# katotetsuro/chainer-maskrcnn

Measured on AMD Instinct MI355X. Metric: images/sec (1024^2 COCO, bs=2/GPU) at 1/2/4/8 MI355X; ROIAlign bwd HBM GB/s, higher is better.
Workload: dtype f32

## Files before the change

chainer-maskrcnn_amd/chainer_maskrcnn/_hip/nn.py:

```python
import torch

from chainer_maskrcnn import _hip
from chainer_maskrcnn._hip import lib, check, ptr, stream_ptr

_ws_cache = {}

PROFILE = None
LOGICAL = None


class _prof(object):
    def __init__(self, kind, n_out_pix, KH, KW, cin, cout, geom=None):
        self.on = PROFILE is not None
        if self.on:
            pass_ = {'fwd': 0, 'bwd_data': 1, 'bwd_filter': 2}[kind]
            executed = lib().mrcnn_conv2d_executed_macs(*geom, pass_) if geom is not None else n_out_pix * KH * KW * cin * cout
            if LOGICAL is not None:
                cin, cout = LOGICAL
            self.rec = [kind, n_out_pix * KH * KW * cin * cout, torch.cuda.Event(enable_timing=True),
                        torch.cuda.Event(enable_timing=True), (n_out_pix, KH, cin, cout), executed, geom,
                        winograd_pass_tiles(),
                        split_operands()]

    def __enter__(self):
# ... 35 lines not shown
    import ctypes
    t = (ctypes.c_int * 3)()
    check(lib().mrcnn_conv2d_get_winograd_pass_tiles(t))
    return (t[0], t[1], t[2])


def split_operands():
    import ctypes
    t = (ctypes.c_int * 3)()
    check(lib().mrcnn_conv2d_get_split_operands(t))
    return (t[0], t[1], t[2])


def set_winograd_pass_tiles(fwd, bwd_data, bwd_filter):
    check(lib().mrcnn_conv2d_set_winograd_pass_tiles(int(fwd), int(bwd_data), int(bwd_filter)))


def conv_out(n, k, s, p):
    return (n + 2 * p - k) // s + 1


CONV_PLAN_FIELDS = ('path', 'bm', 'bn', 'ksplit', 'tail_ks', 'wino_m', 'smallc', 'arithmetic', 'plane_gemm')
CONV_PATHS = ('direct', 'split_k', 'tail_split', 'winograd')


def conv_plan(pass_, x_shape, w_shape, stride, pad):
    import ctypes
    N, H, W, Cin = x_shape
    Cout, KH, KW, _ = w_shape
    out = (ctypes.c_int * len(CONV_PLAN_FIELDS))()
    check(lib().mrcnn_conv2d_plan_query(int(pass_), N, H, W, Cin, Cout, KH, KW, stride, pad, out, len(CONV_PLAN_FIELDS)))
    return dict(zip(CONV_PLAN_FIELDS, out))


def conv2d_fwd_raw(x, w, b, stride, pad, relu, keep_v=False):
    _hip.require_cuda(x, w)
    N, H, W, Cin = x.shape
    Cout, KH, KW, Cin2 = w.shape
    assert Cin == Cin2, (x.shape, w.shape)
    assert x.is_contiguous() and w.is_contiguous()
    y = torch.empty((N, conv_out(H, KH, stride, pad), conv_out(W, KW, stride, pad), Cout),
                    dtype=torch.float32, device=x.device)
    nb = lib().mrcnn_conv2d_workspace_bytes(N, H, W, Cin, Cout, KH, KW, stride, pad)
    ws = workspace(nb, x.device) if nb else None
    v = None
    if keep_v:
        vb = lib().mrcnn_conv2d_winograd_v_bytes(N, H, W, Cin, Cout, KH, KW, stride, pad)
        if vb:
            v = torch.empty((vb // 4,), dtype=torch.float32, device=x.device)
    with _prof('fwd', N * y.shape[1] * y.shape[2], KH, KW, Cin, Cout, (N, H, W, Cin, Cout, KH, KW, stride, pad)):
        check(lib().mrcnn_conv2d_fwd_f32(ptr(x), ptr(w), ptr(b), ptr(y), N, H, W, Cin, Cout, KH, KW,
                                         stride, pad, int(relu), ptr(v), ptr(ws), ws.numel() if ws is not None else 0, stream_ptr()))
    return (y, v) if keep_v else y


def conv2d_fwd_bnstats_raw(x, w, stride, pad, keep_v=False):
    N, H, W, Cin = x.shape
    Cout, KH, KW, _ = w.shape
    rows = lib().mrcnn_conv2d_bnstats_rows(N, H, W, Cin, Cout, KH, KW, stride, pad)
    if rows == 0:
        return None
    assert x.is_contiguous() and w.is_contiguous()
    y = torch.empty((N, conv_out(H, KH, stride, pad), conv_out(W, KW, stride, pad), Cout), dtype=torch.float32, device=x.device)
    part = torch.empty((rows, 2, Cout), dtype=torch.float32, device=x.device)
    nb = lib().mrcnn_conv2d_workspace_bytes(N, H, W, Cin, Cout, KH, KW, stride, pad)
    ws = workspace(nb, x.device) if nb else None
    v = None
    if keep_v:
        vb = lib().mrcnn_conv2d_winograd_v_bytes(N, H, W, Cin, Cout, KH, KW, stride, pad)
        if vb:
            v = torch.empty((vb // 4,), dtype=torch.float32, device=x.device)
    with _prof('fwd', N * y.shape[1] * y.shape[2], KH, KW, Cin, Cout, (N, H, W, Cin, Cout, KH, KW, stride, pad)):
        check(lib().mrcnn_conv2d_fwd_bnstats_f32(ptr(x), ptr(w), ptr(y), N, H, W, Cin, Cout, KH, KW, stride, pad, ptr(part), ptr(v),
                                                 ptr(ws), ws.numel() if ws is not None else 0, stream_ptr()))
    return y, v, part


def winograd_w_bytes(x_shape, w_shape, stride, pad):
    N, H, W, Cin = x_shape
    Cout, KH, KW, _ = w_shape
    return lib().mrcnn_conv2d_winograd_w_bytes(N, H, W, Cin, Cout, KH, KW, stride, pad)


def conv2d_bwd_data_raw(gy, w, x_shape, stride, pad, out=None, relu_x=None, emit_w=False, gb=None, gb_accumulate=False):
    N, H, W, Cin = x_shape
    Cout, KH, KW, _ = w.shape
    assert gy.is_contiguous()
    acc = out is not None
    gx = out if acc else torch.empty(x_shape, dtype=torch.float32, device=gy.device)
    nb = lib().mrcnn_conv2d_workspace_bytes(N, H, W, Cin, Cout, KH, KW, stride, pad)
    ws = workspace(nb, gy.device) if nb else None
    wt = None
    if emit_w:
        wb = lib().mrcnn_conv2d_winograd_w_bytes(N, H, W, Cin, Cout, KH, KW, stride, pad)
        assert wb > 0, 'emit_w: the layer does not take the Winograd path'
        wt = torch.empty((wb // 4,), dtype=torch.float32, device=gy.device)
    with _prof('bwd_data', N * gy.shape[1] * gy.shape[2], KH, KW, Cin, Cout, (N, H, W, Cin, Cout, KH, KW, stride, pad)):
        check(lib().mrcnn_conv2d_bwd_data_f32(ptr(gy), ptr(w), ptr(gx), ptr(relu_x), N, H, W, Cin, Cout, KH, KW,
                                              stride, pad, int(acc), ptr(wt), ptr(gb) if emit_w else None, int(gb_accumulate),
                                              ptr(ws), ws.numel() if ws is not None else 0, stream_ptr()))
    return (gx, wt) if emit_w else gx


def conv2d_bwd_filter_raw(x, gy, w_shape, stride, pad, want_bias, gw=None, gb=None, accumulate=None, wino_v=None,
                          wino_w=None):
    N, H, W, Cin = x.shape
    Cout, KH, KW, _ = w_shape
    assert gy.is_contiguous() and x.is_contiguous()
    acc = (gw is not None) if accumulate is None else bool(accumulate)
    if gw is None:
        gw = torch.empty(w_shape, dtype=torch.float32, device=x.device)
        gb = torch.empty((Cout,), dtype=torch.float32, device=x.device) if want_bias else None
    nbytes = lib().mrcnn_conv2d_bwd_filter_workspace_bytes(N, H, W, Cin, Cout, KH, KW, stride, pad)
    ws = workspace(nbytes, x.device)
    with _prof('bwd_filter', N * gy.shape[1] * gy.shape[2], KH, KW, Cin, Cout, (N, H, W, Cin, Cout, KH, KW, stride, pad)):
        check(lib().mrcnn_conv2d_bwd_filter_f32(ptr(x), ptr(gy), ptr(gw), ptr(gb) if want_bias else None, N, H, W, Cin,
                                                Cout, KH, KW, stride, pad, int(acc), ptr(wino_v), ptr(wino_w), ptr(ws), ws.numel(),
                                                stream_ptr()))
    return gw, gb
```

chainer-maskrcnn_amd/chainer_maskrcnn/model/fpn_maskrcnn_train_chain.py:

```python
import numpy as np
import torch

from chainer_maskrcnn._hip import ops
from chainer_maskrcnn.utils.proposal_target_creator import ProposalTargetCreator


class AnchorTargetCreator(object):

    def __init__(self, n_sample=256, pos_iou_thresh=0.7, neg_iou_thresh=0.3, pos_ratio=0.5):
        self.n_sample, self.pos_iou_thresh, self.neg_iou_thresh, self.pos_ratio = n_sample, pos_iou_thresh, neg_iou_thresh, pos_ratio
        self.keys = ops.KeyStream(1 << 32)

    seed = property(lambda self: self.keys.seed)

    def set_seed(self, seed, device=None):
        self.keys.set_seed(seed, device)

    def __call__(self, bbox, anchor, img_size, n_gt=None, keys=None, per_image_hw=None):
        if bbox.dim() == 2:
            bbox = bbox[None]
        N, G, _ = bbox.shape
        if n_gt is None:
            n_gt = torch.full((N,), G, dtype=torch.int32, device=bbox.device)
        if keys is None:
# ... 78 lines not shown


def select_gemm_arithmetic(name):
    from chainer_maskrcnn._hip import lib, check
    from chainer_maskrcnn.nn import core
    split, backbone_fwd = GEMM_ARITHMETIC[name]
    check(lib().mrcnn_conv2d_set_split_operands(*split))
    core.FWD_EMULATION_IN_BACKBONE = bool(backbone_fwd)


class _PendingBackward(object):

    def __init__(self, features, g_locs, g_scores, g_box, g_mask, g_later, g_iou, point, early_rpn):
        self.features = features
        self.g_locs, self.g_scores = g_locs, g_scores
        self.g_box, self.g_mask = g_box, g_mask
        self.g_later = g_later
        self.g_iou = g_iou
        self.point = point
        self.early_rpn = early_rpn

    def seeds(self):
        return ([self.g_locs, self.g_scores, self.g_box, self.g_mask] + list(self.g_later) + ([self.g_iou] if self.g_iou is not None else [])
                + ([self.point['g_pred']] if self.point is not None else []))


class FPNMaskRCNNTrainChain(object):
    EARLY_RPN_BACKWARD = True
    ACCUMULATE_INTO_EARLY_RPN = True

    def __init__(self, faster_rcnn, mask_loss_fun=calc_mask_loss, binary_mask=True, rpn_sigma=3., roi_sigma=1.,
                 anchor_target_creator=None, strict_batch1=False, mask_rows='positives', gemm_arithmetic=None,
                 box_loss='smooth_l1', rpn_box_loss='smooth_l1', box_loss_weight=1.0, rpn_box_loss_weight=1.0, mask_iou_weight=1.0,
                 point_loss_weight=1.0):
        box_loss_settings(box_loss, rpn_box_loss, box_loss_weight, rpn_box_loss_weight)
        self.mask_iou_weight = mask_iou_weight_setting(mask_iou_weight)
        self.point_loss_weight = point_loss_weight_setting(point_loss_weight)
        self.box_loss, self.rpn_box_loss = box_loss, rpn_box_loss
        self.box_loss_weight, self.rpn_box_loss_weight = float(box_loss_weight), float(rpn_box_loss_weight)
        if gemm_arithmetic is not None and gemm_arithmetic not in GEMM_ARITHMETIC:
            raise ValueError('gemm_arithmetic must be one of %s' % sorted(GEMM_ARITHMETIC))
        self.gemm_arithmetic = gemm_arithmetic
        self.faster_rcnn = faster_rcnn
        self.proposal_target_creator = ProposalTargetCreator(faster_rcnn.extractor.anchor_sizes)
        self.anchor_target_creator = AnchorTargetCreator()
        cascade = getattr(faster_rcnn, 'cascade', None)
        if cascade is not None and cascade[0][0] != float(self.proposal_target_creator.pos_iou_thresh):
            raise ValueError('cascade_ious[0] = %r is not the sampler\'s pos_iou_thresh %r'
                             % (cascade[0][0], self.proposal_target_creator.pos_iou_thresh))
        self.rpn_sigma, self.roi_sigma = 3., 1.
        self.loc_normalize_mean = faster_rcnn.loc_normalize_mean
        self.loc_normalize_std = faster_rcnn.loc_normalize_std
        if not callable(mask_loss_fun):
            raise TypeError('mask_loss_fun must be callable: f(roi_cls_mask, gt_roi_mask, xp, gt_roi_label) -> loss')
        self.mask_loss_fun = mask_loss_fun
        self.mask_loss_kind = getattr(mask_loss_fun, 'fused_kind', None)
        if self.mask_loss_kind not in ('mask_bce', 'keypoint_ce'):
            self.mask_loss_kind = 'generic'
        if getattr(faster_rcnn, 'maskiou_head', None) is not None and self.mask_loss_kind != 'mask_bce':
            raise ValueError('a mask_iou model trains with the fused binary mask loss (calc_mask_loss): a user-supplied mask_loss_fun '
                             're-orders the mask rows, which the MaskIoU target does not follow')
        if getattr(faster_rcnn, 'point_head', None) is not None and self.mask_loss_kind != 'mask_bce':
            raise ValueError('a point_rend model trains with the fused binary mask loss (calc_mask_loss): a user-supplied mask_loss_fun '
                             're-orders the mask rows, which the point targets do not follow')
        self.unit_upstream = False
        self.backward_follows = False
        self.binary_mask = binary_mask
        self.strict_batch1 = strict_batch1
        self.mask_rows = mask_rows
        self.observation = {}
        self.grad_ready_hook = None
        self.sampler_keys = None
        self.point_keys = None
        self._point_stream = ops.KeyStream(1 << 33)
        self.use_aux_stream = True
        self.keep_outputs = False
        self.outputs = {}
        self._aux = {}
        self._loss_rows, self._n_loss_rows = loss_rows(len(getattr(faster_rcnn, 'cascade_heads', [])),
                                                       getattr(faster_rcnn, 'maskiou_head', None) is not None,
                                                       getattr(faster_rcnn, 'point_head', None) is not None)
        self._row = dict(self._loss_rows)
        self.pending = None
        self._arith_found = None

    @property
    def key_streams(self):
        streams = {'proposal_target_creator': self.proposal_target_creator.keys, 'anchor_target_creator': self.anchor_target_creator.keys}
        if getattr(self.faster_rcnn, 'point_head', None) is not None:
            streams['point_rend'] = self._point_stream
        return streams

    def _aux_stream(self, dev):
        key = (dev.type, dev.index)
        if key not in self._aux:
            self._aux[key] = torch.cuda.Stream(device=dev)
        return self._aux[key]

    def __call__(self, imgs, bboxes, labels, masks, scale, n_gt=None, img_sizes=None):
        m = self.faster_rcnn
        n = bboxes.shape[0]
        if self.strict_batch1 and n != 1:
            raise ValueError('Currently only batch size 1 is supported. n={}'.format(n))
        if self.gemm_arithmetic is not None:
            if self._arith_found is None:
                from chainer_maskrcnn._hip import nn as hnn
                from chainer_maskrcnn.nn import core
                self._arith_found = (hnn.split_operands(), core.FWD_EMULATION_IN_BACKBONE)
            select_gemm_arithmetic(self.gemm_arithmetic)
        if torch.is_tensor(scale) and scale.numel() == 1:
            scale = float(scale.reshape(-1)[0].item())
        dev = imgs.device
        _, _, H, W = imgs.shape
        img_size = (H, W)
        per_hw = None
        if img_sizes is not None:
            per_hw = (img_sizes if torch.is_tensor(img_sizes) else torch.from_numpy(np.asarray(img_sizes, np.float32))).to(dev, torch.float32).contiguous()
        i32 = torch.int32
        bboxes = bboxes.contiguous()
        labels = labels.to(i32).contiguous()
        if n_gt is None:
            n_gt = ops.count_valid_labels(labels)

        main = torch.cuda.current_stream(dev)
        aux = self._aux_stream(dev) if self.use_aux_stream else main
        if getattr(m.head, 'merge_deconv', False):
            aux.wait_stream(main)
            with torch.cuda.stream(aux):
                m.head.compose_deconv(dev)
        features = m.extractor(m.to_nhwc4(imgs))
        m.rpn.train = True
        pk, ak = self.sampler_keys if self.sampler_keys is not None else (None, None)
        losses = torch.empty((self._n_loss_rows, 2), dtype=torch.float32, device=dev)
        rpn = {}

        def rpn_loss_branch(locs, scores, anchors):
            rpn.update(self._rpn_loss_branch(locs, scores, anchors, bboxes, img_size, n_gt, ak, per_hw, losses, main, aux))

        r = m.rpn.forward_padded(features, per_hw if per_hw is not None else img_size, scale, after_heads=rpn_loss_branch, batch_size=img_size)
        A = r['anchors'].shape[0]
        t = self.proposal_target_creator.sample_batch(
            r['rois'], r['levels'], r['n_rois'], bboxes, labels, n_gt,
            masks=masks.contiguous() if self.binary_mask else None,
            keypoints=None if self.binary_mask else masks.contiguous(),
            loc_normalize_mean=self.loc_normalize_mean, loc_normalize_std=self.loc_normalize_std,
            mask_size=m.head.mask_size, keys=pk, mask_rows=self.mask_rows)

        scales = m.extractor.spatial_scales
        aux.wait_stream(main)
        with torch.cuda.stream(aux):
            box, g_boxes, casc = self._box_stages(features, t, scales, bboxes, labels, n_gt,
                                                  per_hw if per_hw is not None else (float(H), float(W)), losses)
        m_rois, m_levels, m_label, mask_out, g_mask = self._mask_loss(features, t, scales, losses)
        iou = self._maskiou_branch(masks, n_gt, t, m_label, mask_out, losses) if getattr(m, 'maskiou_head', None) is not None else None
        pt = (self._point_branch(masks, n_gt, t, m_rois, m_label, mask_out, features, scales, losses)
              if getattr(m, 'point_head', None) is not None else None)

        main.wait_stream(aux)
        if aux is not main:
            rpn['g_locs'].record_stream(main)
            rpn['g_scores'].record_stream(main)
        total = ops.loss_total(losses)
        self.pending = _PendingBackward(features, rpn['g_locs'].view(n, A, 4), rpn['g_scores'].view(n, A, 2), g_boxes[0], g_mask, g_boxes[1:],
                                        iou['g_pred'] if iou is not None else None, pt, rpn.get('g_feats'))
        self._publish(losses, total, features, r, box, mask_out, casc, g_boxes, iou, pt, g_mask)
        self.targets = t
        self.rpn_targets = (rpn['loc'], rpn['label'])
        self.mask_inputs = (m_rois, m_levels, m_label)
        self.rpn_out = r
        self._anchor = torch.zeros((), device=dev, requires_grad=True)
        return _LossHandle.apply(self._anchor, self, total[0])

    def backward(self, upstream=None):
        m = self.faster_rcnn
        st = self.pending
        features = st.features
        if upstream is not None:
            from chainer_maskrcnn.functions.loss import _scale_
            for g_ in st.seeds():
                _scale_(g_, upstream)
        hook = self.grad_ready_hook
        dev = features[0].device
        main = torch.cuda.current_stream(dev)
        aux = self._aux_stream(dev) if self.use_aux_stream else main
        into_early = (self.ACCUMULATE_INTO_EARLY_RPN and st.early_rpn is not None and upstream is None
                      and len(st.early_rpn) == len(features))
        if into_early:
            g_feats = list(st.early_rpn)
            for g in g_feats:
                g.record_stream(main)
        else:
            g_feats = [torch.empty_like(f) for f in features]
        aux.wait_stream(main)
        with torch.cuda.stream(aux):
            self._box_stages_backward(st, g_feats, into_early)
        g_iou_in = m.maskiou_head.backward(st.g_iou) if st.g_iou is not None else None
        g_pt_in = m.point_head.backward(st.point['g_pred']) if st.point is not None else None
        g_pool = m.head.backward_mask_convs(st.g_mask)
        if g_iou_in is not None:
            self._maskiou_input_backward(g_iou_in, g_pool)
        main.wait_stream(aux)
        if self.keep_outputs and g_iou_in is not None:
            self.outputs.update(g_feats_box=[g.clone() for g in g_feats])
        m.head.backward_mask_pool(g_pool, g_feats)
        if g_pt_in is not None:
            self._point_input_backward(st.point, g_pt_in, g_feats)
        if self.keep_outputs and (st.g_later or g_iou_in is not None):
            self.outputs.update(g_mask_pool=g_pool, g_feats_heads=[g.clone() for g in g_feats])
        if hook:
            hook(self._offset_of('head/'))
        self._rpn_backward(st, g_feats, into_early, upstream, main)
        if hook:
            hook(self._offset_of('rpn/'))
        m.extractor.backward(g_feats, progress=(lambda prefix: hook(self._offset_of(prefix))) if hook else None)
        from chainer_maskrcnn.nn import core
        core.join_side_stream(features[0].device)
        if hook:
            hook(0)
        self.pending = None
        if self._arith_found is not None:
            from chainer_maskrcnn._hip import lib, check
            split, in_backbone = self._arith_found
            check(lib().mrcnn_conv2d_set_split_operands(*split))
            core.FWD_EMULATION_IN_BACKBONE = in_backbone
            self._arith_found = None

    def _rpn_loss_branch(self, locs, scores, anchors, bboxes, img_size, n_gt, keys, per_hw, losses, main, aux):
        m, row, br1 = self.faster_rcnn, self._row, {}
        n, A_ = bboxes.shape[0], anchors.shape[0]
        aux.wait_stream(main)
        with torch.cuda.stream(aux):
            br1['loc'], br1['label'] = self.anchor_target_creator(bboxes, anchors, img_size, n_gt=n_gt, keys=keys, per_image_hw=per_hw)
            if self.rpn_box_loss == 'smooth_l1':
                _, br1['g_locs'] = ops.smooth_l1(locs.view(n * A_, 4), 4, br1['loc'].view(n * A_, 4), br1['label'].view(-1),
                                                 n * A_, self.rpn_sigma, out=losses[row['rpn_loc_loss']])
            else:
                _, br1['g_locs'] = ops.box_iou_loss(locs.view(n * A_, 4), 4, br1['loc'].view(n * A_, 4), anchors, br1['label'].view(-1),
                                                    n * A_, self.rpn_box_loss, (0., 0., 0., 0.), (1., 1., 1., 1.),
                                                    weight=self.rpn_box_loss_weight, roi_period=A_, out=losses[row['rpn_loc_loss']])
            _, br1['g_scores'] = ops.softmax_ce(scores.view(n * A_, 2), br1['label'].view(-1), n * A_, 2, (1, 2, 0, 1),
                                                out=losses[row['rpn_cls_loss']])
            if self.EARLY_RPN_BACKWARD and self.backward_follows and aux is not main:
                for c1, c2, _, _ in m.rpn.tape:
                    for t_ in tuple(c1) + tuple(c2):
                        if torch.is_tensor(t_):
                            t_.record_stream(aux)
                br1['g_feats'] = m.rpn.backward(br1['g_locs'].view(n, A_, 4), br1['g_scores'].view(n, A_, 2), None)
        return br1

    def _rpn_backward(self, st, g_feats, into_early, upstream, main):
        if into_early:
            st.early_rpn = None
        elif st.early_rpn is not None:
            if upstream is not None:
                raise RuntimeError('the RPN backward pass ran early with d(objective)/d(loss) = 1 (backward_follows was set): '
                                   'a scaled loss needs chain.backward_follows = False during the forward call')
            for gf, g in zip(g_feats, st.early_rpn):
                gf.add_(g)
                g.record_stream(main)
            st.early_rpn = None
        else:
            self.faster_rcnn.rpn.backward(st.g_locs, st.g_scores, g_feats)

    def _box_stage_losses(self, box, roi, gt_loc, label, std, loc_row, cls_row):
        head = self.faster_rcnn.head
        R, ld = label.shape[0], head.out_p
        g_box = torch.empty_like(box)
        ops.softmax_ce(box, label, R, head.n_class, (1, ld, 0, 1), Kfill=head.LOC0, gx=g_box, out=cls_row)
        if self.box_loss == 'smooth_l1':
            ops.smooth_l1(box, ld, gt_loc, label, R, self.roi_sigma, gfill=ld - head.LOC0, col0=head.LOC0, gx=g_box, out=loc_row)
        else:
            ops.box_iou_loss(box, ld, gt_loc, roi, label, R, self.box_loss, self.loc_normalize_mean, std, weight=self.box_loss_weight,
                             roi_period=R, gfill=ld - head.LOC0, col0=head.LOC0, gx=g_box, out=loc_row)
        return g_box

    def _box_stages(self, features, t, scales, bboxes, labels, n_gt, img_hw, losses):
        m, row = self.faster_rcnn, self._row
        head, n = m.head, bboxes.shape[0]
        box = head.box_branch(features, t['rois_xy5'], t['sample_levels'], scales)
        g_boxes = [self._box_stage_losses(box, t['sample_roi'], t['gt_roi_loc'], t['gt_roi_label'], self.loc_normalize_std,
                                          losses[row['roi_loc_loss']], losses[row['roi_cls_loss']])]
        casc = []
        prev = dict(roi=t['sample_roi'], label=t['gt_roi_label'], box=box)
        for k, stage in enumerate(getattr(m, 'cascade_heads', []), 2):
            ious, stds = m.cascade
            ref = ops.cascade_refine(prev['roi'], prev['box'], head.LOC0, n, self.loc_normalize_mean, stds[k - 2], img_hw,
                                     prev_label=prev['label'], gt_boxes=bboxes, gt_labels=labels, n_gt=n_gt, iou_thresh=ious[k - 1],
                                     std_next=stds[k - 1])
            ref['box'] = stage.box_branch(features, ref['rois_xy5'], ref['levels'], scales)
            g_boxes.append(self._box_stage_losses(ref['box'], ref['roi'], ref['gt_loc'], ref['label'], stds[k - 1],
                                                  losses[row['roi_loc_loss_s%d' % k]], losses[row['roi_cls_loss_s%d' % k]]))
            casc.append(ref)
            prev = ref
        return box, g_boxes, casc

    def _box_stages_backward(self, st, g_feats, into_early):
        m = self.faster_rcnn
        m.head.backward_box(st.g_box, g_feats, accumulate=into_early)
        for stage, g_k in zip(getattr(m, 'cascade_heads', []), st.g_later):
            stage.backward_box(g_k, g_feats, accumulate=True)

    def _mask_loss(self, features, t, scales, losses):
        head = self.faster_rcnn.head
        if self.mask_loss_kind == 'generic':
            g_mask = self._generic_mask_loss(t, features, scales, losses)
            return self._generic_inputs + (None, g_mask)
        S, rows = self.proposal_target_creator.n_sample, t['mask_rows']
        n = t['rois_xy5'].shape[0] // S
        if rows == S:
            m_rois, m_levels, m_label = t['rois_xy5'], t['sample_levels'], t['gt_roi_label']
        else:
            m_rois = t['rois_xy5'].view(n, S, 5)[:, :rows].reshape(n * rows, 5)
            m_levels = t['sample_levels'].view(n, S)[:, :rows].reshape(n * rows)
            m_label = t['gt_roi_label'].view(n, S)[:, :rows].reshape(n * rows)
        mask_out = head.mask_branch(features, m_rois, m_levels, scales)
        out = losses[self._row['mask_loss']]
        if self.mask_loss_kind == 'mask_bce':
            _, g_mask = ops.mask_bce(mask_out, t['gt_roi_mask'], m_label, out=out)
        else:
            Rm, Hm, Wm, Cm = mask_out.shape
            K = head.n_keypoints
            xmap = (K, Hm * Wm * Cm, 1, Cm)
            g_mask = torch.empty_like(mask_out) if ops.softmax_ce_fills_gradient(Rm * K, Hm * Wm, xmap) else torch.zeros_like(mask_out)
            ops.softmax_ce(mask_out, t['gt_roi_mask'].view(-1), Rm * K, Hm * Wm, xmap, gx=g_mask, out=out)
        return m_rois, m_levels, m_label, mask_out, g_mask

    def _generic_mask_loss(self, t, features, scales, losses):
        from chainer_maskrcnn.functions import loss as FL
        m = self.faster_rcnn
        head = m.head
        S = self.proposal_target_creator.n_sample
        n = t['n_pos'].shape[0]
        n_pos = [int(v) for v in t['n_pos'].cpu().tolist()]
        n_smp = [int(v) for v in t['n_sampled'].cpu().tolist()]
        rows_of = lambda x, lo, hi: [x.view(n, S, *x.shape[1:])[i, lo(i):hi(i)] for i in range(n)]
        order = lambda x: torch.cat(rows_of(x, lambda i: 0, lambda i: n_pos[i]) +
                                    rows_of(x, lambda i: n_pos[i], lambda i: n_smp[i]), 0).contiguous()
        m_rois, m_levels, m_label = order(t['rois_xy5']), order(t['sample_levels']), order(t['gt_roi_label'])
        rows = t['mask_rows']
        gt = t['gt_roi_mask']
        gt = torch.cat([gt.view(n, rows, *gt.shape[1:])[i, :n_pos[i]] for i in range(n)], 0).contiguous()
        self._generic_inputs = (m_rois, m_levels, m_label)
        mask_out = head.mask_branch(features, m_rois, m_levels, scales)
        leaf = mask_out.detach().requires_grad_(True)
        C = head.mask_out_channels
        with torch.enable_grad():
            x = FL.nhwc_to_nchw(leaf, C).as_subclass(FL.MaskLogits)
            loss = self.mask_loss_fun(x, gt, FL.XP(leaf.device), m_label)
            if not torch.is_tensor(loss) or loss.numel() != 1:
                raise TypeError('mask_loss_fun must return a scalar tensor')
            (g_mask,) = torch.autograd.grad(loss.reshape(()), leaf)
        out = losses[self._row['mask_loss']]
        out[0].copy_(loss.detach().reshape(()))
        out[1].fill_(1.0)
        return g_mask.contiguous()

    def _maskiou_branch(self, masks, n_gt, t, m_label, mask_out, losses):
        m = self.faster_rcnn
        mh, S = m.maskiou_head, self.proposal_target_creator.n_sample
        m_label = m_label.contiguous()
        iou = ops.maskiou_target(masks.contiguous(), n_gt, t['sample_roi'], t['gt_assign'], m_label, t['n_pos'], S, t['mask_rows'], mask_out,
                                 t['gt_roi_mask'], mh.out_channels, label_base=1, want_counts=self.keep_outputs)
        iou['input'] = mh.assemble(m.head.last_mask_pool, mask_out, m_label, label_base=1)
        iou['pred'] = mh.forward(iou['input'])
        _, iou['g_pred'] = ops.maskiou_l2(iou['pred'], iou['target'], m_label, mh.out_channels, weight=self.mask_iou_weight, label_base=1,
                                          out=losses[self._row['maskiou_loss']])
        return iou

    def _maskiou_input_backward(self, g_iou_in, g_pool):
        if self.keep_outputs:
            self.outputs.update(g_mask_pool_convs=g_pool.clone(), g_maskiou_in=g_iou_in)
        ops.maskiou_input_bwd(g_iou_in, g_pool)

    def _point_branch(self, masks, n_gt, t, m_rois, m_label, mask_out, features, scales, losses):
        m = self.faster_rcnn
        ph, st, S = m.point_head, m.point_rend, self.proposal_target_creator.n_sample
        m_label, m_rois = m_label.contiguous(), m_rois.contiguous()
        keys = self.point_keys
        if keys is None:
            keys = self._point_stream.draw((mask_out.shape[0], ops.point_n_keys(st['train_points'], st['n_candidates'], st['n_important'])),
                                           mask_out.device)
        pt = dict(coords=ops.point_train_coords(keys, mask_out, m_label, ph.out_channels, st['train_points'], st['n_candidates'],
                                                st['n_important'], label_base=1), rois=m_rois)
        pt['input'] = ph.assemble(pt['coords'], m_rois, features[0], scales[0], mask_out)
        pt['pred'] = ph.forward(pt['input'])
        pt['target'] = ops.point_target(masks.contiguous(), n_gt, m_rois, t['gt_assign'], m_label, t['n_pos'], S, t['mask_rows'], pt['coords'])
        _, pt['g_pred'] = ops.point_bce(pt['pred'], pt['target'], m_label, ph.out_channels, weight=self.point_loss_weight, label_base=1,
                                        out=losses[self._row['point_loss']])
        return pt

    def _point_input_backward(self, pt, g_pt_in, g_feats):
        if self.keep_outputs:
            pt['g_in'] = g_pt_in
            self.outputs.update(g_feats0_heads=g_feats[0].clone())
        ops.point_features_bwd(g_pt_in, pt['coords'], pt['rois'], self.faster_rcnn.extractor.spatial_scales[0], g_feats[0])
        if self.keep_outputs:
            self.outputs.update(g_feats0_point=g_feats[0].clone())

    def _publish(self, losses, total, features, r, box, mask_out, casc, g_boxes, iou, pt, g_mask):
        self.observation = {}
        for key, row in self._loss_rows:
# ... 19 lines not shown
```

chainer-maskrcnn_amd/chainer_maskrcnn/model/head/fpn_roi_mask_head.py:

```python
import ctypes

import numpy as np
import torch

from chainer_maskrcnn import _hip
from chainer_maskrcnn._hip import lib, check, ptr, stream_ptr, ops
from chainer_maskrcnn._hip.nn import workspace
from chainer_maskrcnn.nn.core import Conv, GroupNorm, ParamStore, normal, pad_to


def _level_args(xs, scales):
    L = len(xs)
    arr_p = (ctypes.c_void_p * L)(*[x.data_ptr() for x in xs])
    Hs = (ctypes.c_int * L)(*[x.shape[1] for x in xs])
    Ws = (ctypes.c_int * L)(*[x.shape[2] for x in xs])
    sc = (ctypes.c_float * L)(*[float(s) for s in scales])
    return L, arr_p, Hs, Ws, sc


def roi_align_fpn_fwd(xs, rois_xy5, levels, out_size, scales, sampling_ratio=2):
    _hip.require_cuda(rois_xy5, levels, *xs)
    L, arr_p, Hs, Ws, sc = _level_args(xs, scales)
    N, C = xs[0].shape[0], xs[0].shape[3]
    R = rois_xy5.shape[0]
# ... 225 lines not shown
class FPNRoIMaskHead(FPNRoIBoxHead):
    mask_size = 28
    keep_mask_pool = False
    last_mask_pool = None

    def __init__(self, n_class, roi_size_box, roi_size_mask, loc_initialW=None, score_initialW=None,
                 mask_initialW=None, ps=None, prefix='head', in_channels=256, fc_channels=1024,
                 n_mask_convs=4, mask_out_channels=None, upsample2x=False, mask_conv_names=None, norm=None, gn_groups=32):
        super().__init__(n_class, roi_size_box, loc_initialW=loc_initialW, score_initialW=score_initialW, ps=ps, prefix=prefix,
                         in_channels=in_channels, fc_channels=fc_channels, norm=norm, gn_groups=gn_groups)
        self.roi_size_mask = roi_size_mask
        c = in_channels
        gn = norm == 'gn'
        p = prefix + '/'
        mi = 0.01 if mask_initialW is None else mask_initialW
        names = mask_conv_names or ['mask%d' % (i + 1) for i in range(n_mask_convs)]
        self.mask_convs, self.mask_gns = [], []
        for nm in names:
            self.mask_convs.append(Conv(self.ps, p + nm, c, c, 3, 1, 1, relu=not gn, fwd_tile=0))
            self.mask_gns.append(GroupNorm(self.ps, p + nm + '/gn', c, gn_groups) if gn else None)
        self.mask_out_channels = (n_class - 1) if mask_out_channels is None else mask_out_channels
        self.upsample2x = upsample2x
        self.deconv1 = Conv(self.ps, p + 'deconv1', c, 4 * c, 1, bias=False, init=normal(mi))
        self.ps.register(p + 'deconv1/b', (c,), lambda rs: np.zeros((c,), np.float32))
        self.deconv_b = p + 'deconv1/b'
        self.conv2 = Conv(self.ps, p + 'conv2', c, self.mask_out_channels, 1, init=normal(mi))
        self.merge_deconv = (c % 8 == 0)

    def mask_branch(self, xs, rois_xy5, levels, spatial_scales):
        pool = roi_align_fpn_fwd(xs, rois_xy5, levels, self.roi_size_mask, spatial_scales)
        if self.keep_mask_pool:
            self.last_mask_pool = pool
        h, tapes = pool, []
        for cv, gn in zip(self.mask_convs, self.mask_gns):
            h, t = cv.fwd(h)
            nt = None
            if gn is not None:
                h, nt = gn.fwd(h, relu=True)
            tapes.append((t, nt))
        if self.merge_deconv:
            m, td, t2 = self._merged_deconv_fwd(h)
        else:
            d, td = self.deconv1.fwd(h)
            up = ops.pixel_shuffle2x(d, bias=self.ps.p(self.deconv_b))
            m, t2 = self.conv2.fwd(up)
        if self.upsample2x:
            m = ops.bilinear2x_fwd(m)
        from chainer_maskrcnn.nn import core
        plan = _plan_beside_forward(xs, rois_xy5, levels, self.roi_size_mask, spatial_scales) if core.TRAIN else None
        self.mask_tape = (tapes, td, t2, rois_xy5, levels, spatial_scales, plan)
        return m

    def compose_deconv(self, device):
        dc, c2, C = self.deconv1, self.conv2, self.channels
        K2 = c2.cout_p
        wm = torch.empty((4 * K2, 1, 1, dc.cin_p), dtype=torch.float32, device=device)
        bm = torch.empty((K2,), dtype=torch.float32, device=device)
        check(lib().mrcnn_deconv_merge_fwd_f32(ptr(dc.W), ptr(self.ps.p(self.deconv_b)), ptr(c2.W), ptr(c2.b), ptr(wm), ptr(bm),
                                               C, dc.cin_p, K2, c2.cin_p, stream_ptr()))
        ev = torch.cuda.Event()
        ev.record(torch.cuda.current_stream(device))
        self._composed = (wm, bm, ev)
        return wm, bm, ev

    def _merged_deconv_fwd(self, h):
        from chainer_maskrcnn._hip import nn as hnn
        dc, c2 = self.deconv1, self.conv2
        composed = getattr(self, '_composed', None)
        self._composed = None
        wm, bm, ev = composed if composed is not None else self.compose_deconv(h.device)
        self._composed = None
        cur = torch.cuda.current_stream(h.device)
        cur.wait_event(ev)
        wm.record_stream(cur)
        bm.record_stream(cur)
        hnn.LOGICAL = (dc.cin, 4 * c2.cout)
        try:
            d = hnn.conv2d_fwd_raw(h, wm, None, 1, 0, False)
        finally:
            hnn.LOGICAL = None
        m = ops.pixel_shuffle2x(d, bias=bm)
        return m, (h, wm), None

    def _merged_deconv_bwd(self, td, g_mask):
        from chainer_maskrcnn._hip import nn as hnn
        dc, c2, C = self.deconv1, self.conv2, self.channels
        x_in, wm = td
        K2 = c2.cout_p
        g4 = ops.pixel_shuffle2x(g_mask, inverse=True)
        hnn.LOGICAL = (dc.cin, 4 * c2.cout)
        try:
            G, gb4 = hnn.conv2d_bwd_filter_raw(x_in, g4, tuple(wm.shape), 1, 0, True)
            g = hnn.conv2d_bwd_data_raw(g4, wm, tuple(x_in.shape), 1, 0, relu_x=x_in if self.mask_convs else None)
        finally:
            hnn.LOGICAL = None
        ps = self.ps
        check(lib().mrcnn_deconv_merge_bwd_f32(ptr(G), ptr(gb4), ptr(dc.W), ptr(ps.p(self.deconv_b)), ptr(c2.W),
                                               ptr(ps.g(dc.name + '/W')), ptr(ps.g(self.deconv_b)), ptr(ps.g(c2.name + '/W')),
                                               ptr(ps.g(c2.name + '/b')) if c2.has_bias else None, C, dc.cin_p, K2, c2.cin_p,
                                               stream_ptr()))
        return g

    def __call__(self, x, indices_and_rois, levels, spatial_scales, train=True):
        xy5 = indices_and_rois[:, [0, 2, 1, 4, 3]].contiguous()
        lv = levels.to(torch.int32).contiguous()
        o = self.box_branch(x, xy5, lv, spatial_scales)
        locs, scores = o[:, self.LOC0:self.LOC0 + 4], o[:, :self.n_class]
        if not train:
            self.x = x
            return locs, scores
        m = self.mask_branch(x, xy5, lv, spatial_scales)
        return locs, scores, m[..., :self.mask_out_channels].permute(0, 3, 1, 2)

    def predict_mask(self, levels, indices_and_rois, spatial_scales):
        xy5 = indices_and_rois[:, [0, 2, 1, 4, 3]].contiguous()
        m = self.mask_branch(self.x, xy5, levels.to(torch.int32).contiguous(), spatial_scales)
        return m[..., :self.mask_out_channels].permute(0, 3, 1, 2)

    def backward(self, g_box_out, g_mask, g_feats):
        self.backward_box(g_box_out, g_feats)
        if g_mask is not None:
            self.backward_mask_pool(self.backward_mask_convs(g_mask), g_feats)

    def backward_mask_convs(self, g_mask):
        from chainer_maskrcnn._hip import nn as hnn
        tapes, td, tc2, rois, levels, scales, _ = self.mask_tape
        if self.upsample2x:
            g_mask = ops.bilinear2x_bwd(g_mask)
        if self.merge_deconv:
            g = self._merged_deconv_bwd(td, g_mask)
            n = len(self.mask_convs)
            for i in range(n - 1, -1, -1):
                t, nt = tapes[i]
                if self.mask_gns[i] is not None:
                    g = self.mask_gns[i].bwd(nt, g, gy_masked=True)
                g = self.mask_convs[i].bwd(t, g, gy_masked=True, mask_gx=(i > 0))
            return g
        g = self.conv2.bwd(tc2, g_mask)
        g4 = ops.pixel_shuffle2x(g, inverse=True)
        C = self.channels
        gb4 = torch.empty((4 * C,), dtype=torch.float32, device=g.device)
        gw = self.ps.g(self.deconv1.name + '/W')
        x_in = td[0]
        hnn.conv2d_bwd_filter_raw(x_in, g4, tuple(gw.shape), 1, 0, True, gw=gw, gb=gb4, accumulate=False)
        gb = self.ps.g(self.deconv_b)
        ops.add(gb4[0:C], gb4[C:2 * C], out=gb)
        ops.add(gb, gb4[2 * C:3 * C], out=gb)
        ops.add(gb, gb4[3 * C:4 * C], out=gb)
        g = hnn.conv2d_bwd_data_raw(g4, self.deconv1.W, tuple(x_in.shape), 1, 0)
        for cv, gn, (t, nt) in zip(reversed(self.mask_convs), reversed(self.mask_gns), reversed(tapes)):
            if gn is not None:
                g = gn.bwd(nt, g)
            g = cv.bwd(t, g)
        return g

    def backward_mask_pool(self, g_pool, g_feats):
        tapes, td, tc2, rois, levels, scales, plan = self.mask_tape
        roi_align_fpn_bwd(g_pool, g_feats, rois, levels, self.roi_size_mask, scales, accumulate=True, plan=plan)
        self.mask_tape = None
```

chainer-maskrcnn_amd/chainer_maskrcnn/nn/core.py:

```python
import math

import numpy as np
import torch

from chainer_maskrcnn._hip import nn as hnn
from chainer_maskrcnn._hip import ops


TRAIN = True

FILTER_GRAD_ON_SIDE_STREAM = True
WINOGRAD_SHARED_GY_TRANSFORM = False
LAYER_TILE_HINTS = True
FWD_TILE_RULE = None
FUSE_BN_STATS = True
FWD_EMULATION_BEHIND_BACKBONE = True
FWD_EMULATION_IN_BACKBONE = True
COMPOSITE_BLOCKS = True


class _layer_tiles(object):
    def __init__(self, conv):
        self.t = FWD_TILE_RULE(conv.name) if FWD_TILE_RULE is not None else (conv.fwd_tile if LAYER_TILE_HINTS else None)
        self.keep = None
        self.behind = not conv.in_backbone

    def __enter__(self):
        self.keep_split = None
        if (not FWD_EMULATION_BEHIND_BACKBONE and self.behind) or (not FWD_EMULATION_IN_BACKBONE and not self.behind):
            sp = hnn.split_operands()
            if sp[0] == 3:
                self.keep_split = sp
                from chainer_maskrcnn._hip import lib, check
                check(lib().mrcnn_conv2d_set_split_operands(0, sp[1], sp[2]))
        if self.t is None:
            return
        cur = hnn.winograd_pass_tiles()
        if cur[0] == 2 and cur[0] != self.t:
            self.keep = cur
            hnn.set_winograd_pass_tiles(self.t, cur[1], cur[2])

    def __exit__(self, *a):
        if self.keep is not None:
            hnn.set_winograd_pass_tiles(*self.keep)
        if self.keep_split is not None:
            from chainer_maskrcnn._hip import lib, check
            check(lib().mrcnn_conv2d_set_split_operands(*self.keep_split))


def join_side_stream(device):
    torch.cuda.current_stream(device).wait_stream(hnn.side_stream(device))


def pad_to(n, m):
    return (n + m - 1) // m * m


class ParamStore(object):

    ALIGN = 64

    def __init__(self):
        self._specs = []
        self.offsets = {}
        self.params = self.grads = self.momentum = None
        self.size = 0
        self.buffers = {}
        self._views = {}
        self.frozen = frozenset()
        self.frozen_mask = None

    def register(self, name, shape, init, trainable=True):
        if name in self.offsets:
            raise KeyError('duplicate parameter %s' % name)
        n = int(np.prod(shape))
        if trainable:
            self.offsets[name] = (self.size, tuple(shape))
            self.size += pad_to(n, self.ALIGN)
        self._specs.append((name, tuple(shape), init, trainable))

    def materialise(self, device, seed=1234):
        rs = np.random.RandomState(seed)
        host = np.zeros((self.size,), np.float32)
        for name, shape, init, trainable in self._specs:
            v = np.asarray(init(rs), np.float32).reshape(shape)
            if trainable:
                o = self.offsets[name][0]
                host[o:o + v.size] = v.ravel()
            else:
                self.buffers[name] = torch.from_numpy(v.copy()).to(device)
        self.params = torch.from_numpy(host).to(device)
        self.grads = torch.zeros_like(self.params)
        self.momentum = torch.zeros_like(self.params)
        self._views = {}
        return self
# ... 23 lines not shown
        v = cache[1].get(name)
        if v is None:
            o, shape = self.offsets[name]
            v = cache[1][name] = flat[o:o + int(np.prod(shape))].view(shape)
        return v

    def p(self, name):
        return self._view(self.params, name)

    def g(self, name):
        return self._view(self.grads, name)

    def names(self):
        return list(self.offsets)

    def n_params(self):
        return sum(int(np.prod(s)) for _, s in self.offsets.values())


def lecun_normal(fan_in):
    return lambda shape: (lambda rs: rs.standard_normal(shape) * (1.0 / math.sqrt(fan_in)))


def normal(std):
    return lambda shape: (lambda rs: rs.standard_normal(shape) * std)


class Conv(object):

    def __init__(self, ps, name, cin, cout, k=1, stride=1, pad=0, bias=True, relu=False, init=None,
                 cin_p=None, cout_p=None, cout_index=None, fwd_tile=None, in_backbone=None):
        self.ps, self.name, self.fwd_tile = ps, name, fwd_tile
        self.in_backbone = ('/resnet/' in name) if in_backbone is None else bool(in_backbone)
        self.cin, self.cout, self.k, self.stride, self.pad, self.relu = cin, cout, k, stride, pad, relu
        self.cin_p = cin_p or (4 if cin <= 4 else pad_to(cin, 32))
        self.cout_p = cout_p or pad_to(cout, 32)
        self.has_bias = bias
        idx = np.arange(cout) if cout_index is None else np.asarray(cout_index)
        fan_in = cin * k * k
        gen = (init or lecun_normal(fan_in))((cout, k, k, cin))

        def w_init(rs):
            w = np.zeros((self.cout_p, k, k, self.cin_p), np.float32)
            w[idx, :, :, :cin] = gen(rs)
            return w
        ps.register(name + '/W', (self.cout_p, k, k, self.cin_p), w_init)
        if bias:
            ps.register(name + '/b', (self.cout_p,), lambda rs: np.zeros((self.cout_p,), np.float32))

    @property
    def W(self):
        return self.ps.p(self.name + '/W')

    @property
    def b(self):
        return self.ps.p(self.name + '/b') if self.has_bias else None

    @property
    def gW(self):
        return self.ps.g(self.name + '/W')

    def fwd(self, x, relu=None, bn_stats=False, tape=True):
        relu = self.relu if relu is None else relu
        self.last_bn_part = None
        hnn.LOGICAL = (self.cin, self.cout)
        if not tape:
            with _layer_tiles(self):
                y = hnn.conv2d_fwd_raw(x, self.W, self.b, self.stride, self.pad, relu)
            hnn.LOGICAL = None
            return y, None
        if bn_stats and FUSE_BN_STATS and TRAIN and not relu and not self.has_bias:
            with _layer_tiles(self):
                res = hnn.conv2d_fwd_bnstats_raw(x, self.W, self.stride, self.pad, keep_v=True)
            if res is not None:
                hnn.LOGICAL = None
                y, v, self.last_bn_part = res
                return y, (x, None, v)
        with _layer_tiles(self):
            y, v = hnn.conv2d_fwd_raw(x, self.W, self.b, self.stride, self.pad, relu, keep_v=True) if TRAIN else \
                (hnn.conv2d_fwd_raw(x, self.W, self.b, self.stride, self.pad, relu), None)
        hnn.LOGICAL = None
        return y, (x, y if relu else None, v)

    def bwd(self, ctx, gy, need_gx=True, gx_acc=None, accumulate_params=False, gy_masked=False, mask_gx=False):
        with _layer_tiles(self):
            return self._bwd(ctx, gy, need_gx, gx_acc, accumulate_params, gy_masked, mask_gx)

    def _bwd(self, ctx, gy, need_gx, gx_acc, accumulate_params, gy_masked, mask_gx):
        x, y, v = ctx
        if y is not None and not gy_masked:
            gy = ops.relu_bwd(gy, y)
        gw = self.gW
        gb = self.ps.g(self.name + '/b') if self.has_bias else None
        hnn.LOGICAL = (self.cin, self.cout)
        try:
            if WINOGRAD_SHARED_GY_TRANSFORM and need_gx and self.stride == 1 and hnn.winograd_w_bytes(tuple(x.shape), tuple(gw.shape), 1, self.pad) > 0:
                assert not (mask_gx and gx_acc is not None)
                gx, wt = hnn.conv2d_bwd_data_raw(gy, self.W, tuple(x.shape), 1, self.pad, out=gx_acc, relu_x=x if mask_gx else None,
                                                 emit_w=True, gb=gb, gb_accumulate=accumulate_params)
                main = torch.cuda.current_stream(gy.device)
                side = hnn.side_stream(gy.device) if (FILTER_GRAD_ON_SIDE_STREAM and hnn.PROFILE is None) else main
                side.wait_stream(main)
                with torch.cuda.stream(side):
                    hnn.conv2d_bwd_filter_raw(x, gy, tuple(gw.shape), 1, self.pad, False, gw=gw, gb=None,
                                              accumulate=accumulate_params, wino_v=v, wino_w=wt)
                if side is not main:
                    for t_ in (gy, x, v, wt):
                        if t_ is not None:
                            t_.record_stream(side)
                return gx
            if FILTER_GRAD_ON_SIDE_STREAM and hnn.PROFILE is None:
                main = torch.cuda.current_stream(gy.device)
                side = hnn.side_stream(gy.device)
                side.wait_stream(main)
                with torch.cuda.stream(side):
                    hnn.conv2d_bwd_filter_raw(x, gy, tuple(gw.shape), self.stride, self.pad, self.has_bias, gw=gw, gb=gb,
                                              accumulate=accumulate_params, wino_v=v)
                gy.record_stream(side)
                x.record_stream(side)
                if v is not None:
                    v.record_stream(side)
            else:
                hnn.conv2d_bwd_filter_raw(x, gy, tuple(gw.shape), self.stride, self.pad, self.has_bias, gw=gw, gb=gb,
                                          accumulate=accumulate_params, wino_v=v)
            if not need_gx:
                return None
            if self.stride == 1:
                assert not (mask_gx and gx_acc is not None) or self.k == 1
                return hnn.conv2d_bwd_data_raw(gy, self.W, tuple(x.shape), 1, self.pad, out=gx_acc,
                                               relu_x=x if mask_gx else None)
            if self.k > 1:
                assert self.k == 2 * self.pad + 1 and gx_acc is None, 'strided k x k backward-data: odd kernel with "same" padding'
                N, H, W, _ = x.shape
                g_up = ops.subsample_bwd(gy, (N, H, W, gy.shape[3]), self.stride)
                return hnn.conv2d_bwd_data_raw(g_up, self.W, tuple(x.shape), 1, self.pad, relu_x=x if mask_gx else None)
            assert self.pad == 0, 'strided backward-data of a 1x1 convolution takes no padding'
            g_sub = self.bwd_data_sub(gy)
        finally:
            hnn.LOGICAL = None
        return ops.subsample_bwd(g_sub, tuple(x.shape), self.stride, gx=gx_acc, relu_x=x if mask_gx else None)

    def bwd_data_sub(self, gy, out=None):
        N, Ho, Wo, _ = gy.shape
        keep = hnn.LOGICAL
        hnn.LOGICAL = (self.cin, self.cout)
        g = hnn.conv2d_bwd_data_raw(gy, self.W, (N, Ho, Wo, self.cin_p), 1, 0, out=out)
        hnn.LOGICAL = keep
        return g


class _ColsGemm(Conv):

    def __init__(self, conv):
        self.ps, self.name, self.fwd_tile, self.in_backbone = conv.ps, conv.name, None, conv.in_backbone
        self.cin, self.cout, self.k, self.stride, self.pad, self.relu = 9 * conv.cin, conv.cout, 1, 1, 0, False
        self.cin_p, self.cout_p, self.has_bias = 9 * conv.cin_p, conv.cout_p, False

    @property
    def W(self):
        return self.ps.p(self.name + '/W').view(self.cout_p, 1, 1, self.cin_p)

    @property
    def gW(self):
        return self.ps.g(self.name + '/W').view(self.cout_p, 1, 1, self.cin_p)


class DeformConv(Conv):

    def __init__(self, ps, name, cin, cout, modulated=False, init=None, in_backbone=None):
        Conv.__init__(self, ps, name, cin, cout, 3, 1, 1, bias=False, init=init, in_backbone=in_backbone)
        self.modulated = bool(modulated)
        self.n_offset = 27 if self.modulated else 18
        zeros = lambda shape: (lambda rs: np.zeros(shape, np.float32))
        self.offset = Conv(ps, name + '_offset', cin, self.n_offset, 3, 1, 1, bias=True, init=zeros, in_backbone=False)
        self.gemm = _ColsGemm(self)

    def fwd(self, x, relu=None, bn_stats=False, tape=True):
        off, octx = self.offset.fwd(x, relu=False, tape=tape)
        cols = ops.deform_cols_fwd(x, off, self.modulated)
        y, gctx = self.gemm.fwd(cols, relu=self.relu if relu is None else relu, bn_stats=bn_stats, tape=tape)
        self.last_bn_part = self.gemm.last_bn_part
        return y, ((x, off, octx, gctx) if tape else None)

    def bwd(self, ctx, gy, need_gx=True, gx_acc=None, accumulate_params=False, gy_masked=False, mask_gx=False):
        x, off, octx, gctx = ctx
        g_cols = self.gemm.bwd(gctx, gy, accumulate_params=accumulate_params, gy_masked=gy_masked)
        g_off = ops.deform_offset_bwd(g_cols, x, off, self.modulated)
        if not need_gx:
            self.offset.bwd(octx, g_off, need_gx=False, accumulate_params=accumulate_params)
            return None
        gx = self.offset.bwd(octx, g_off, gx_acc=gx_acc, accumulate_params=accumulate_params)
        return ops.deform_input_bwd(g_cols, off, self.modulated, tuple(x.shape), gx=gx, relu_x=x if mask_gx else None)


class BatchNorm(object):

    def __init__(self, ps, name, c):
        self.ps, self.name, self.c = ps, name, c
        self.frozen = False
        ps.register(name + '/gamma', (c,), lambda rs: np.ones((c,), np.float32))
        ps.register(name + '/beta', (c,), lambda rs: np.zeros((c,), np.float32))
        ps.register(name + '/avg_mean', (c,), lambda rs: np.zeros((c,), np.float32), trainable=False)
        ps.register(name + '/avg_var', (c,), lambda rs: np.ones((c,), np.float32), trainable=False)

    def fwd(self, x, relu=False, residual=None, partials=None):
        gamma, beta = self.ps.p(self.name + '/gamma'), self.ps.p(self.name + '/beta')
        if not TRAIN or self.frozen:
            y = ops.bn_infer_fwd(x, gamma, beta, self.ps.buffers[self.name + '/avg_mean'], self.ps.buffers[self.name + '/avg_var'],
                                 residual, relu)
            if not TRAIN:
                return y, None
            return y, ('frozen', y if relu else None)
        if partials is not None and partials.shape[2] == x.shape[-1]:
# ... 282 lines not shown
```

chainer-maskrcnn_amd/csrc/conv.hip:

```cpp
#include "common.h"
#include "bn_common.h"
#include <algorithm>
#include <cstdlib>

namespace {

typedef float f32x16 __attribute__((ext_vector_type(16)));

constexpr int BK = 32;
constexpr int LDK = BK + 4;
constexpr int CONV_THREADS = 256;

enum { MODE_FWD = 0, MODE_BWD_DATA = 1, MODE_BWD_FILTER = 2 };

struct ConvP {
    const float *a;
    const float *b;
    float *c;
    const float *bias;
    const float *relu_x;
    int N, H, W, Cin;
    int Ho, Wo, Cout;
    int KH, KW, stride, pad;
    int pad_w;
// ... 1201 lines not shown
        const float p12 = D[1] + D[2], m12 = D[1] - D[2], p34 = D[3] + D[4], m34 = D[3] - D[4];
        r[0] = (0.25f * D[0] - p12 * (1.0f / 6.0f)) + p34 * (1.0f / 24.0f);
        r[1] = m34 * (1.0f / 12.0f) - m12 * (1.0f / 6.0f);
        r[2] = (p34 * (1.0f / 6.0f) - p12 * (1.0f / 6.0f)) + D[5];
    }
}

template <int M_>
__device__ __forceinline__ void wino_filter_body(const float *__restrict__ w, float *__restrict__ U, int Cout, int Cin,
                                                 int transposed, unsigned blk, int uplanes = 0) {
    constexpr int A_ = M_ + 2;
    const int i = (int)(blk * 256u + threadIdx.x);
    if (i >= Cout * Cin) return;
    const int ci = transposed ? i / Cout : i % Cin, co = transposed ? i % Cout : i / Cin;
    float t[A_][3];
#pragma unroll
    for (int v = 0; v < 3; ++v) {
        float g[3], c[A_];
#pragma unroll
        for (int u = 0; u < 3; ++u) {
            const int uu = transposed ? 2 - u : u, vv = transposed ? 2 - v : v;
            g[u] = w[(((size_t)co * 3 + uu) * 3 + vv) * Cin + ci];
        }
        wino_g<M_>(g, c);
#pragma unroll
        for (int r = 0; r < A_; ++r) t[r][v] = c[r];
    }
    const size_t stride = (size_t)Cout * Cin;
    const size_t o = transposed ? (size_t)ci * Cout + co : (size_t)co * Cin + ci;
    if (uplanes) {
        const unsigned rows = transposed ? (unsigned)Cin : (unsigned)Cout, cols = transposed ? (unsigned)Cout : (unsigned)Cin;
        const unsigned rr = transposed ? (unsigned)ci : (unsigned)co, cc = transposed ? (unsigned)co : (unsigned)ci;
        unsigned short *Up = reinterpret_cast<unsigned short *>(U);
#pragma unroll
        for (int r = 0; r < A_; ++r) {
            float row[A_];
            wino_g<M_>(t[r], row);
#pragma unroll
            for (int q = 0; q < A_; ++q) {
                const unsigned off = pg_off_r4((unsigned)(r * A_ + q) * rows + rr, cc & ~3u, cols) / 2u + (cc & 3u);
                const float v = row[q];
                const __bf16 h = (__bf16)v;
                const float r1 = v - (float)h;
                const __bf16 m = (__bf16)r1;
                const __bf16 l = (__bf16)(r1 - (float)m);
                Up[off] = __builtin_bit_cast(unsigned short, h);
                Up[off + 64] = __builtin_bit_cast(unsigned short, m);
                Up[off + 128] = __builtin_bit_cast(unsigned short, l);
            }
        }
        return;
    }
#pragma unroll
    for (int r = 0; r < A_; ++r) {
        float row[A_];
        wino_g<M_>(t[r], row);
#pragma unroll
        for (int q = 0; q < A_; ++q) U[(size_t)(r * A_ + q) * stride + o] = row[q];
    }
}
template <int M_>
__global__ __launch_bounds__(256) void k_wino_filter(const float *__restrict__ w, float *__restrict__ U, int Cout, int Cin,
                                                     int transposed, int uplanes) {
    wino_filter_body<M_>(w, U, Cout, Cin, transposed, blockIdx.x, uplanes);
}

typedef unsigned u32x4 __attribute__((ext_vector_type(4)));
__device__ __forceinline__ V4 v4buf(__amdgpu_buffer_rsrc_t rs, unsigned voff, unsigned soff) {
    const u32x4 v = __builtin_amdgcn_raw_buffer_load_b128(rs, voff, soff, 0);
    return {__uint_as_float(v.x), __uint_as_float(v.y), __uint_as_float(v.z), __uint_as_float(v.w)};
}
__device__ __forceinline__ V4 v4buf_nt(__amdgpu_buffer_rsrc_t rs, unsigned voff, unsigned soff) {
    const u32x4 v = __builtin_amdgcn_raw_buffer_load_b128(rs, voff, soff, 2);
    return {__uint_as_float(v.x), __uint_as_float(v.y), __uint_as_float(v.z), __uint_as_float(v.w)};
}
__device__ __forceinline__ void v4bufst(__amdgpu_buffer_rsrc_t rs, unsigned voff, unsigned soff, V4 v) {
    const u32x4 d = {__float_as_uint(v.x), __float_as_uint(v.y), __float_as_uint(v.z), __float_as_uint(v.w)};
    __builtin_amdgcn_raw_buffer_store_b128(d, rs, voff, soff, 0);
}
struct InBN { const float *gamma, *beta, *mean, *invstd; };
template <int M_>
__device__ __forceinline__ void wino_input_body(const float *__restrict__ x, float *__restrict__ V, int N, int H, int W, int C,
                                                int th, int tw, long long T, long long Tp, unsigned blk, const InBN bn = InBN{},
                                                int panel = 0) {
    constexpr int A_ = M_ + 2;
    const unsigned C4 = (unsigned)C / 4u;
    const unsigned i = blk * 256u + threadIdx.x;
    if (i >= (unsigned)Tp * C4) return;
    unsigned t = i / C4;
    const int c = (int)(i - t * C4) * 4;
    const unsigned ks = (unsigned)((size_t)Tp * C * 4);
    const auto rsV = __builtin_amdgcn_make_buffer_rsrc((void *)V, 0, (unsigned)((size_t)A_ * A_ * Tp * C * 4), 0x00020000);
    if (panel > 1 && t < (unsigned)T) {
        const unsigned per = (unsigned)th * (unsigned)tw, pw = (unsigned)panel;
        const unsigned n0 = t / per, q = t - n0 * per;
        const unsigned full = (unsigned)tw / pw * pw, nf = (unsigned)th * full;
        unsigned ty0, tx0;
        if (q < nf) {
            const unsigned pp = q / ((unsigned)th * pw), r = q - pp * (unsigned)th * pw;
            ty0 = r / pw; tx0 = pp * pw + (r - ty0 * pw);
        } else {
            const unsigned wr = (unsigned)tw - full, q2 = q - nf;
            ty0 = q2 / wr; tx0 = full + (q2 - ty0 * wr);
        }
        t = n0 * per + ty0 * (unsigned)tw + tx0;
    }
    const unsigned vo = (unsigned)(((size_t)t * C + c) * 4);
    if (t >= (unsigned)T) {
#pragma unroll
        for (int k = 0; k < A_ * A_; ++k) v4bufst(rsV, vo + (unsigned)k * ks, 0, v4zero());
        return;
    }
    const unsigned trow = t / (unsigned)tw;
    const int tx = (int)(t - trow * (unsigned)tw);
    const int n = (int)(trow / (unsigned)th);
    const int ty = (int)(trow - (unsigned)n * (unsigned)th);
    const auto rsX = __builtin_amdgcn_make_buffer_rsrc((void *)x, 0, (unsigned)((size_t)N * H * W * C * 4), 0x00020000);
    const unsigned OOB = 0xFFFFFFFFu;
    unsigned rowo[A_], colo[A_];
#pragma unroll
    for (int r = 0; r < A_; ++r) {
        const int h = M_ * ty - 1 + r, ww = M_ * tx - 1 + r;
        rowo[r] = (unsigned)h < (unsigned)H ? (unsigned)(((size_t)n * H + h) * W * C * 4) : OOB;
        colo[r] = (unsigned)ww < (unsigned)W ? (unsigned)(((size_t)ww * C + c) * 4) : OOB;
    }
    V4 bg = v4zero(), bb = v4zero(), bm = v4zero(), bs = v4zero();
    if (bn.gamma) { bg = v4ld(bn.gamma + c); bb = v4ld(bn.beta + c); bm = v4ld(bn.mean + c); bs = v4ld(bn.invstd + c); }
    V4 b[A_][A_];
#pragma unroll
    for (int q = 0; q < A_; ++q) {
        V4 d[A_], r[A_];
#pragma unroll
        for (int rr = 0; rr < A_; ++rr) d[rr] = v4buf(rsX, (rowo[rr] == OOB || colo[q] == OOB) ? OOB : rowo[rr] + colo[q], 0);
        if (bn.gamma) {
#pragma unroll
            for (int rr = 0; rr < A_; ++rr) {
                const bool in = !(rowo[rr] == OOB || colo[q] == OOB);
                const V4 v = d[rr];
                V4 o;
                o.x = relu1(bn_affine1(v.x, bg.x, bm.x, bs.x, bb.x)); o.y = relu1(bn_affine1(v.y, bg.y, bm.y, bs.y, bb.y));
                o.z = relu1(bn_affine1(v.z, bg.z, bm.z, bs.z, bb.z)); o.w = relu1(bn_affine1(v.w, bg.w, bm.w, bs.w, bb.w));
                d[rr] = in ? o : v4zero();
            }
        }
        wino_bt<M_, V4>(d, r);
#pragma unroll
        for (int rr = 0; rr < A_; ++rr) b[rr][q] = r[rr];
    }
#pragma unroll
    for (int rr = 0; rr < A_; ++rr) {
        V4 row[A_];
        wino_bt<M_, V4>(b[rr], row);
#pragma unroll
        for (int q = 0; q < A_; ++q) v4bufst(rsV, vo + (unsigned)(rr * A_ + q) * ks, 0, row[q]);
    }
}
__device__ __forceinline__ unsigned xcd_banded(unsigned g, unsigned first, unsigned nb, int on) {
    const unsigned b = g - first;
    if (!on) return b;
    const unsigned f0 = first & 7u, n2 = nb + f0, b2 = b + f0;
    const unsigned q = n2 >> 3, r = n2 & 7u, xcd = b2 & 7u;
    const unsigned v2 = (xcd < r ? xcd * (q + 1) : r * (q + 1) + (xcd - r) * q) + (b2 >> 3);
    return v2 - min(xcd + 1u, f0);
}
template <int M_>
__global__ __launch_bounds__(256) void k_wino_input(const float *__restrict__ x, float *__restrict__ V, int N, int H, int W, int C,
                                                    int th, int tw, long long T, long long Tp, int banded, InBN bn) {
    wino_input_body<M_>(x, V, N, H, W, C, th, tw, T, Tp, xcd_banded(blockIdx.x, 0, gridDim.x, banded), bn, banded);
}
template <int M_>
__global__ __launch_bounds__(256) void k_wino_input_filter(const float *__restrict__ x, float *__restrict__ V, int N, int H, int W, int C,
                                                           int th, int tw, long long T, long long Tp, const float *__restrict__ w,
                                                           float *__restrict__ U, int Cout_w, int Cin_w, int transposed, unsigned fblocks,
                                                           int banded, int uplanes, InBN bn) {
    if (blockIdx.x < fblocks) wino_filter_body<M_>(w, U, Cout_w, Cin_w, transposed, blockIdx.x, uplanes);
    else wino_input_body<M_>(x, V, N, H, W, C, th, tw, T, Tp, xcd_banded(blockIdx.x, fblocks, gridDim.x - fblocks, banded), bn, banded);
}

template <int M_>
__global__ __launch_bounds__(256) void k_wino_output(const float *__restrict__ Mb, float *__restrict__ y, int N, int H, int W, int C,
                                                     int th, int tw, long long T, long long Tp, const float *__restrict__ bias,
                                                     int relu, int accumulate, const float *__restrict__ relu_x,
                                                     float *__restrict__ bn_part) {
    constexpr int A_ = M_ + 2;
    __shared__ float4 sred[2][256];
    const unsigned C4 = (unsigned)C / 4u;
    const unsigned i = blockIdx.x * 256u + threadIdx.x;
    V4 bs = v4zero(), bq = v4zero();
    if (i < (unsigned)T * C4) {
        const unsigned t = i / C4;
        const int c = (int)(i - t * C4) * 4;
        const unsigned trow = t / (unsigned)tw;
        const int tx = (int)(t - trow * (unsigned)tw);
        const int n = (int)(trow / (unsigned)th);
        const int ty = (int)(trow - (unsigned)n * (unsigned)th);
        const unsigned ks = (unsigned)((size_t)Tp * C * 4);
        const auto rsM = __builtin_amdgcn_make_buffer_rsrc((void *)Mb, 0, (unsigned)((size_t)A_ * A_ * Tp * C * 4), 0x00020000);
        const unsigned ybytes = (unsigned)((size_t)N * H * W * C * 4);
        const auto rsY = __builtin_amdgcn_make_buffer_rsrc((void *)y, 0, ybytes, 0x00020000);
        const auto rsR = __builtin_amdgcn_make_buffer_rsrc((void *)relu_x, 0, relu_x ? ybytes : 0u, 0x00020000);
        const unsigned mo = (unsigned)(((size_t)t * C + c) * 4);
        V4 s[M_][A_];
#pragma unroll
        for (int q = 0; q < A_; ++q) {
            V4 m[A_], r[M_];
#pragma unroll
            for (int rr = 0; rr < A_; ++rr) m[rr] = v4buf_nt(rsM, mo, (unsigned)(rr * A_ + q) * ks);
            wino_at<M_, V4>(m, r);
#pragma unroll
            for (int a = 0; a < M_; ++a) s[a][q] = r[a];
        }
        const V4 bv = bias ? v4ld(bias + c) : v4zero();
        const unsigned OOB = 0xFFFFFFFFu;
#pragma unroll
        for (int a = 0; a < M_; ++a) {
            V4 row[M_], old[M_], xm[M_];
            wino_at<M_, V4>(s[a], row);
            const int h = M_ * ty + a;
            unsigned off[M_];
#pragma unroll
            for (int b = 0; b < M_; ++b) {
                const int ww = M_ * tx + b;
                off[b] = (h < H && ww < W) ? (unsigned)((((size_t)n * H + h) * W + ww) * C + c) * 4u : OOB;
            }
            if (accumulate) {
#pragma unroll
                for (int b = 0; b < M_; ++b) old[b] = v4buf(rsY, off[b], 0);
            }
            if (relu_x) {
#pragma unroll
                for (int b = 0; b < M_; ++b) xm[b] = v4buf(rsR, off[b], 0);
            }
#pragma unroll
            for (int b = 0; b < M_; ++b) {
                V4 v = row[b] + bv;
                if (relu) { v.x = fmaxf(v.x, 0.f); v.y = fmaxf(v.y, 0.f); v.z = fmaxf(v.z, 0.f); v.w = fmaxf(v.w, 0.f); }
                if (accumulate) v = v + old[b];
                if (relu_x) {
                    v.x = xm[b].x > 0.f ? v.x : 0.f; v.y = xm[b].y > 0.f ? v.y : 0.f; v.z = xm[b].z > 0.f ? v.z : 0.f; v.w = xm[b].w > 0.f ? v.w : 0.f;
                }
                v4bufst(rsY, off[b], 0, v);
                if (off[b] != OOB) {
                    bs = bs + v;
                    bq.x = fmaf(v.x, v.x, bq.x); bq.y = fmaf(v.y, v.y, bq.y); bq.z = fmaf(v.z, v.z, bq.z); bq.w = fmaf(v.w, v.w, bq.w);
                }
            }
        }
    }
    if (bn_part) {
        sred[0][threadIdx.x] = make_float4(bs.x, bs.y, bs.z, bs.w);
        sred[1][threadIdx.x] = make_float4(bq.x, bq.y, bq.z, bq.w);
        __syncthreads();
        if (threadIdx.x < C4) {
            float4 a = sred[0][threadIdx.x], b2 = sred[1][threadIdx.x];
            for (unsigned k = threadIdx.x + C4; k < 256; k += C4) {
                const float4 q = sred[0][k], r = sred[1][k];
                a.x += q.x; a.y += q.y; a.z += q.z; a.w += q.w;
                b2.x += r.x; b2.y += r.y; b2.z += r.z; b2.w += r.w;
            }
            *reinterpret_cast<float4 *>(bn_part + ((size_t)blockIdx.x * 2) * C + threadIdx.x * 4) = a;
            *reinterpret_cast<float4 *>(bn_part + ((size_t)blockIdx.x * 2 + 1) * C + threadIdx.x * 4) = b2;
        }
    }
}

template <int M_>
__global__ __launch_bounds__(256) void k_wino_gy(const float *__restrict__ gy, float *__restrict__ Wt, int N, int H, int W, int C,
                                                 int th, int tw, long long T, long long Tp, float *__restrict__ bias_part, int wplanes) {
    constexpr int A_ = M_ + 2;
    __shared__ float4 sred[256];
    const unsigned C4 = (unsigned)C / 4u;
    const unsigned i = blockIdx.x * 256u + threadIdx.x;
    const bool in_range = i < (unsigned)Tp * C4;
    const unsigned t = in_range ? i / C4 : (unsigned)Tp;
    const int c = in_range ? (int)(i - t * C4) * 4 : 0;
    V4 bsum = v4zero();
    const unsigned ks = wplanes ? (unsigned)((size_t)Tp * C * 6) : (unsigned)((size_t)Tp * C * 4);
    const auto rsW = __builtin_amdgcn_make_buffer_rsrc((void *)Wt, 0, (unsigned)((size_t)A_ * A_ * ks), 0x00020000);
    const unsigned vo = wplanes ? (unsigned)(((size_t)t * 3 * C + c) * 2) : (unsigned)(((size_t)t * C + c) * 4);
    typedef unsigned u32x2 __attribute__((ext_vector_type(2)));
    auto put = [&](unsigned off, V4 v) {
        if (!wplanes) { v4bufst(rsW, off, 0, v); return; }
        uint2 hi, mid, lo;
        split3_bf16x4(make_float4(v.x, v.y, v.z, v.w), hi, mid, lo);
        __builtin_amdgcn_raw_buffer_store_b64(u32x2{hi.x, hi.y}, rsW, off, 0, 0);
        __builtin_amdgcn_raw_buffer_store_b64(u32x2{mid.x, mid.y}, rsW, off + (unsigned)C * 2u, 0, 0);
        __builtin_amdgcn_raw_buffer_store_b64(u32x2{lo.x, lo.y}, rsW, off + (unsigned)C * 4u, 0, 0);
    };
    if (in_range && t >= (unsigned)T) {
#pragma unroll
        for (int k = 0; k < A_ * A_; ++k) put(vo + (unsigned)k * ks, v4zero());
    } else if (in_range) {
        const unsigned trow = t / (unsigned)tw;
        const int tx = (int)(t - trow * (unsigned)tw);
        const int n = (int)(trow / (unsigned)th);
        const int ty = (int)(trow - (unsigned)n * (unsigned)th);
        const auto rsG = __builtin_amdgcn_make_buffer_rsrc((void *)gy, 0, (unsigned)((size_t)N * H * W * C * 4), 0x00020000);
        V4 r[A_][M_];
#pragma unroll
        for (int b = 0; b < M_; ++b) {
            const int ww = M_ * tx + b;
            V4 y[M_], col[A_];
#pragma unroll
            for (int a = 0; a < M_; ++a) {
                const int h = M_ * ty + a;
                y[a] = v4buf(rsG, (h < H && ww < W) ? (unsigned)((((size_t)n * H + h) * W + ww) * C + c) * 4u : 0xFFFFFFFFu, 0);
                bsum = bsum + y[a];
            }
            wino_a<M_, V4>(y, col, v4zero());
#pragma unroll
            for (int q = 0; q < A_; ++q) r[q][b] = col[q];
        }
#pragma unroll
        for (int q = 0; q < A_; ++q) {
            V4 row[A_];
            wino_a<M_, V4>(r[q], row, v4zero());
#pragma unroll
            for (int j = 0; j < A_; ++j) put(vo + (unsigned)(q * A_ + j) * ks, row[j]);
        }
    }
    if (bias_part) {
        sred[threadIdx.x] = make_float4(bsum.x, bsum.y, bsum.z, bsum.w);
        __syncthreads();
        if (threadIdx.x < C4) {
            float4 a = sred[threadIdx.x];
            for (unsigned k = threadIdx.x + C4; k < 256; k += C4) {
                const float4 q = sred[k];
                a.x += q.x; a.y += q.y; a.z += q.z; a.w += q.w;
            }
            *reinterpret_cast<float4 *>(bias_part + (size_t)blockIdx.x * C + threadIdx.x * 4) = a;
        }
    }
}

template <int M_>
__global__ __launch_bounds__(256) void k_wino_gy_dual(const float *__restrict__ gy, float *__restrict__ V, float *__restrict__ Wt,
                                                      float *__restrict__ bias_part, int N, int H, int W, int C, int th, int tw,
                                                      long long T, long long Tp) {
    constexpr int A_ = M_ + 2;
    __shared__ float4 sred[256];
    const int C4 = C / 4;
    const size_t ks = (size_t)Tp * C;
    V4 bsum = v4zero();
    const long long total = Tp * C4;
    for (long long i = (long long)blockIdx.x * 256 + threadIdx.x; i < total; i += (long long)gridDim.x * 256) {
        const int c = (int)(i % C4) * 4;
        const long long t = i / C4;
        if (t >= T) {
#pragma unroll
            for (int k = 0; k < A_ * A_; ++k) {
                v4st(V + ((size_t)k * Tp + t) * C + c, v4zero());
                v4st(Wt + ((size_t)k * Tp + t) * C + c, v4zero());
            }
            continue;
        }
        const int tx = (int)(t % tw);
        const int ty = (int)((t / tw) % th);
        const int n = (int)(t / ((long long)tw * th));
        {
            V4 b[A_][A_];
#pragma unroll
            for (int q = 0; q < A_; ++q) {
                const int ww = M_ * tx - 1 + q;
                V4 d[A_], r[A_];
#pragma unroll
                for (int rr = 0; rr < A_; ++rr) {
                    const int h = M_ * ty - 1 + rr;
                    const bool ok = (unsigned)h < (unsigned)H && (unsigned)ww < (unsigned)W;
                    d[rr] = ok ? v4ld(gy + (((size_t)n * H + h) * W + ww) * C + c) : v4zero();
                }
                wino_bt<M_, V4>(d, r);
// ... 61 lines not shown
        for (int j = 0; j < A_; ++j) Dall[q][j] = dU[o0 + (size_t)(q * A_ + j) * Cin];
    for (int sl = 1; sl < nslab; ++sl) {
        const float *ds = dU + (size_t)sl * Cout * (A_ * A_) * Cin + o0;
#pragma unroll
        for (int q = 0; q < A_; ++q)
#pragma unroll
            for (int j = 0; j < A_; ++j) Dall[q][j] += ds[(size_t)(q * A_ + j) * Cin];
    }
    float old[3][3];
    if (accumulate) {
#pragma unroll
        for (int u = 0; u < 3; ++u)
#pragma unroll
            for (int v = 0; v < 3; ++v) old[u][v] = gw[(((size_t)co * 3 + u) * 3 + v) * Cin + ci];
    }
    float r[3][A_];
#pragma unroll
    for (int j = 0; j < A_; ++j) {
        float D[A_], c3[3];
#pragma unroll
        for (int q = 0; q < A_; ++q) D[q] = Dall[q][j];
        wino_gt<M_>(D, c3);
#pragma unroll
        for (int u = 0; u < 3; ++u) r[u][j] = c3[u];
    }
#pragma unroll
    for (int u = 0; u < 3; ++u) {
        float o[3];
        wino_gt<M_>(r[u], o);
#pragma unroll
        for (int v = 0; v < 3; ++v) gw[(((size_t)co * 3 + u) * 3 + v) * Cin + ci] = accumulate ? old[u][v] + o[v] : o[v];
    }
}

#define WINO_LAUNCH(KERN, G, GRID, ...)                                                              \
    do {                                                                                             \
        if (g_debug_skip & 2) break;                                                                 \
        if ((G).m == 2) hipLaunchKernelGGL((KERN<2>), GRID, dim3(256), 0, st, __VA_ARGS__);          \
        else hipLaunchKernelGGL((KERN<4>), GRID, dim3(256), 0, st, __VA_ARGS__);                     \
        MRCNN_LAUNCH_CHECK();                                                                        \
    } while (0)

#define WINO_LAUNCH_OUT(G, GRID, ...) WINO_LAUNCH(k_wino_output, G, GRID, __VA_ARGS__)

int g_pg_big = 1, g_pg_min_tiles = 256;
bool pg_big_g_ok(const WinoGeom &g, int Cin, int Cout) {
    if (g_split_mode[PASS_BWD_FILTER] != 3 || !g_pg_big) return false;
    if (Cout % PGB_BM || Cin % PGB_BN || g.Tp % 32) return false;
    return g.Tp >= 2048 && (long long)g.nk * g.Tp * Cout * 6 < (1ll << 32) && (long long)g.nk * g.Tp * Cin * 4 < (1ll << 32);
}
struct WinoFLayout { size_t v, w, slabs, du, total; WinoGeom g; int ksplit, kchunk; int big; int ks32, kc32; };
ConvP wino_filter_p(const WinoGeom &g, int Cin, int Cout) {
    ConvP p = make_p(ConvGeom{1, 1, (int)g.Tp, Cin, Cout, 1, 1, 1, 0});
    p.wbatch_rows = (int)g.Tp; p.wbatch_n = g.nk;
    bwd_filter_gemm(p);
    return p;
}
WinoFLayout wino_filter_layout(const ConvGeom &cg) {
    const int Cin = cg.Cin, Cout = cg.Cout;
    WinoFLayout L;
    L.g = wino_geom(cg, PASS_BWD_FILTER);
    ConvP p = wino_filter_p(L.g, Cin, Cout);
    filter_plan(p, L.ksplit, L.kchunk);
    L.ks32 = L.ksplit; L.kc32 = L.kchunk;
    L.big = pg_big_g_ok(L.g, Cin, Cout) ? 1 : 0;
    if (L.big) {
        const long long tiles = (long long)L.g.nk * (Cout / PGB_BM) * (Cin / PGB_BN);
        long long ks = std::max(1ll, (long long)g_cus() / tiles);
        ks = std::min(ks, std::max(1ll, L.g.Tp / 256));
        L.kchunk = (int)((L.g.Tp / 32 + ks - 1) / ks * 32);
        L.ksplit = (int)((L.g.Tp + L.kchunk - 1) / L.kchunk);
    }
    auto al = [](size_t b) { return (b + 255) / 256 * 256; };
    size_t o = 0;
    L.v = o; o += al((size_t)L.g.nk * L.g.Tp * Cin * 4);
    L.w = o; o += al((size_t)L.g.nk * L.g.Tp * Cout * 6);
    L.slabs = o; o += al((size_t)std::max(L.ksplit, L.ks32) * Cout * L.g.nk * Cin * 4);
    L.du = o; o += al((size_t)Cout * L.g.nk * Cin * 4);
    L.total = o;
    return L;
}

int wino_bwd_filter(const float *x, const float *gy, float *gw, const ConvGeom &cg, const InBN &inbn, int accumulate, void *ws,
                    hipStream_t st, const float *v_cached, const float *w_cached, float *bias_part = nullptr, int *bias_rows = nullptr) {
    const int N = cg.N, H = cg.H, W = cg.W, Cin = cg.Cin, Cout = cg.Cout;
    const WinoFLayout L = wino_filter_layout(cg);
    const WinoGeom &g = L.g;
    char *base = (char *)ws;
    float *Vw = (float *)(base + L.v), *Wt = (float *)(base + L.w), *slabs = (float *)(base + L.slabs), *dU = (float *)(base + L.du);
    const float *V = v_cached ? v_cached : Vw;
    const long long nin = g.Tp * (Cin / 4), nout = g.Tp * (Cout / 4);
    if (!v_cached) WINO_LAUNCH(k_wino_input, g, dim3((unsigned)((nin + 255) / 256)), x, Vw, N, H, W, Cin, g.th, g.tw, g.T, g.Tp, g_wino_banded, inbn);
    const int C4o = Cout / 4;
    const bool fuse_bias = bias_part && bias_rows && !w_cached && C4o <= 256 && 256 % C4o == 0 && !(g_debug_skip & 2);
    if (bias_rows) *bias_rows = fuse_bias ? (int)((nout + 255) / 256) : 0;
    const int big = (L.big && !w_cached) ? 1 : 0;
    if (!w_cached) WINO_LAUNCH(k_wino_gy, g, dim3((unsigned)((nout + 255) / 256)), gy, Wt, N, H, W, Cout, g.th, g.tw, g.T, g.Tp,
                               fuse_bias ? bias_part : (float *)nullptr, big);
    const int ksplit = big ? L.ksplit : L.ks32;
    const size_t n4 = (size_t)Cout * g.nk * Cin / 4;
    if (big) {
        PlaneGemmP q{};
        q.a = reinterpret_cast<const unsigned short *>(Wt); q.b = reinterpret_cast<const unsigned short *>(V);
        q.c = ksplit > 1 ? slabs : dU;
        q.M = Cout; q.N = Cin; q.K = (int)g.Tp; q.batch_rows = (int)g.Tp; q.nbatch = g.nk; q.ksplit = ksplit; q.kchunk = L.kchunk;
        q.bytes_a = (unsigned)((size_t)g.nk * g.Tp * Cout * 6); q.bytes_b = (unsigned)((size_t)g.nk * g.Tp * Cin * 4);
        q.ldc = g.nk * Cin; q.dbg = 0; q.stamps = nullptr;
        if (!(g_debug_skip & 1)) launch_pgemm<5>(q, PGB_BM, PGB_BN, st);
        MRCNN_LAUNCH_CHECK();
        if (ksplit > 1) if (int e = sum_slabs(slabs, dU, n4, ksplit, 0, st)) return e;
        WINO_LAUNCH(k_wino_filter_grad, g, dim3(mrcnn::cdiv(Cout * Cin, 256)), dU, gw, Cout, Cin, accumulate, 1);
        return 0;
    }
    ConvP p = wino_filter_p(g, Cin, Cout);
    p.ksplit = ksplit; p.kchunk = L.kc32;
    p.a = w_cached ? w_cached : Wt; p.b = V; p.c = ksplit > 1 ? slabs : dU;
    p.bytes_a = (unsigned)((size_t)g.nk * g.Tp * Cout * 4); p.bytes_b = (unsigned)((size_t)g.nk * g.Tp * Cin * 4);
    launch_conv<MODE_BWD_FILTER>(p, g.nk * ksplit, filter_tile(p), PASS_BWD_FILTER, st);
    MRCNN_LAUNCH_CHECK();
    if (ksplit > 1) if (int e = sum_slabs(slabs, dU, n4, ksplit, 0, st)) return e;
    WINO_LAUNCH(k_wino_filter_grad, g, dim3(mrcnn::cdiv(Cout * Cin, 256)), dU, gw, Cout, Cin, accumulate, 1);
    return 0;
}

bool pg_big_ok(int pass, const WinoGeom &g, int K, int Nn) {
    if (g_split_mode[pass] != 3 || !g_pg_big) return false;
    if (g.Tp % PGB_BM || Nn % PGB_BN || K % 16) return false;
    const long long tiles = (long long)g.nk * g.Tp / PGB_BM * (Nn / PGB_BN);
    const long long rounds = (tiles + g_cus() - 1) / g_cus();
    if (tiles * 10 < rounds * g_cus() * 8) return false;
    return tiles >= g_pg_min_tiles && (long long)g.nk * g.Tp * K * 4 < (1ll << 32) && (long long)g.nk * Nn * K * 6 < (1ll << 32);
}

int wino_gemm_p(ConvP &p, const WinoGeom &g, int Cin, int Cout) {
    p = make_p(ConvGeom{1, 1, (int)(g.nk * g.Tp), Cin, Cout, 1, 1, 1, 0});
    p.M = (int)(g.nk * g.Tp); p.Ng = Cout;
    p.wbatch_rows = (int)g.Tp; p.wbatch_n = g.nk;
    return Cin / BK;
}

int wino_conv(const float *in, const float *w, float *out, const ConvGeom &cg, int pass, const InBN &inbn,
              const float *bias, int relu, int accumulate, const float *relu_x, void *ws, size_t ws_bytes, hipStream_t st,
              float *v_keep, float *w_keep = nullptr, float *gbias = nullptr, int gbias_accumulate = 0, float *bn_part = nullptr) {
    const int N = cg.N, H = cg.H, W = cg.W, Cin = cg.Cin, Cout = cg.Cout;
    const bool transposed = pass == PASS_BWD_DATA;
    const WinoLayout L = wino_layout(cg, pass);
    const WinoGeom &g = L.g;
    char *base = (char *)ws;
    float *U = (float *)(base + L.u), *V = v_keep ? v_keep : (float *)(base + L.v), *Mb = (float *)(base + L.m);
    const long long nin = g.Tp * (Cin / 4), nout = g.T * (Cout / 4);
    const unsigned fblocks = (unsigned)mrcnn::cdiv(Cout * Cin, 256);
    const int big = pg_big_ok(pass, g, Cin, Cout) ? 1 : 0;
    if (w_keep) WINO_LAUNCH(k_wino_filter, g, dim3(fblocks), w, U, transposed ? Cin : Cout, transposed ? Cout : Cin, transposed ? 1 : 0, big);
    if (w_keep) {
        const bool wb = gbias && (256 % (Cin / 4)) == 0;
        const int nblk = (int)std::min<long long>((nin + 255) / 256, 512);
        float *bias_part = wb ? (float *)(base + L.m) : nullptr;
        WINO_LAUNCH(k_wino_gy_dual, g, dim3(nblk), in, V, w_keep, bias_part, N, H, W, Cin, g.th, g.tw, g.T, g.Tp);
        if (wb) {
            if (int e = colsum_final(bias_part, gbias, nblk, Cin, gbias_accumulate, st)) return e;
        } else if (gbias) {
            if (int e = colsum(in, (float *)(base + L.m), gbias, N * H * W, Cin, gbias_accumulate, st)) return e;
        }
    } else
        WINO_LAUNCH(k_wino_input_filter, g, dim3(fblocks + (unsigned)((nin + 255) / 256)), in, V, N, H, W, Cin, g.th, g.tw, g.T, g.Tp, w, U,
                    transposed ? Cin : Cout, transposed ? Cout : Cin, transposed ? 1 : 0, fblocks, g_wino_banded, big, inbn);
    if (big) {
        PlaneGemmP q{};
        q.a = reinterpret_cast<const unsigned short *>(V); q.b = reinterpret_cast<const unsigned short *>(U); q.c = Mb;
        q.M = (int)(g.nk * g.Tp); q.N = Cout; q.K = Cin; q.batch_rows = (int)g.Tp; q.nbatch = g.nk; q.ksplit = 1; q.kchunk = Cin;
        q.bytes_a = (unsigned)((size_t)g.nk * g.Tp * Cin * 4); q.bytes_b = (unsigned)((size_t)g.nk * Cout * Cin * 6);
        q.ldc = Cout; q.dbg = 0; q.stamps = nullptr;
        if (!(g_debug_skip & 1)) launch_pgemm<4>(q, PGB_BM, PGB_BN, st);
        MRCNN_LAUNCH_CHECK();
        WINO_LAUNCH_OUT(g, dim3((unsigned)((nout + 255) / 256)), Mb, out, N, H, W, Cout, g.th, g.tw, g.T, g.Tp, bias, relu,
                    accumulate, relu_x, bn_part);
        return 0;
    }
    ConvP p;
    const int nsteps = wino_gemm_p(p, g, Cin, Cout);
    p.a = V; p.b = U; p.c = Mb;
    p.bytes_a = (unsigned)((size_t)g.nk * g.Tp * Cin * 4); p.bytes_b = (unsigned)((size_t)g.nk * Cout * Cin * 4);
    if (int e = run_data_conv<MODE_FWD>(p, nsteps, Cout, pass, base + L.inner, ws_bytes - L.inner, st)) return e;
    WINO_LAUNCH_OUT(g, dim3((unsigned)((nout + 255) / 256)), Mb, out, N, H, W, Cout, g.th, g.tw, g.T, g.Tp, bias, relu,
                accumulate, relu_x, bn_part);
    return 0;
}

bool fwd_takes_wino(const ConvGeom &cg, bool have_ws, size_t ws_bytes) {
    return wino_ok(cg, PASS_FWD) && have_ws && ws_bytes >= wino_ws_bytes(cg, PASS_FWD);
}
bool bwd_data_takes_wino(const ConvGeom &cg, bool have_ws, size_t ws_bytes) {
    const ConvGeom pipe = cg.transposed();
    return wino_ok(pipe, PASS_BWD_DATA) && have_ws && ws_bytes >= wino_ws_bytes(pipe, PASS_BWD_DATA);
}
int check_bwd_data(const ConvGeom &cg) {
    if (cg.stride != 1)
        return mrcnn::fail_arg(MRCNN_E_UNSUPPORTED, "conv2d_bwd_data: stride %d (only 1; strided 1x1 convs are "
                                                    "handled by the host as a subsample + stride-1 conv)", cg.stride);
    if (cg.Cin == 4) return mrcnn::fail_arg(MRCNN_E_UNSUPPORTED, "conv2d_bwd_data: Cin == 4 (image layer) has no data gradient");
    return 0;
}

}

extern "C" size_t mrcnn_conv2d_workspace_bytes(int N, int H, int W, int Cin, int Cout, int KH, int KW, int stride, int pad) {
    const ConvGeom cg{N, H, W, Cin, Cout, KH, KW, stride, pad};
    if (!cg.valid()) return 0;
    const long long Ho = cg.Ho(), Wo = cg.Wo();
    if (Ho <= 0 || Wo <= 0) return 0;
    const long long a = (long long)N * Ho * Wo * Cout, b = (long long)N * H * W * Cin;
    const long long fill = (long long)g_plan_fill * g_cus();
    const long long cap = fill * 8192;
    long long need = 0;
    if (a < cap) need = std::max(need, a);
    if (b < cap) need = std::max(need, b);
    const size_t tail = (size_t)4 * g_cus() * 128 * 128 * sizeof(float);
    size_t bytes = std::max((size_t)need * 16 * sizeof(float), tail);
    if (Cin % BK == 0 && deep_forward(KH * KW * (Cin / BK))) bytes = std::max(bytes, (size_t)a * DEEP_SPLIT * sizeof(float));
    if (wino_ok(cg, PASS_FWD)) bytes = std::max(bytes, wino_ws_bytes(cg, PASS_FWD));
    if (wino_ok(cg.transposed(), PASS_BWD_DATA)) bytes = std::max(bytes, wino_ws_bytes(cg.transposed(), PASS_BWD_DATA));
    return bytes;
}

extern "C" int mrcnn_debug_conv_parts(int mask) {
    g_dbg_parts = mask & 0xff;
    g_pg_big = (mask & 0x100) ? 0 : 1;
    return 0;
}

extern "C" int mrcnn_debug_split_planes_f32(const float *x, void *planes, int R, int C, int r4, void *stream) {
    if (!x || !planes || R <= 0 || C <= 0 || C % 16 || (long long)R * C * 6 >= (1ll << 32) || (r4 == 1 && R % 4))
        return mrcnn::fail_arg(MRCNN_E_INVALID, "debug_split_planes: null pointer, C %% 16 != 0, R %% 4 != 0 (P16R4) or more than 4 GiB of planes");
    hipLaunchKernelGGL(k_split_planes, dim3(mrcnn::cdiv((long long)R * (C / 4), 256)), dim3(256), 0, (hipStream_t)stream, x,
                       (unsigned short *)planes, (unsigned)R, (unsigned)C, r4);
    MRCNN_LAUNCH_CHECK();
    return 0;
}
static unsigned long long *g_pg_stamps = nullptr;
extern "C" int mrcnn_debug_planes_gemm_stamps(unsigned long long *stamps) {
    g_pg_stamps = stamps;
    return 0;
}
extern "C" int mrcnn_debug_planes_gemm(int kind, const void *a, const void *b, float *c, int M, int N, int K, int batch_rows, int nbatch,
                                       int ksplit, int bm, int bn, void *stream) {
    if (!a || !b || !c || M <= 0 || N <= 0 || K <= 0 || nbatch <= 0 || ksplit <= 0 || kind < 0 || kind > 5)
        return mrcnn::fail_arg(MRCNN_E_INVALID, "debug_planes_gemm: bad arguments");
    PlaneGemmP p{};
    p.a = (const unsigned short *)a; p.b = (const unsigned short *)b; p.c = c;
    p.M = M; p.N = N; p.K = K; p.batch_rows = batch_rows; p.nbatch = nbatch; p.ksplit = ksplit;
    long long ba, bb;
    if (kind == 5) {
        if (K != batch_rows || K % 32 || M % 16 || N % 16 || bm != 256 || bn != 256)
            return mrcnn::fail_arg(MRCNN_E_INVALID, "debug_planes_gemm G big: K == batch_rows, K %% 32, tile 256 x 256");
        ba = (long long)nbatch * K * M * 6; bb = (long long)nbatch * K * N * 4;
        p.kchunk = (K / 32 + ksplit - 1) / ksplit * 32;
        if ((K + p.kchunk - 1) / p.kchunk != ksplit) return mrcnn::fail_arg(MRCNN_E_INVALID, "debug_planes_gemm G big: ksplit %d leaves an empty split", ksplit);
        p.ldc = nbatch * N;
    } else if (kind == 3 || kind == 4) {
        if (K % 16 || batch_rows % 256 || M != nbatch * batch_rows || N % 16 || bm != 256 || bn != 256)
            return mrcnn::fail_arg(MRCNN_E_INVALID, "debug_planes_gemm big: K %% 16, batch_rows %% 256, tile 256 x 256");
        ba = (long long)M * K * 4; bb = (long long)nbatch * N * K * 6;
        p.ldc = N; p.ksplit = 1; p.kchunk = K;
    } else if (kind == 0 || kind == 2) {
        if (K % 32 || batch_rows % 128 || M != nbatch * batch_rows || N % 16 || bm != 128 || (bn != 128 && bn != 64))
            return mrcnn::fail_arg(MRCNN_E_INVALID, "debug_planes_gemm F: K %% 32, batch_rows %% 128, M == nbatch * batch_rows, tile 128 x 128|64");
        ba = (long long)M * K * (kind == 2 ? 4 : 6); bb = (long long)nbatch * N * K * 6;
        p.ldc = N; p.ksplit = 1; p.kchunk = K;
// ... 188 lines not shown
    ConvP p;
    TileChoice t;
    bool wino;
    return (size_t)bnstats_plan(p, t, wino, ConvGeom{N, H, W, Cin, Cout, KH, KW, stride, pad});
}
static int conv_fwd_bnstats(const float *x, const float *w, float *y, const ConvGeom &cg, float *bn_part, float *wino_v, void *ws,
                            size_t ws_bytes, hipStream_t st, const InBN &inbn = InBN{}) {
    if (int e = check_conv(x, w, y, cg)) return e;
    ConvP p;
    TileChoice t;
    bool wino;
    if (!bn_part || bnstats_plan(p, t, wino, cg) == 0)
        return mrcnn::fail_arg(MRCNN_E_UNSUPPORTED, "conv2d_fwd_bnstats: no fused statistics for this geometry (mrcnn_conv2d_bnstats_rows == 0)");
    if (wino) {
        if (!ws || ws_bytes < wino_ws_bytes(cg, PASS_FWD))
            return mrcnn::fail_arg(MRCNN_E_WORKSPACE, "conv2d_fwd_bnstats: workspace %zu < %zu", ws_bytes, wino_ws_bytes(cg, PASS_FWD));
        return wino_conv(x, w, y, cg, PASS_FWD, inbn, nullptr, 0, 0, nullptr, ws, ws_bytes, st, wino_v, nullptr, nullptr, 0, bn_part);
    }
    p.a = x; p.b = w; p.c = y; p.bias = nullptr; p.relu = 0; p.bn_part = bn_part;
    p.bytes_a = (unsigned)((size_t)cg.N * cg.H * cg.W * cg.Cin * 4); p.bytes_b = (unsigned)((size_t)cg.Cout * cg.KH * cg.KW * cg.Cin * 4);
    launch_conv<MODE_FWD>(p, 1, t, PASS_FWD, st);
    MRCNN_LAUNCH_CHECK();
    return 0;
}
extern "C" int mrcnn_conv2d_fwd_bnstats_f32(const float *x, const float *w, float *y, int N, int H, int W, int Cin, int Cout, int KH,
                                            int KW, int stride, int pad, float *bn_part, float *wino_v, void *ws, size_t ws_bytes,
                                            void *stream) {
    return conv_fwd_bnstats(x, w, y, ConvGeom{N, H, W, Cin, Cout, KH, KW, stride, pad}, bn_part, wino_v, ws, ws_bytes, (hipStream_t)stream);
}

static bool inbn_ok(const ConvGeom &cg) {
    if (!cg.valid() || cg.KH != 3 || cg.KW != 3 || cg.stride != 1 || cg.pad != 1 || (cg.Cin % 4)) return false;
    return wino_ok(cg, PASS_FWD) && wino_ok(cg, PASS_BWD_FILTER);
}
extern "C" int mrcnn_conv2d_inbn_ok(int N, int H, int W, int Cin, int Cout, int KH, int KW, int stride, int pad) {
    return inbn_ok(ConvGeom{N, H, W, Cin, Cout, KH, KW, stride, pad}) ? 1 : 0;
}
static int inbn_args(const InBN &inbn, const ConvGeom &cg, const char *who) {
    if (!inbn.gamma || !inbn.beta || !inbn.mean || !inbn.invstd) return mrcnn::fail_arg(MRCNN_E_INVALID, "%s: null BatchNorm pointer", who);
    if (!inbn_ok(cg))
        return mrcnn::fail_arg(MRCNN_E_UNSUPPORTED, "%s: this geometry does not take the Winograd path in both passes (mrcnn_conv2d_inbn_ok == 0)", who);
    return 0;
}
extern "C" int mrcnn_conv2d_fwd_inbn_f32(const float *x, const float *in_gamma, const float *in_beta, const float *in_mean, const float *in_invstd,
                                         const float *w, float *y, int N, int H, int W, int Cin, int Cout, int KH, int KW, int stride, int pad,
                                         float *bn_part, float *wino_v, void *ws, size_t ws_bytes, void *stream) {
    const ConvGeom cg{N, H, W, Cin, Cout, KH, KW, stride, pad};
    const InBN inbn{in_gamma, in_beta, in_mean, in_invstd};
    if (int e = inbn_args(inbn, cg, "conv2d_fwd_inbn")) return e;
    if (!ws || ws_bytes < wino_ws_bytes(cg, PASS_FWD))
        return mrcnn::fail_arg(MRCNN_E_WORKSPACE, "conv2d_fwd_inbn: workspace %zu < %zu", ws_bytes, wino_ws_bytes(cg, PASS_FWD));
    return bn_part ? conv_fwd_bnstats(x, w, y, cg, bn_part, wino_v, ws, ws_bytes, (hipStream_t)stream, inbn)
                   : conv_fwd(x, w, nullptr, y, cg, 0, wino_v, ws, ws_bytes, (hipStream_t)stream, inbn);
}

extern "C" int mrcnn_conv2d_fwd_rect_f32(const float *x, const float *w, const float *bias, float *y, int N, int H, int W,
                                         int Cin, int Cout, int KH, int KW, int stride, int pad_h, int pad_w, int relu, void *ws,
                                         size_t ws_bytes, void *stream) {
    if (pad_h < 0 || pad_w < 0) return mrcnn::fail_arg(MRCNN_E_INVALID, "conv2d_fwd_rect: negative padding");
    ConvGeom cg{N, H, W, Cin, Cout, KH, KW, stride, std::max(pad_h, pad_w)};
    if (int e = check_conv(x, w, y, cg)) return e;
    if (conv_out(H, KH, stride, pad_h) <= 0 || conv_out(W, KW, stride, pad_w) <= 0 || Cin == 4)
        return mrcnn::fail_arg(MRCNN_E_INVALID, "conv2d_fwd_rect: empty output (or the 4-channel image layer)");
    cg.pad = pad_h;
    ConvP p = make_p(cg);
    p.pad_w = pad_w;
    p.Wo = conv_out(W, KW, stride, pad_w);
    p.a = x; p.b = w; p.c = y; p.bias = bias; p.relu = relu;
    p.bytes_a = (unsigned)((size_t)N * H * W * Cin * 4); p.bytes_b = (unsigned)((size_t)Cout * KH * KW * Cin * 4);
    p.M = N * p.Ho * p.Wo; p.Ng = Cout;
    return run_data_conv<MODE_FWD>(p, KH * KW * (Cin / BK), Cout, PASS_FWD, ws, ws_bytes, (hipStream_t)stream);
}

static size_t winograd_w_bytes(const ConvGeom &cg) {
    if (!cg.valid() || !wino_ok(cg.transposed(), PASS_BWD_DATA) || !wino_ok(cg, PASS_BWD_FILTER)) return 0;
    const WinoGeom g = wino_geom(cg, PASS_BWD_DATA);
    if (g.m != wino_geom(cg, PASS_BWD_FILTER).m) return 0;
    return (size_t)g.nk * g.Tp * cg.Cout * sizeof(float);
}
extern "C" size_t mrcnn_conv2d_winograd_w_bytes(int N, int H, int W, int Cin, int Cout, int KH, int KW, int stride, int pad) {
    return winograd_w_bytes(ConvGeom{N, H, W, Cin, Cout, KH, KW, stride, pad});
}

extern "C" int mrcnn_conv2d_bwd_data_f32(const float *gy, const float *w, float *gx, const float *relu_x, int N, int H, int W,
                                         int Cin, int Cout, int KH, int KW, int stride, int pad,
                                         int accumulate, float *wino_w, float *gbias, int gbias_accumulate, void *ws,
                                         size_t ws_bytes, void *stream) {
    const ConvGeom cg{N, H, W, Cin, Cout, KH, KW, stride, pad};
    if (int e = check_conv(gy, w, gx, cg)) return e;
    if (int e = check_bwd_data(cg)) return e;
    ConvP p = make_p(cg);
    if (bwd_data_takes_wino(cg, ws != nullptr, ws_bytes))
        return wino_conv(gy, w, gx, cg.transposed(), PASS_BWD_DATA, InBN{}, nullptr, 0, accumulate, relu_x, ws, ws_bytes, (hipStream_t)stream,
                         nullptr, wino_w, wino_w ? gbias : nullptr, gbias_accumulate);
    if (wino_w || gbias) return mrcnn::fail_arg(MRCNN_E_UNSUPPORTED, "conv2d_bwd_data: wino_w / gbias only on the Winograd path (mrcnn_conv2d_winograd_w_bytes() > 0)");
    p.a = gy; p.b = w; p.c = gx; p.accumulate = accumulate; p.relu_x = relu_x;
    p.bytes_a = (unsigned)((size_t)N * p.Ho * p.Wo * Cout * 4); p.bytes_b = (unsigned)((size_t)Cout * KH * KW * Cin * 4);
    const int nsteps = bwd_data_gemm(p);
    return run_data_conv<MODE_BWD_DATA>(p, nsteps, Cin, PASS_BWD_DATA, ws, ws_bytes, (hipStream_t)stream);
}

static size_t bwd_filter_ws_bytes(const ConvGeom &cg) {
    if (!cg.valid()) return 0;
    ConvP p = make_p(cg);
    if (p.Ho <= 0 || p.Wo <= 0) return 0;
    int ksplit, kchunk;
    filter_plan(p, ksplit, kchunk);
    const size_t wsz = (size_t)cg.Cout * cg.KH * cg.KW * cg.Cin * sizeof(float);
    const size_t P = (size_t)cg.N * p.Ho * p.Wo;
    const size_t bias_part = (size_t)col_plan((int)P, cg.Cout).nblk * cg.Cout * sizeof(float);
    if (wino_ok(cg, PASS_BWD_FILTER)) {
        const WinoFLayout L = wino_filter_layout(cg);
        const size_t rows = (size_t)((L.g.Tp * (cg.Cout / 4) + 255) / 256);
        return L.total + std::max(bias_part, rows * cg.Cout * sizeof(float)) + 256;
    }
    return wsz * ksplit + bias_part + 256;
}
extern "C" size_t mrcnn_conv2d_bwd_filter_workspace_bytes(int N, int H, int W, int Cin, int Cout, int KH, int KW,
                                                          int stride, int pad) {
    return bwd_filter_ws_bytes(ConvGeom{N, H, W, Cin, Cout, KH, KW, stride, pad});
}

static int conv_bwd_filter(const float *x, const float *gy, float *gw, float *gbias, const ConvGeom &cg, int accumulate, const float *wino_v,
                           const float *wino_w, void *ws, size_t ws_bytes, hipStream_t st, const InBN &inbn = InBN{}) {
    if (int e = check_conv(x, gy, gw, cg)) return e;
    if (g_debug_skip & 4) return 0;
    const size_t need = bwd_filter_ws_bytes(cg);
    if (!ws || ws_bytes < need) return mrcnn::fail_arg(MRCNN_E_WORKSPACE, "conv2d_bwd_filter: workspace %zu < %zu", ws_bytes, need);
    ConvP p = make_p(cg);
    const int P = cg.N * p.Ho * p.Wo, Cout = cg.Cout;
    if (wino_ok(cg, PASS_BWD_FILTER)) {
        const WinoFLayout L = wino_filter_layout(cg);
        if (wino_v && !(wino_ok(cg, PASS_FWD) && wino_geom(cg, PASS_FWD).m == L.g.m)) wino_v = nullptr;
        if (wino_w && winograd_w_bytes(cg) == 0) wino_w = nullptr;
        float *bias_part = (float *)((char *)ws + L.total);
        int bias_rows = 0;
        if (int e = wino_bwd_filter(x, gy, gw, cg, inbn, accumulate, ws, st, wino_v, wino_w, gbias ? bias_part : nullptr, &bias_rows)) return e;
        if (!gbias) return 0;
        return bias_rows ? colsum_final(bias_part, gbias, bias_rows, Cout, accumulate, st) : colsum(gy, bias_part, gbias, P, Cout, accumulate, st);
    }
    filter_plan(p, p.ksplit, p.kchunk);
    const size_t wcount = (size_t)Cout * cg.KH * cg.KW * cg.Cin;
    float *slabs = (float *)ws;
    float *bias_part = (float *)ws + wcount * p.ksplit;
    const bool use_slabs = p.ksplit > 1 || accumulate;
    p.a = gy; p.b = x; p.c = use_slabs ? slabs : gw;
    p.bytes_a = (unsigned)((size_t)P * Cout * 4); p.bytes_b = (unsigned)((size_t)cg.N * cg.H * cg.W * cg.Cin * 4);
    bwd_filter_gemm(p);
    launch_conv<MODE_BWD_FILTER>(p, (p.smallc ? 1 : cg.KH * cg.KW) * p.ksplit, filter_tile(p), PASS_BWD_FILTER, st);
    MRCNN_LAUNCH_CHECK();
    if (use_slabs) if (int e = sum_slabs(slabs, gw, wcount / 4, p.ksplit, accumulate, st)) return e;
    return gbias ? colsum(gy, bias_part, gbias, P, Cout, accumulate, st) : 0;
}
extern "C" int mrcnn_conv2d_bwd_filter_f32(const float *x, const float *gy, float *gw, float *gbias, int N,
                                           int H, int W, int Cin, int Cout, int KH, int KW, int stride, int pad,
                                           int accumulate, const float *wino_v, const float *wino_w, void *ws, size_t ws_bytes,
                                           void *stream) {
    return conv_bwd_filter(x, gy, gw, gbias, ConvGeom{N, H, W, Cin, Cout, KH, KW, stride, pad}, accumulate, wino_v, wino_w, ws, ws_bytes,
                           (hipStream_t)stream);
}

extern "C" int mrcnn_conv2d_bwd_filter_inbn_f32(const float *x, const float *in_gamma, const float *in_beta, const float *in_mean,
                                                const float *in_invstd, const float *gy, float *gw, int N, int H, int W, int Cin, int Cout, int KH,
                                                int KW, int stride, int pad, int accumulate, const float *wino_v, void *ws, size_t ws_bytes,
                                                void *stream) {
    const ConvGeom cg{N, H, W, Cin, Cout, KH, KW, stride, pad};
    const InBN inbn{in_gamma, in_beta, in_mean, in_invstd};
    if (int e = inbn_args(inbn, cg, "conv2d_bwd_filter_inbn")) return e;
    return conv_bwd_filter(x, gy, gw, nullptr, cg, accumulate, wino_v, nullptr, ws, ws_bytes, (hipStream_t)stream, inbn);
}
```

chainer-maskrcnn_amd/csrc/planes_gemm.h:

```cpp

constexpr int PG_THREADS = 256;
constexpr int PG_BK = 16;

struct PlaneGemmP {
    const unsigned short *a, *b;
    float *c;
    int M, N, K;
    int batch_rows, nbatch;
    int tiles_m, tiles_n, remap_n;
    int ksplit, kchunk;
    unsigned bytes_a, bytes_b;
    int ldc;
    unsigned long long *stamps;
    int dbg;
};

__device__ __forceinline__ void pg_dma16(__amdgpu_buffer_rsrc_t rs, unsigned char *lds, unsigned voff, unsigned soff) {
    __builtin_amdgcn_raw_ptr_buffer_load_lds(rs, (__attribute__((address_space(3))) void *)lds, 16, voff, soff, 0, 0);
}

__device__ __forceinline__ unsigned long long pg_now() {
    unsigned long long t;
    asm volatile("s_memtime %0\n\ts_waitcnt lgkmcnt(0)" : "=s"(t)::"memory");
    return t;
}
#define PG_BF(x) __builtin_bit_cast(bf16x8_t, x)
#define PG_MMA6(ACC, AH, AM, AL, BH, BM, BL)                                                              \
    do {                                                                                                  \
        ACC = __builtin_amdgcn_mfma_f32_32x32x16_bf16(PG_BF(AL), PG_BF(BH), ACC, 0, 0, 0);                \
        ACC = __builtin_amdgcn_mfma_f32_32x32x16_bf16(PG_BF(AH), PG_BF(BL), ACC, 0, 0, 0);                \
        ACC = __builtin_amdgcn_mfma_f32_32x32x16_bf16(PG_BF(AM), PG_BF(BM), ACC, 0, 0, 0);                \
        ACC = __builtin_amdgcn_mfma_f32_32x32x16_bf16(PG_BF(AM), PG_BF(BH), ACC, 0, 0, 0);                \
        ACC = __builtin_amdgcn_mfma_f32_32x32x16_bf16(PG_BF(AH), PG_BF(BM), ACC, 0, 0, 0);                \
        ACC = __builtin_amdgcn_mfma_f32_32x32x16_bf16(PG_BF(AH), PG_BF(BH), ACC, 0, 0, 0);                \
    } while (0)

template <int TM, int TN>
__device__ __forceinline__ void pg_store_tiles(f32x16 (&acc)[TM][TN], float *et, float *cbase, size_t ldc, int mrow0, int ncol0,
                                               int M, int N, int lane) {
    constexpr int EPI_LD = 36;
    const int r = lane & 31, h = lane >> 5;
    const int er = lane >> 3, ec = (lane & 7) * 4;
#pragma unroll
    for (int tm = 0; tm < TM; ++tm)
#pragma unroll
        for (int tn = 0; tn < TN; ++tn) {
#pragma unroll
            for (int e = 0; e < 16; ++e) et[((e & 3) + 8 * (e >> 2) + 4 * h) * EPI_LD + r] = acc[tm][tn][e];
            const int n = ncol0 + tn * 32 + ec;
#pragma unroll
            for (int j = 0; j < 4; ++j) {
                const int row = er + 8 * j;
                const int m = mrow0 + tm * 32 + row;
                const float4 v = *reinterpret_cast<const float4 *>(&et[row * EPI_LD + ec]);
                if (n < N && m < M) *reinterpret_cast<float4 *>(cbase + (size_t)m * ldc + n) = v;
            }
        }
}

template <int BM_, int BN_>
__global__ __launch_bounds__(PG_THREADS, 2) void k_pgemm_f(PlaneGemmP p) {
    constexpr int TM = BM_ / 64, TN = BN_ / 64;
    constexpr int ROWB = 96;
    constexpr int A_STAGE = BM_ * ROWB, B_STAGE = BN_ * ROWB, STAGE = A_STAGE + B_STAGE;
    constexpr int NPA = A_STAGE / 1024, NPB = B_STAGE / 1024;
    constexpr int SA = (NPA + 3) / 4, SB = (NPB + 3) / 4;
    constexpr int EPI_BYTES = 4 * 32 * 36 * 4;
    static_assert(STAGE >= EPI_BYTES, "the epilogue's transpose tiles reuse stage 0");
    __shared__ __attribute__((aligned(1024))) unsigned char smem0[STAGE];
    __shared__ __attribute__((aligned(1024))) unsigned char smem1[STAGE];

    const int tid = threadIdx.x, lane = tid & 63, wave = __builtin_amdgcn_readfirstlane(tid >> 6);
    const int wm = wave >> 1, wn = wave & 1;
    int vid = blockIdx.x;
    {
        const int q = p.remap_n >> 3, r = p.remap_n & 7, xcd = vid & 7;
        vid = (xcd < r ? xcd * (q + 1) : r * (q + 1) + (xcd - r) * q) + (vid >> 3);
    }
    unsigned long long st_t0 = 0, st_r0 = 0;
    if (p.stamps) { st_t0 = pg_now(); st_r0 = __builtin_amdgcn_s_memrealtime(); }
    const int bx = vid / p.tiles_n, by = vid - bx * p.tiles_n;
    const int m0 = bx * BM_, n0 = by * BN_;
    const unsigned rowbytes = (unsigned)p.K * 6u;
    const int batch = m0 / p.batch_rows;
    const int m0l = (p.dbg & 2) ? 0 : m0;

    const auto rsA = __builtin_amdgcn_make_buffer_rsrc((void *)p.a, 0, p.bytes_a, 0x00020000);
    const auto rsB = __builtin_amdgcn_make_buffer_rsrc((void *)p.b, 0, p.bytes_b, 0x00020000);
    unsigned voffA[SA], voffB[SB];
#pragma unroll
    for (int i = 0; i < SA; ++i) {
        const int f = 64 * (wave + 4 * i) + lane, row = f / 6, pc = f - row * 6, lc = pc ^ ((row >> 3) & 1);
        voffA[i] = (m0 + row < p.M && row < BM_) ? (unsigned)(m0l + row) * rowbytes + (unsigned)lc * 16u : 0xFFFFFFFFu;
    }
#pragma unroll
    for (int i = 0; i < SB; ++i) {
        const int f = 64 * (wave + 4 * i) + lane, row = f / 6, pc = f - row * 6, lc = pc ^ ((row >> 3) & 1);
        voffB[i] = (n0 + row < p.N && row < BN_) ? (unsigned)(batch * p.N + n0 + row) * rowbytes + (unsigned)lc * 16u : 0xFFFFFFFFu;
// ... 317 lines not shown
                for (int tn = 0; tn < 2; ++tn) PG_MMA6(acc[tm][tn], a[tm][0], a[tm][1], a[tm][2], b[tn][0], b[tn][1], b[tn][2]);
        }
        asm volatile("s_waitcnt lgkmcnt(0)" ::: "memory");
        __builtin_amdgcn_sched_barrier(0);
        if (!(p.dbg & 1)) {
#pragma unroll
            for (int tm = 0; tm < 2; ++tm)
#pragma unroll
                for (int tn = 2; tn < 4; ++tn) PG_MMA6(acc[tm][tn], a[tm][0], a[tm][1], a[tm][2], b[tn][0], b[tn][1], b[tn][2]);
        } else {
#pragma unroll
            for (int t = 0; t < 2; ++t)
#pragma unroll
                for (int pl = 0; pl < 3; ++pl) asm volatile("" :: "v"(a[t][pl].x), "v"(a[t][pl].y), "v"(a[t][pl].z), "v"(a[t][pl].w));
        }
    };

    const int nsteps = (int)kblocks;
    unsigned b0 = 0, b1 = PGB_STAGE, b2 = 2 * PGB_STAGE;
    if (!(p.dbg & 8)) { issue(b0, 0); if (nsteps > 1) issue(b1, 1); }
    for (int s = 0; s < nsteps; ++s) {
        __builtin_amdgcn_sched_barrier(0);
        if (s + 1 < nsteps) asm volatile("s_waitcnt vmcnt(5)" ::: "memory");
        else asm volatile("s_waitcnt vmcnt(0)" ::: "memory");
        __builtin_amdgcn_s_barrier();
        __builtin_amdgcn_sched_barrier(0);
        if (s + 2 < nsteps && !(p.dbg & 8)) issue(b2, (unsigned)(s + 2));
        __builtin_amdgcn_sched_barrier(0);
        compute(b0);
        const unsigned t = b0; b0 = b1; b1 = b2; b2 = t;
    }
    if (!(p.dbg & 4)) {
        const int col = n0 + wn * 128 + (lane & 31);
#pragma unroll
        for (int tm = 0; tm < 2; ++tm)
#pragma unroll
            for (int e = 0; e < 16; ++e) {
                const int m = m0 + wm * 64 + tm * 32 + (e & 3) + 8 * (e >> 2) + 4 * h;
                float *dst = p.c + (size_t)m * p.ldc + col;
#pragma unroll
                for (int tn = 0; tn < 4; ++tn)
                    if (m < p.M && col + tn * 32 < p.N) dst[tn * 32] = acc[tm][tn][e];
            }
    }
    if (p.stamps && tid == 0) {
        unsigned long long *o = p.stamps + (size_t)blockIdx.x * 5;
        o[0] = st_t0; o[1] = pg_now(); o[2] = st_r0; o[3] = __builtin_amdgcn_s_memrealtime();
        o[4] = (unsigned long long)__builtin_amdgcn_s_getreg((31 << 11) | 4) | ((unsigned long long)__builtin_amdgcn_s_getreg((31 << 11) | 20) << 32);
    }
}

__device__ __forceinline__ void pg_split3x4(const float4 v, uint2 &hi, uint2 &mid, uint2 &lo) {
    const f32x2_t v01 = {v.x, v.y}, v23 = {v.z, v.w};
    const unsigned h01 = __builtin_bit_cast(unsigned, __builtin_convertvector(v01, bf16x2_t));
    const unsigned h23 = __builtin_bit_cast(unsigned, __builtin_convertvector(v23, bf16x2_t));
    float r0 = v.x - __uint_as_float(h01 << 16), r1 = v.y - __uint_as_float(h01 & 0xffff0000u);
    float r2 = v.z - __uint_as_float(h23 << 16), r3 = v.w - __uint_as_float(h23 & 0xffff0000u);
    asm volatile("" : "+v"(r0)); asm volatile("" : "+v"(r1)); asm volatile("" : "+v"(r2)); asm volatile("" : "+v"(r3));
    const f32x2_t r01 = {r0, r1}, r23 = {r2, r3};
    const unsigned m01 = __builtin_bit_cast(unsigned, __builtin_convertvector(r01, bf16x2_t));
    const unsigned m23 = __builtin_bit_cast(unsigned, __builtin_convertvector(r23, bf16x2_t));
    float q0 = r0 - __uint_as_float(m01 << 16), q1 = r1 - __uint_as_float(m01 & 0xffff0000u);
    float q2 = r2 - __uint_as_float(m23 << 16), q3 = r3 - __uint_as_float(m23 & 0xffff0000u);
    asm volatile("" : "+v"(q0)); asm volatile("" : "+v"(q1)); asm volatile("" : "+v"(q2)); asm volatile("" : "+v"(q3));
    const f32x2_t q01 = {q0, q1}, q23 = {q2, q3};
    hi = make_uint2(h01, h23);
    mid = make_uint2(m01, m23);
    lo = make_uint2(__builtin_bit_cast(unsigned, __builtin_convertvector(q01, bf16x2_t)),
                    __builtin_bit_cast(unsigned, __builtin_convertvector(q23, bf16x2_t)));
}

__global__ __launch_bounds__(PGB_THREADS, 2) void k_pgemm_pp(PlaneGemmP p) {
    __shared__ __attribute__((aligned(1024))) unsigned char smem[PGB_NSTAGE * PGB_STAGE];
    const int tid = threadIdx.x, lane = tid & 63, wave = __builtin_amdgcn_readfirstlane(tid >> 6);
    const int half = wave >> 2, wm = half * 2 + ((wave >> 1) & 1), wn = wave & 1;
    int vid0 = blockIdx.x;
    {
        const int G = (int)gridDim.x, q = G >> 3, r = G & 7, xcd = vid0 & 7;
        vid0 = (xcd < r ? xcd * (q + 1) : r * (q + 1) + (xcd - r) * q) + (vid0 >> 3);
    }
    unsigned long long st_t0 = 0, st_r0 = 0;
    if (p.stamps) { st_t0 = pg_now(); st_r0 = __builtin_amdgcn_s_memrealtime(); }
    const int ntiles = p.tiles_m * p.tiles_n;
    const int nj = vid0 < ntiles ? (ntiles - vid0 + (int)gridDim.x - 1) / (int)gridDim.x : 0;
    const unsigned rowbytesA = (unsigned)p.K * 4u;
    const unsigned kblocks = (unsigned)p.K / 16u;
    const int nsteps = (int)kblocks;
    const int S = nj * nsteps;

    const auto rsA = __builtin_amdgcn_make_buffer_rsrc((void *)p.a, 0, p.bytes_a, 0x00020000);
    const auto rsB = __builtin_amdgcn_make_buffer_rsrc((void *)p.b, 0, p.bytes_b, 0x00020000);
    unsigned voffA[2], voffB[3];
    int ij = 0, is = 0;
    auto setup = [&](int j) {
        const int tile = vid0 + j * (int)gridDim.x;
        const int bx = tile / p.tiles_n, by = tile - bx * p.tiles_n;
        const int m0 = bx * PGB_BM, n0 = by * PGB_BN, batch = m0 / p.batch_rows;
#pragma unroll
        for (int i = 0; i < 2; ++i) {
            const int f = 64 * (wave + 8 * i) + lane, row = f >> 2, pc = f & 3, lc = pc ^ ((row >> 2) & 3);
            voffA[i] = (m0 + row < p.M) ? (unsigned)(m0 + row) * rowbytesA + (unsigned)lc * 16u : 0xFFFFFFFFu;
        }
#pragma unroll
        for (int i = 0; i < 3; ++i) {
            const int piece = wave + 8 * i, pl = piece >> 3, rb = piece & 7;
            const int row = 32 * rb + (lane >> 1), hf = (lane & 1) ^ ((row >> 3) & 1);
            const int n = n0 + row;
            voffB[i] = (n < p.N) ? ((unsigned)((batch * p.N + n) >> 2) * kblocks) * 384u + (unsigned)pl * 128u + (unsigned)(n & 3) * 32u + (unsigned)hf * 16u
                                 : 0xFFFFFFFFu;
        }
    };
    const bool loads = !(p.dbg & 8), mfma = !(p.dbg & 1);
    auto issue_next = [&](unsigned buf) {
        if (is == 0) setup(ij);
        unsigned char *sa = smem + buf, *sb = sa + PGB_A_STAGE;
        const unsigned soffA = (unsigned)is * 64u, soffB = (unsigned)is * 384u;
        if (loads) {
#pragma unroll
            for (int i = 0; i < 2; ++i) pg_dma16(rsA, sa + (wave + 8 * i) * 1024, voffA[i], soffA);
#pragma unroll
            for (int i = 0; i < 3; ++i) pg_dma16(rsB, sb + (wave + 8 * i) * 1024, voffB[i], soffB);
        }
        if (++is == nsteps) { is = 0; ++ij; }
    };

    f32x16 acc[2][4];
#pragma unroll
    for (int i = 0; i < 2; ++i)
#pragma unroll
        for (int j = 0; j < 4; ++j)
#pragma unroll
            for (int e = 0; e < 16; ++e) acc[i][j][e] = 0.0f;

    const int r = lane & 31, h = lane >> 5;
    const unsigned sA = (unsigned)((r >> 2) & 3);
    const unsigned smem_base = (unsigned)(size_t)(__attribute__((address_space(3))) unsigned char *)smem;
    const unsigned fragA0 = smem_base + (unsigned)(wm * 64 + r) * 64u + (((unsigned)(2 * h) ^ sA) * 16u);
    const unsigned fragA1 = smem_base + (unsigned)(wm * 64 + r) * 64u + (((unsigned)(2 * h + 1) ^ sA) * 16u);
    const unsigned fragB = smem_base + (unsigned)PGB_A_STAGE + (unsigned)(wn * 128 + r) * 32u + (unsigned)((h ^ ((r >> 3) & 1)) * 16);

    unsigned b0 = 0, b1 = PGB_STAGE, b2 = 2 * PGB_STAGE;
    if (S > 0) issue_next(b0);
    if (S > 1) issue_next(b1);
    if (S > 1) asm volatile("s_waitcnt vmcnt(5)" ::: "memory");
    else asm volatile("s_waitcnt vmcnt(0)" ::: "memory");
    __builtin_amdgcn_s_barrier();
    __builtin_amdgcn_sched_barrier(0);
    if (half) { __builtin_amdgcn_s_barrier(); __builtin_amdgcn_sched_barrier(0); }
    int cs = 0, cj = 0;
    for (int g = 0; g < S; ++g) {
        if (g + 2 < S) issue_next(b2);
        const unsigned a0 = fragA0 + b0, a1 = fragA1 + b0, bb = fragB + b0;
        pg_u32x4 ra[2][2], b[4][3];
        PG_DSR128(ra[0][0], a0, 0); PG_DSR128(ra[0][1], a1, 0);
        PG_DSR128(ra[1][0], a0, 32 * 64); PG_DSR128(ra[1][1], a1, 32 * 64);
#pragma unroll
        for (int t = 0; t < 2; ++t)
#pragma unroll
            for (int pl = 0; pl < 3; ++pl) PG_DSR128(b[t][pl], bb, pl * PGB_B_PLANE + t * 32 * 32);
        asm volatile("s_waitcnt lgkmcnt(6)" ::: "memory");
        __builtin_amdgcn_sched_barrier(0);
        uint4 a[2][3];
#pragma unroll
        for (int t = 0; t < 2; ++t) {
            uint2 h0, m0_, l0, h1, m1, l1;
            pg_split3x4(__builtin_bit_cast(float4, ra[t][0]), h0, m0_, l0);
            pg_split3x4(__builtin_bit_cast(float4, ra[t][1]), h1, m1, l1);
            a[t][0] = make_uint4(h0.x, h0.y, h1.x, h1.y);
            a[t][1] = make_uint4(m0_.x, m0_.y, m1.x, m1.y);
            a[t][2] = make_uint4(l0.x, l0.y, l1.x, l1.y);
        }
#pragma unroll
        for (int t = 0; t < 2; ++t)
#pragma unroll
            for (int pl = 0; pl < 3; ++pl) asm volatile("" : "+v"(a[t][pl].x), "+v"(a[t][pl].y), "+v"(a[t][pl].z), "+v"(a[t][pl].w));
        __builtin_amdgcn_sched_barrier(0);
        if (g + 2 < S) asm volatile("s_waitcnt vmcnt(5) lgkmcnt(0)" ::: "memory");
        else asm volatile("s_waitcnt vmcnt(0) lgkmcnt(0)" ::: "memory");
        __builtin_amdgcn_s_barrier();
        __builtin_amdgcn_sched_barrier(0);
#pragma unroll
        for (int t = 2; t < 4; ++t)
#pragma unroll
            for (int pl = 0; pl < 3; ++pl) PG_DSR128(b[t][pl], bb, pl * PGB_B_PLANE + t * 32 * 32);
        __builtin_amdgcn_s_setprio(1);
        if (mfma) {
#pragma unroll
            for (int tm = 0; tm < 2; ++tm)
#pragma unroll
                for (int tn = 0; tn < 2; ++tn) PG_MMA6(acc[tm][tn], a[tm][0], a[tm][1], a[tm][2], b[tn][0], b[tn][1], b[tn][2]);
            asm volatile("s_waitcnt lgkmcnt(0)" ::: "memory");
            __builtin_amdgcn_sched_barrier(0);
#pragma unroll
            for (int tm = 0; tm < 2; ++tm)
#pragma unroll
                for (int tn = 2; tn < 4; ++tn) PG_MMA6(acc[tm][tn], a[tm][0], a[tm][1], a[tm][2], b[tn][0], b[tn][1], b[tn][2]);
        } else {
            asm volatile("s_waitcnt lgkmcnt(0)" ::: "memory");
#pragma unroll
            for (int t = 0; t < 2; ++t)
#pragma unroll
                for (int pl = 0; pl < 3; ++pl) asm volatile("" :: "v"(a[t][pl].x), "v"(a[t][pl].y), "v"(a[t][pl].z), "v"(a[t][pl].w));
#pragma unroll
            for (int t = 0; t < 4; ++t)
#pragma unroll
                for (int pl = 0; pl < 3; ++pl) asm volatile("" :: "v"(b[t][pl]));
        }
        __builtin_amdgcn_s_setprio(0);
        if (++cs == nsteps) {
            const int tile = vid0 + cj * (int)gridDim.x;
            const int bx = tile / p.tiles_n, by = tile - bx * p.tiles_n;
            const int m0 = bx * PGB_BM, n0 = by * PGB_BN;
            const int col = n0 + wn * 128 + (lane & 31);
#pragma unroll
            for (int tm = 0; tm < 2; ++tm)
#pragma unroll
                for (int e = 0; e < 16; ++e) {
                    const int m = m0 + wm * 64 + tm * 32 + (e & 3) + 8 * (e >> 2) + 4 * h;
                    float *dst = p.c + (size_t)m * p.ldc + col;
#pragma unroll
                    for (int tn = 0; tn < 4; ++tn) {
                        if (!(p.dbg & 4) && m < p.M && col + tn * 32 < p.N) dst[tn * 32] = acc[tm][tn][e];
                        acc[tm][tn][e] = 0.0f;
                    }
                }
            cs = 0; ++cj;
        }
        __builtin_amdgcn_sched_barrier(0);
        __builtin_amdgcn_s_barrier();
        __builtin_amdgcn_sched_barrier(0);
        const unsigned t_ = b0; b0 = b1; b1 = b2; b2 = t_;
    }
    if (!half) { __builtin_amdgcn_s_barrier(); __builtin_amdgcn_sched_barrier(0); }
    if (p.stamps && tid == 0) {
        unsigned long long *o = p.stamps + (size_t)blockIdx.x * 5;
        o[0] = st_t0; o[1] = pg_now(); o[2] = st_r0; o[3] = __builtin_amdgcn_s_memrealtime();
        o[4] = (unsigned long long)__builtin_amdgcn_s_getreg((31 << 11) | 4) | ((unsigned long long)__builtin_amdgcn_s_getreg((31 << 11) | 20) << 32);
    }
}

__global__ __launch_bounds__(PGB_THREADS, 2) void k_pgemm_gpp(PlaneGemmP p) {
    constexpr int W_ROW = 3 * 512, W_STAGE = 16 * W_ROW, V_ROW = 1024, V_STAGE = 16 * V_ROW;
    static_assert(W_STAGE + V_STAGE == PGB_STAGE, "stage size");
    __shared__ __attribute__((aligned(1024))) unsigned char smem[PGB_NSTAGE * PGB_STAGE];
    const int tid = threadIdx.x, lane = tid & 63, wave = __builtin_amdgcn_readfirstlane(tid >> 6);
    const int half = wave >> 2, wn = wave & 3;
    int vid = blockIdx.x;
    {
        const int q = p.remap_n >> 3, r = p.remap_n & 7, xcd = vid & 7;
        vid = (xcd < r ? xcd * (q + 1) : r * (q + 1) + (xcd - r) * q) + (vid >> 3);
    }
    const int by = vid % p.tiles_n; vid /= p.tiles_n;
    const int bx = vid % p.tiles_m; vid /= p.tiles_m;
    const int batch = vid % p.nbatch, split = vid / p.nbatch;
    const int m0 = bx * PGB_BM, n0 = by * PGB_BN;
    const int kbeg = split * p.kchunk, kend = min(p.K, kbeg + p.kchunk);
    const int nsteps = kend > kbeg ? (kend - kbeg) / PG_BK : 0;
    const unsigned rowW = (unsigned)p.M * 6u, rowV = (unsigned)p.N * 4u;

    const auto rsA = __builtin_amdgcn_make_buffer_rsrc((void *)p.a, 0, p.bytes_a, 0x00020000);
    const auto rsB = __builtin_amdgcn_make_buffer_rsrc((void *)p.b, 0, p.bytes_b, 0x00020000);
    unsigned voffW[3], voffV[2];
#pragma unroll
    for (int i = 0; i < 3; ++i) {
        const int irow = 2 * (wave + 8 * i) + (lane >> 5), t = irow / 3, pl = irow - 3 * t;
        const int pc = lane & 31, lc = pc ^ ((t & 3) << 2);
        const int co = m0 + lc * 8;
        voffW[i] = (co < p.M) ? (unsigned)t * rowW + (unsigned)pl * (unsigned)p.M * 2u + (unsigned)co * 2u : 0xFFFFFFFFu;
    }
#pragma unroll
    for (int i = 0; i < 2; ++i) {
        const int t = wave + 8 * i, ci = n0 + lane * 4;
        voffV[i] = (ci < p.N) ? (unsigned)t * rowV + (unsigned)ci * 4u : 0xFFFFFFFFu;
    }
    const unsigned row0 = (unsigned)(batch * p.batch_rows + kbeg);
    auto issue = [&](unsigned buf, unsigned kstep) {
        unsigned char *sw = smem + buf, *sv = sw + W_STAGE;
        const unsigned soffW = (row0 + kstep * 16u) * rowW, soffV = (row0 + kstep * 16u) * rowV;
#pragma unroll
        for (int i = 0; i < 3; ++i) pg_dma16(rsA, sw + (wave + 8 * i) * 1024, voffW[i], soffW);
#pragma unroll
        for (int i = 0; i < 2; ++i) pg_dma16(rsB, sv + (wave + 8 * i) * 1024, voffV[i], soffV);
    };

    f32x16 acc[4][2];
#pragma unroll
    for (int i = 0; i < 4; ++i)
#pragma unroll
        for (int j = 0; j < 2; ++j)
#pragma unroll
            for (int e = 0; e < 16; ++e) acc[i][j][e] = 0.0f;

    const int h = lane >> 5, g16 = (lane >> 4) & 1, q = (lane >> 2) & 3, pp = lane & 3;
    const unsigned smem_base = (unsigned)(size_t)(__attribute__((address_space(3))) unsigned char *)smem;
    unsigned offW[4];
#pragma unroll
    for (int tm = 0; tm < 4; ++tm) {
        const unsigned lc = (unsigned)(half * 16 + tm * 4 + 2 * g16 + (pp >> 1));
        offW[tm] = smem_base + (unsigned)(8 * h + q) * W_ROW + ((lc ^ ((unsigned)q << 2)) * 16u) + (unsigned)(pp & 1) * 8u;
    }
    const unsigned offV = smem_base + (unsigned)W_STAGE + (unsigned)(8 * h) * V_ROW + (unsigned)(wn * 64 + (lane & 31)) * 4u;

    const bool loads = !(p.dbg & 8), mfma = !(p.dbg & 1);
    unsigned b0 = 0, b1 = PGB_STAGE, b2 = 2 * PGB_STAGE;
    if (nsteps > 0) {
        if (loads) { issue(b0, 0); if (nsteps > 1) issue(b1, 1); }
        if (nsteps > 1) asm volatile("s_waitcnt vmcnt(5)" ::: "memory");
        else asm volatile("s_waitcnt vmcnt(0)" ::: "memory");
    }
    __builtin_amdgcn_s_barrier();
    __builtin_amdgcn_sched_barrier(0);
    if (half) { __builtin_amdgcn_s_barrier(); __builtin_amdgcn_sched_barrier(0); }
    typedef unsigned pg_u32x2 __attribute__((ext_vector_type(2)));
#define PG_DSTR(DST, ADDR, OFF) asm volatile("ds_read_b64_tr_b16 %0, %1 offset:%2" : "=v"(DST) : "v"(ADDR), "n"(OFF) : "memory")
#define PG_DSR2ST64(DST, ADDR, O0, O1) asm volatile("ds_read2st64_b32 %0, %1 offset0:%2 offset1:%3" : "=v"(DST) : "v"(ADDR), "n"(O0), "n"(O1) : "memory")
    for (int s = 0; s < nsteps; ++s) {
        if (s + 2 < nsteps && loads) issue(b2, (unsigned)(s + 2));
        pg_u32x2 rv[2][4];
        const unsigned av = offV + b0;
#pragma unroll
        for (int tn = 0; tn < 2; ++tn) {
            PG_DSR2ST64(rv[tn][0], av + tn * 128, 0, 4); PG_DSR2ST64(rv[tn][1], av + tn * 128, 8, 12);
            PG_DSR2ST64(rv[tn][2], av + tn * 128, 16, 20); PG_DSR2ST64(rv[tn][3], av + tn * 128, 24, 28);
        }
        pg_u32x2 rw[4][3][2];
#pragma unroll
        for (int tm = 0; tm < 2; ++tm) {
            const unsigned aw = offW[tm] + b0;
#pragma unroll
            for (int pl = 0; pl < 3; ++pl) { PG_DSTR(rw[tm][pl][0], aw, pl * 512); PG_DSTR(rw[tm][pl][1], aw, pl * 512 + 4 * W_ROW); }
        }
        asm volatile("s_waitcnt lgkmcnt(12)" ::: "memory");
#pragma unroll
        for (int tm = 2; tm < 4; ++tm) {
            const unsigned aw = offW[tm] + b0;
#pragma unroll
            for (int pl = 0; pl < 3; ++pl) { PG_DSTR(rw[tm][pl][0], aw, pl * 512); PG_DSTR(rw[tm][pl][1], aw, pl * 512 + 4 * W_ROW); }
        }
        __builtin_amdgcn_sched_barrier(0);
        uint4 bfr[2][3];
#pragma unroll
        for (int tn = 0; tn < 2; ++tn) {
            uint2 h0, m0_, l0, h1, m1, l1;
            split3_bf16x4(make_float4(__uint_as_float(rv[tn][0].x), __uint_as_float(rv[tn][0].y), __uint_as_float(rv[tn][1].x), __uint_as_float(rv[tn][1].y)), h0, m0_, l0);
            split3_bf16x4(make_float4(__uint_as_float(rv[tn][2].x), __uint_as_float(rv[tn][2].y), __uint_as_float(rv[tn][3].x), __uint_as_float(rv[tn][3].y)), h1, m1, l1);
            bfr[tn][0] = make_uint4(h0.x, h0.y, h1.x, h1.y);
            bfr[tn][1] = make_uint4(m0_.x, m0_.y, m1.x, m1.y);
            bfr[tn][2] = make_uint4(l0.x, l0.y, l1.x, l1.y);
        }
#pragma unroll
        for (int tn = 0; tn < 2; ++tn)
#pragma unroll
            for (int pl = 0; pl < 3; ++pl) asm volatile("" : "+v"(bfr[tn][pl].x), "+v"(bfr[tn][pl].y), "+v"(bfr[tn][pl].z), "+v"(bfr[tn][pl].w));
        __builtin_amdgcn_sched_barrier(0);
        if (s + 2 < nsteps) asm volatile("s_waitcnt vmcnt(5) lgkmcnt(0)" ::: "memory");
        else asm volatile("s_waitcnt vmcnt(0) lgkmcnt(0)" ::: "memory");
        __builtin_amdgcn_s_barrier();
        __builtin_amdgcn_sched_barrier(0);
        if (mfma) {
#pragma unroll
            for (int tm = 0; tm < 4; ++tm) {
                uint4 a[3];
#pragma unroll
                for (int pl = 0; pl < 3; ++pl) a[pl] = make_uint4(rw[tm][pl][0].x, rw[tm][pl][0].y, rw[tm][pl][1].x, rw[tm][pl][1].y);
#pragma unroll
                for (int tn = 0; tn < 2; ++tn) PG_MMA6(acc[tm][tn], a[0], a[1], a[2], bfr[tn][0], bfr[tn][1], bfr[tn][2]);
            }
        } else {
#pragma unroll
            for (int tm = 0; tm < 4; ++tm)
#pragma unroll
                for (int pl = 0; pl < 3; ++pl) asm volatile("" :: "v"(rw[tm][pl][0]), "v"(rw[tm][pl][1]));
#pragma unroll
            for (int tn = 0; tn < 2; ++tn)
#pragma unroll
                for (int pl = 0; pl < 3; ++pl) asm volatile("" :: "v"(bfr[tn][pl].x), "v"(bfr[tn][pl].y), "v"(bfr[tn][pl].z), "v"(bfr[tn][pl].w));
        }
        __builtin_amdgcn_sched_barrier(0);
        __builtin_amdgcn_s_barrier();
        __builtin_amdgcn_sched_barrier(0);
        const unsigned t_ = b0; b0 = b1; b1 = b2; b2 = t_;
    }
    if (!half) { __builtin_amdgcn_s_barrier(); __builtin_amdgcn_sched_barrier(0); }
    if (!(p.dbg & 4)) {
        float *cbase = p.c + (size_t)split * p.M * p.ldc + (size_t)batch * p.N;
        const int col = n0 + wn * 64 + (lane & 31);
#pragma unroll
        for (int tm = 0; tm < 4; ++tm)
#pragma unroll
            for (int e = 0; e < 16; ++e) {
                const int m = m0 + half * 128 + tm * 32 + (e & 3) + 8 * (e >> 2) + 4 * h;
                float *dst = cbase + (size_t)m * p.ldc + col;
#pragma unroll
                for (int tn = 0; tn < 2; ++tn)
                    if (m < p.M && col + tn * 32 < p.N) dst[tn * 32] = acc[tm][tn][e];
            }
    }
}

__device__ __forceinline__ unsigned pg_off_r4(unsigned row, unsigned c, unsigned C) {
// ... 195 lines not shown
```

chainer-maskrcnn_amd/csrc/targets.hip:

```cpp
#include "common.h"
#include "box_common.h"

#pragma clang fp contract(off)

namespace {

typedef unsigned long long u64;

__device__ void bitonic_sort(u64 *s, int n) {
    for (int k = 2; k <= n; k <<= 1)
        for (int j = k >> 1; j > 0; j >>= 1) {
            for (int i = threadIdx.x; i < n; i += blockDim.x) {
                const int ixj = i ^ j;
                if (ixj > i) {
                    const u64 a = s[i], b = s[ixj];
                    const bool up = (i & k) == 0;
                    if ((a > b) == up) { s[i] = b; s[ixj] = a; }
                }
            }
            __syncthreads();
        }
}

constexpr int PT_THREADS = 1024;
// ... 343 lines not shown
    const float4 stdv = make_float4(loc_std4[0], loc_std4[1], loc_std4[2], loc_std4[3]);
    hipLaunchKernelGGL(k_proposal_target, dim3(N), dim3(PT_THREADS), 0, (hipStream_t)stream, rois, roi_levels, n_rois,
                       roi_cap, gt_boxes, gt_labels, n_gt, gt_cap, keys, n_sample, n_pos_max, pos_iou_thresh,
                       neg_iou_thresh_hi, neg_iou_thresh_lo, mean, stdv, sample_roi, rois_xy5, sample_levels, gt_roi_loc,
                       gt_roi_label, gt_assign, sample_src, n_pos, n_sampled, pos_order, neg_order, n_cand);
    MRCNN_LAUNCH_CHECK();
    return 0;
}

extern "C" int mrcnn_mask_target_u8(const unsigned char *masks, int N, int gt_cap, int H, int W, const float *sample_roi,
                                    const int32_t *gt_assign, const int32_t *n_pos, int n_sample, int pos_cap,
                                    int mask_size, int32_t *gt_roi_mask, void *stream) {
    if (!masks || !sample_roi || !gt_assign || !n_pos || !gt_roi_mask || N <= 0 || gt_cap <= 0 || H <= 0 || W <= 0 ||
        n_sample <= 0 || pos_cap <= 0 || pos_cap > n_sample || mask_size <= 0)
        return mrcnn::fail_arg(MRCNN_E_INVALID, "mask_target: bad arguments");
    hipLaunchKernelGGL(k_mask_target, dim3(N * pos_cap), dim3(256), 0, (hipStream_t)stream, masks, gt_cap, H, W, sample_roi,
                       gt_assign, n_pos, n_sample, pos_cap, mask_size, gt_roi_mask);
    MRCNN_LAUNCH_CHECK();
    return 0;
}

extern "C" int mrcnn_keypoint_target_f32(const float *keypoints, int N, int gt_cap, int K, const float *sample_roi,
                                         const int32_t *gt_assign, const int32_t *n_pos, int n_sample, int pos_cap,
                                         int mask_size, int inplace_quirk, int32_t *gt_roi_kp, void *stream) {
    if (!keypoints || !sample_roi || !gt_assign || !n_pos || !gt_roi_kp || N <= 0 || gt_cap <= 0 || K <= 0 ||
        n_sample <= 0 || pos_cap <= 0 || pos_cap > n_sample || mask_size <= 0)
        return mrcnn::fail_arg(MRCNN_E_INVALID, "keypoint_target: bad arguments");
    hipLaunchKernelGGL(k_keypoint_target, dim3(N * pos_cap), dim3(64), 0, (hipStream_t)stream, keypoints, gt_cap, K,
                       sample_roi, gt_assign, n_pos, n_sample, pos_cap, mask_size, inplace_quirk, gt_roi_kp);
    MRCNN_LAUNCH_CHECK();
    return 0;
}

extern "C" int mrcnn_count_valid_labels_i32(const int32_t *labels, int N, int G, int32_t *n_gt, void *stream) {
    if (!labels || !n_gt || N <= 0 || G <= 0) return mrcnn::fail_arg(MRCNN_E_INVALID, "count_valid_labels: bad arguments");
    hipLaunchKernelGGL(k_count_valid_labels, dim3(N), dim3(64), 0, (hipStream_t)stream, labels, G, n_gt);
    MRCNN_LAUNCH_CHECK();
    return 0;
}

extern "C" size_t mrcnn_anchor_target_workspace_bytes(int N, int A) {
    if (N <= 0 || A <= 0) return 0;
    return at_layout(N, A).total;
}

extern "C" int mrcnn_anchor_target_f32(const float *anchors, int A, const float *gt_boxes, const int32_t *n_gt, int gt_cap,
                                       int N, float img_h, float img_w, const float *per_image_hw, const uint32_t *keys,
                                       int n_sample, float pos_iou_thresh, float neg_iou_thresh, float pos_ratio, int do_sample,
                                       float *gt_rpn_loc, int32_t *gt_rpn_label, void *ws, size_t ws_bytes,
                                       void *stream) {
    if (!anchors || !gt_boxes || !n_gt || !gt_rpn_loc || !gt_rpn_label || !ws || (do_sample && !keys))
        return mrcnn::fail_arg(MRCNN_E_INVALID, "anchor_target: null pointer");
    if (N <= 0 || A <= 0 || gt_cap <= 0 || gt_cap > AT_GCAP || n_sample <= 0 || A >= (1 << 30))
        return mrcnn::fail_arg(MRCNN_E_INVALID, "anchor_target: bad sizes (gt_cap <= %d)", AT_GCAP);
    const ATLayout L = at_layout(N, A);
    if (ws_bytes < L.total) return mrcnn::fail_arg(MRCNN_E_WORKSPACE, "anchor_target: workspace %zu < %zu", ws_bytes, L.total);
    hipStream_t st = (hipStream_t)stream;
    char *w = (char *)ws;
    float *max_iou = (float *)(w + L.max_iou);
    int32_t *argmax = (int32_t *)(w + L.argmax);
    int *gtmax = (int *)(w + L.gtmax), *counts = (int *)(w + L.counts);
    u64 *skeys = (u64 *)(w + L.skeys), *kth = (u64 *)(w + L.kth);
    unsigned *kreq = (unsigned *)(w + L.kreq);
    MRCNN_HIP_TRY(hipMemsetAsync(w + L.gtmax, 0, (L.counts - L.gtmax) + al((size_t)N * 2 * 4), st));
    const dim3 grid(mrcnn::cdiv(A, 256), N);
    hipLaunchKernelGGL(k_at_iou, grid, dim3(256), 0, st, anchors, A, gt_boxes, n_gt, gt_cap, img_h, img_w, per_image_hw, max_iou, argmax, gtmax);
    MRCNN_LAUNCH_CHECK();
    hipLaunchKernelGGL(k_at_label, grid, dim3(256), 0, st, anchors, A, gt_boxes, n_gt, gt_cap, max_iou, argmax, gtmax,
                       do_sample ? keys : (const uint32_t *)max_iou, pos_iou_thresh, neg_iou_thresh, gt_rpn_label, skeys, counts);
    MRCNN_LAUNCH_CHECK();
    if (do_sample) {
        const int n_pos_max = (int)(pos_ratio * n_sample);
        hipLaunchKernelGGL(k_at_ranks, dim3(mrcnn::cdiv(N, 64)), dim3(64), 0, st, counts, N, n_sample, n_pos_max, kreq);
        MRCNN_LAUNCH_CHECK();
        for (int c = 0; c < 2; ++c)
            if (int e = mrcnn::select_kth(skeys, N, (size_t)A, 64, false, kreq + c, 2, kth + c, 2, w + L.tmp, st)) return e;
        hipLaunchKernelGGL(k_at_disable, grid, dim3(256), 0, st, skeys, A, counts, kth, n_sample, n_pos_max, gt_rpn_label);
        MRCNN_LAUNCH_CHECK();
    }
    hipLaunchKernelGGL(k_at_loc, grid, dim3(256), 0, st, anchors, A, gt_boxes, n_gt, gt_cap, argmax, gt_rpn_loc);
    MRCNN_LAUNCH_CHECK();
    return 0;
}
```

include/mrcnn_hip.h:

```cpp
#ifndef MRCNN_HIP_H
#define MRCNN_HIP_H

#include <stddef.h>
#include <stdint.h>

#ifdef __cplusplus
extern "C" {
#endif

#define MRCNN_ABI_VERSION 10

enum {
    MRCNN_OK = 0,
    MRCNN_E_INVALID = -1,
    MRCNN_E_UNSUPPORTED = -2,
    MRCNN_E_WORKSPACE = -3
};

enum { MRCNN_LAYOUT_NCHW = 0, MRCNN_LAYOUT_NHWC = 1 };

#define MRCNN_MAX_LEVELS 8

int mrcnn_abi_version(void);
const char *mrcnn_last_error(void);
// ... 13 lines not shown
int mrcnn_roi_align_bwd_ws_f32(const float *gy, int layout, int N, int C, int H, int W,
                               const float *rois, int R, int PH, int PW, float spatial_scale,
                               int sampling_ratio, float *gx, void *ws, size_t ws_bytes, void *stream);
size_t mrcnn_roi_align_bwd_workspace_bytes(int N, int C, int H, int W, int R, int PH, int PW, int sampling_ratio);

int mrcnn_roi_align_fpn_fwd_f32(const float *const *xs, const int *Hs, const int *Ws,
                                const float *scales, int L, int N, int C, const float *rois,
                                const int32_t *levels, int R, int PH, int PW,
                                int sampling_ratio, float *y, void *stream);
int mrcnn_roi_align_fpn_fwd_ws_f32(const float *const *xs, const int *Hs, const int *Ws,
                                   const float *scales, int L, int N, int C, const float *rois,
                                   const int32_t *levels, int R, int PH, int PW,
                                   int sampling_ratio, float *y, void *ws, size_t ws_bytes, void *stream);
int mrcnn_roi_align_fpn_bwd_f32(const float *gy, float *const *gxs, const int *Hs, const int *Ws,
                                const float *scales, int L, int N, int C, const float *rois,
                                const int32_t *levels, int R, int PH, int PW,
                                int sampling_ratio, int accumulate, void *ws, size_t ws_bytes, void *stream);
size_t mrcnn_roi_align_fpn_bwd_workspace_bytes(const int *Hs, const int *Ws, int L, int N, int C, int R, int PH, int PW,
                                               int sampling_ratio);
size_t mrcnn_roi_align_fpn_bwd_plan_bytes(const int *Hs, const int *Ws, int L, int N, int R, int PH, int PW, int split_levels);
int mrcnn_roi_align_fpn_bwd_plan_f32(const int *Hs, const int *Ws, const float *scales, int L, int N, int C, const float *rois,
                                     const int32_t *levels, int R, int PH, int PW, int sampling_ratio, int split_levels,
                                     void *plan, size_t plan_bytes, void *stream);
int mrcnn_debug_roi_align_lean_variant(int v);
int mrcnn_debug_roi_align_lean_stamps(unsigned long long *stamps);
int mrcnn_roi_align_fpn_bwd_planned_f32(const float *gy, float *const *gxs, const int *Hs, const int *Ws, const float *scales, int L,
                                        int N, int C, const float *rois, const int32_t *levels, int R, int PH, int PW,
                                        int sampling_ratio, int accumulate, void *ws, size_t ws_bytes, void *plan,
                                        size_t plan_bytes, int plan_verified, void *stream);
int mrcnn_roi_align_bwd_plan_status(const void *plan, size_t plan_bytes, int *status3, void *stream);

int mrcnn_roi_align_set_bwd_variant(int variant);

int mrcnn_debug_roi_align_bwd_stamps(const float *gy, int N, int C, int H, int W, const float *rois, int R, int PH, int PW,
                                     float spatial_scale, int sampling_ratio, float *gx, unsigned long long *stamps,
                                     void *stream);

int mrcnn_debug_dispatch_census(unsigned long long *out, int nblocks, int spin_us, void *stream);

int mrcnn_roi_align_sample_tables(const float *rois, int R, int H, int W, int PH, int PW,
                                  float spatial_scale, int sampling_ratio, int smax,
                                  int32_t *cnt, int32_t *idx, float *wgt, void *stream);

size_t mrcnn_conv2d_workspace_bytes(int N, int H, int W, int Cin, int Cout, int KH, int KW, int stride, int pad);
long long mrcnn_conv2d_executed_macs(int N, int H, int W, int Cin, int Cout, int KH, int KW, int stride, int pad, int pass);
int mrcnn_conv2d_set_winograd_thresholds(int min_channels, int min_pixels, int tile);
int mrcnn_conv2d_set_winograd_pass_tiles(int fwd, int bwd_data, int bwd_filter);
int mrcnn_conv2d_get_winograd_pass_tiles(int *tiles3);
int mrcnn_conv2d_set_split_operands(int fwd, int bwd_data, int bwd_filter);
int mrcnn_conv2d_get_split_operands(int *modes3);
#define MRCNN_CONV_PLAN_FIELDS 9
int mrcnn_conv2d_plan_query(int pass, int N, int H, int W, int Cin, int Cout, int KH, int KW, int stride, int pad, int *out, int n_out);
int mrcnn_debug_conv_plan(int fill, int filter_rounds, int force_tile);
int mrcnn_debug_wino_banded(int on);
int mrcnn_debug_conv_parts(int mask);
int mrcnn_debug_split_planes_f32(const float *x, void *planes, int R, int C, int r4, void *stream);
int mrcnn_debug_planes_gemm_stamps(unsigned long long *stamps);
int mrcnn_debug_planes_gemm(int kind, const void *a, const void *b, float *c, int M, int N, int K, int batch_rows, int nbatch,
                            int ksplit, int bm, int bn, void *stream);

int mrcnn_conv2d_set_debug_skip(int mask);
int mrcnn_debug_bn_skip(int mask);
int mrcnn_debug_bn_plan(int red_cap, int fin_quads);
size_t mrcnn_conv2d_winograd_v_bytes(int N, int H, int W, int Cin, int Cout, int KH, int KW, int stride, int pad);
int mrcnn_conv2d_fwd_f32(const float *x, const float *w, const float *bias, float *y, int N, int H,
                         int W, int Cin, int Cout, int KH, int KW, int stride, int pad, int relu,
                         float *wino_v, void *ws, size_t ws_bytes, void *stream);
size_t mrcnn_conv2d_bnstats_rows(int N, int H, int W, int Cin, int Cout, int KH, int KW, int stride, int pad);
int mrcnn_conv2d_fwd_bnstats_f32(const float *x, const float *w, float *y, int N, int H, int W, int Cin, int Cout, int KH, int KW,
                                 int stride, int pad, float *bn_part, float *wino_v, void *ws, size_t ws_bytes, void *stream);
int mrcnn_conv2d_fwd_rect_f32(const float *x, const float *w, const float *bias, float *y, int N, int H, int W, int Cin,
                              int Cout, int KH, int KW, int stride, int pad_h, int pad_w, int relu, void *ws,
                              size_t ws_bytes, void *stream);
size_t mrcnn_conv2d_winograd_w_bytes(int N, int H, int W, int Cin, int Cout, int KH, int KW, int stride, int pad);
int mrcnn_conv2d_bwd_data_f32(const float *gy, const float *w, float *gx, const float *relu_x, int N, int H, int W, int Cin,
                              int Cout, int KH, int KW, int stride, int pad, int accumulate, float *wino_w,
                              float *gbias, int gbias_accumulate, void *ws, size_t ws_bytes, void *stream);
size_t mrcnn_conv2d_bwd_filter_workspace_bytes(int N, int H, int W, int Cin, int Cout, int KH, int KW,
                                               int stride, int pad);
int mrcnn_conv2d_bwd_filter_f32(const float *x, const float *gy, float *gw, float *gbias, int N, int H,
                                int W, int Cin, int Cout, int KH, int KW, int stride, int pad, int accumulate,
                                const float *wino_v, const float *wino_w,
                                void *ws, size_t ws_bytes, void *stream);

size_t mrcnn_bn_workspace_bytes(int P, int C);
int mrcnn_bn_train_fwd_f32(const float *x, const float *gamma, const float *beta, const float *residual,
                           float *y, float *save_mean, float *save_invstd, float *running_mean,
                           float *running_var, int P, int C, float eps, float decay, int relu, void *ws,
                           size_t ws_bytes, void *stream);
int mrcnn_bn_train_fwd_stats_f32(const float *x, const float *part, int rows, const float *gamma, const float *beta,
                                 const float *residual, float *y, float *save_mean, float *save_invstd, float *running_mean,
                                 float *running_var, int P, int C, float eps, float decay, int relu, void *stream);
int mrcnn_bn_train_bwd_f32(const float *gy, const float *x, const float *y, const float *gamma, const float *beta,
                           const float *save_mean, const float *save_invstd, float *gx, float *gres,
                           float *ggamma, float *gbeta, int P, int C, int relu, void *ws, size_t ws_bytes,
                           void *stream);
int mrcnn_bn_train_stats_f32(const float *x, const float *part, int rows, float *save_mean, float *save_invstd, float *running_mean,
                             float *running_var, int P, int C, float eps, float decay, void *ws, size_t ws_bytes, void *stream);
int mrcnn_conv2d_inbn_ok(int N, int H, int W, int Cin, int Cout, int KH, int KW, int stride, int pad);
int mrcnn_conv2d_fwd_inbn_f32(const float *x, const float *in_gamma, const float *in_beta, const float *in_mean, const float *in_invstd,
                              const float *w, float *y, int N, int H, int W, int Cin, int Cout, int KH, int KW, int stride, int pad,
                              float *bn_part, float *wino_v, void *ws, size_t ws_bytes, void *stream);
int mrcnn_conv2d_bwd_filter_inbn_f32(const float *x, const float *in_gamma, const float *in_beta, const float *in_mean,
                                     const float *in_invstd, const float *gy, float *gw, int N, int H, int W, int Cin, int Cout, int KH,
                                     int KW, int stride, int pad, int accumulate, const float *wino_v, void *ws, size_t ws_bytes,
                                     void *stream);
size_t mrcnn_bn_pair_workspace_bytes(int P, int C);
int mrcnn_bn_train_fwd_pair_f32(const float *xa, const float *part_a, int rows_a, const float *gamma_a, const float *beta_a,
                                float *mean_a, float *invstd_a, float *run_mean_a, float *run_var_a, const float *xb,
                                const float *part_b, int rows_b, const float *gamma_b, const float *beta_b, float *mean_b,
                                float *invstd_b, float *run_mean_b, float *run_var_b, float *y, int P, int C, float eps, float decay,
                                void *ws, size_t ws_bytes, void *stream);
int mrcnn_bn_train_bwd_pair_f32(const float *gy, const float *y, const float *xa, const float *xb, const float *gamma_a,
                                const float *mean_a, const float *invstd_a, const float *gamma_b, const float *mean_b,
                                const float *invstd_b, float *gxa, float *gxb, float *ggamma_a, float *gbeta_a, float *ggamma_b,
                                float *gbeta_b, int P, int C, void *ws, size_t ws_bytes, void *stream);
int mrcnn_bn_infer_fwd_f32(const float *x, const float *gamma, const float *beta, const float *mean,
                           const float *var, const float *residual, float *y, int P, int C, float eps, int relu,
                           void *stream);
int mrcnn_relu_bwd_f32(const float *gy, const float *y, float *gx, size_t n, void *stream);
int mrcnn_add_f32(const float *a, const float *b, float *out, size_t n, void *stream);
int mrcnn_maxpool2x2_fwd_f32(const float *x, float *y, int N, int H, int W, int C, void *stream);
int mrcnn_maxpool2x2_bwd_f32(const float *x, const float *gy, float *gx, int N, int H, int W, int C, void *stream);
int mrcnn_maxpool3x3s2_fwd_f32(const float *x, float *y, int N, int H, int W, int C, void *stream);
int mrcnn_global_avg_pool_fwd_f32(const float *x, float *y, int R, int P, int C, void *stream);
int mrcnn_relu_fwd_f32(const float *x, float *y, size_t n, void *stream);
int mrcnn_upsample2x_add_fwd_f32(const float *top, const float *lat, float *out, int N, int H, int W, int Ht,
                                 int Wt, int C, void *stream);
int mrcnn_upsample2x_bwd_f32(const float *gout, float *gtop, int N, int H, int W, int Ht, int Wt, int C,
                             int accumulate, void *stream);
int mrcnn_subsample_bwd_f32(const float *gsub, float *gx, int N, int H, int W, int C, int stride, int accumulate,
                            const float *relu_x, void *stream);
int mrcnn_pixel_shuffle2x_f32(const float *src, const float *bias, float *dst, int N, int H, int W, int C, int inverse,
                              void *stream);
int mrcnn_deconv_merge_fwd_f32(const float *wd, const float *bd, const float *w2, const float *b2, float *wm,
                               float *bm, int C, int Cin, int K2, int ld2, void *stream);
int mrcnn_deconv_merge_bwd_f32(const float *G, const float *gb4, const float *wd, const float *bd,
                               const float *w2, float *gwd, float *gbd, float *gw2, float *gb2, int C,
                               int Cin, int K2, int ld2, void *stream);
int mrcnn_bilinear2x_fwd_f32(const float *x, float *y, int N, int H, int W, int C, void *stream);
int mrcnn_bilinear2x_bwd_f32(const float *gy, float *gx, int N, int H, int W, int C, void *stream);
int mrcnn_image_nchw3_to_nhwc4_f32(const float *x, float *y, int N, int H, int W, void *stream);
int mrcnn_image_resize_u8_f32(const uint8_t *src, int H, int W, float *dst, int oh, int ow, int dst_h, int dst_w,
                              float div, void *stream);
int mrcnn_mask_resize_nearest_u8(const uint8_t *src, int G, int H, int W, uint8_t *dst, int oh, int ow, int dst_h,
                                 int dst_w, void *stream);
int mrcnn_image_resize_f32(const float *src, int C, int H, int W, float *dst, int oh, int ow, int dst_h, int dst_w,
                           float div, void *stream);
int mrcnn_random_keys_u32(uint32_t *out, size_t n, unsigned long long seed, void *stream);
int mrcnn_random_keys_dev_u32(uint32_t *out, size_t n, unsigned long long *state, void *stream);
int mrcnn_sgd_momentum_wd_f32(float *p, const float *g, float *v, size_t n, float lr, float momentum,
                              float weight_decay, void *stream);

typedef struct mrcnn_bottleneck {
    int32_t N, H, W;
    int32_t cin, mid, cout;
    int32_t stride, project;
    int32_t fwd_split;
    float eps, decay;
    const float *w[4];
    const float *gamma[4];
    const float *beta[4];
    float *run_mean[4];
    float *run_var[4];
    float *gw[4];
    float *ggamma[4];
// ... 294 lines not shown
```

Baseline: 98.01.

## Skip inactive (non-positive) ROI rows in mask head conv backward passes

Measured after the change: 105.6 (median of 6 runs). 1.08x the previous value.

```diff
diff --git a/chainer-maskrcnn_amd/chainer_maskrcnn/_hip/nn.py b/chainer-maskrcnn_amd/chainer_maskrcnn/_hip/nn.py
--- a/chainer-maskrcnn_amd/chainer_maskrcnn/_hip/nn.py
+++ b/chainer-maskrcnn_amd/chainer_maskrcnn/_hip/nn.py
@@ -141,7 +141,14 @@
     return lib().mrcnn_conv2d_winograd_w_bytes(N, H, W, Cin, Cout, KH, KW, stride, pad)
 
 
-def conv2d_bwd_data_raw(gy, w, x_shape, stride, pad, out=None, relu_x=None, emit_w=False, gb=None, gb_accumulate=False):
+def active_rows(n_pos, rows_per_block):
+    assert n_pos.dtype == torch.int32 and n_pos.is_contiguous()
+    active = torch.empty((n_pos.numel() * int(rows_per_block),), dtype=torch.uint8, device=n_pos.device)
+    check(lib().mrcnn_active_rows_u8(ptr(n_pos), n_pos.numel(), int(rows_per_block), ptr(active), stream_ptr()))
+    return active
+
+
+def conv2d_bwd_data_raw(gy, w, x_shape, stride, pad, out=None, relu_x=None, emit_w=False, gb=None, gb_accumulate=False, active=None):
     N, H, W, Cin = x_shape
     Cout, KH, KW, _ = w.shape
     assert gy.is_contiguous()
@@ -154,6 +161,13 @@
         wb = lib().mrcnn_conv2d_winograd_w_bytes(N, H, W, Cin, Cout, KH, KW, stride, pad)
         assert wb > 0, 'emit_w: the layer does not take the Winograd path'
         wt = torch.empty((wb // 4,), dtype=torch.float32, device=gy.device)
+    if active is not None:
+        assert not emit_w and active.dtype == torch.uint8 and active.is_contiguous()
+        with _prof('bwd_data', N * gy.shape[1] * gy.shape[2], KH, KW, Cin, Cout, (N, H, W, Cin, Cout, KH, KW, stride, pad)):
+            check(lib().mrcnn_conv2d_bwd_data_active_f32(ptr(gy), ptr(w), ptr(gx), ptr(relu_x), N, H, W, Cin, Cout, KH, KW,
+                                                         stride, pad, int(acc), ptr(active), active.numel(),
+                                                         ptr(ws), ws.numel() if ws is not None else 0, stream_ptr()))
+        return gx
     with _prof('bwd_data', N * gy.shape[1] * gy.shape[2], KH, KW, Cin, Cout, (N, H, W, Cin, Cout, KH, KW, stride, pad)):
         check(lib().mrcnn_conv2d_bwd_data_f32(ptr(gy), ptr(w), ptr(gx), ptr(relu_x), N, H, W, Cin, Cout, KH, KW,
                                               stride, pad, int(acc), ptr(wt), ptr(gb) if emit_w else None, int(gb_accumulate),
@@ -162,7 +176,7 @@
 
 
 def conv2d_bwd_filter_raw(x, gy, w_shape, stride, pad, want_bias, gw=None, gb=None, accumulate=None, wino_v=None,
-                          wino_w=None):
+                          wino_w=None, active=None):
     N, H, W, Cin = x.shape
     Cout, KH, KW, _ = w_shape
     assert gy.is_contiguous() and x.is_contiguous()
@@ -172,6 +186,13 @@
         gb = torch.empty((Cout,), dtype=torch.float32, device=x.device) if want_bias else None
     nbytes = lib().mrcnn_conv2d_bwd_filter_workspace_bytes(N, H, W, Cin, Cout, KH, KW, stride, pad)
     ws = workspace(nbytes, x.device)
+    if active is not None:
+        assert wino_w is None and active.dtype == torch.uint8 and active.is_contiguous()
+        with _prof('bwd_filter', N * gy.shape[1] * gy.shape[2], KH, KW, Cin, Cout, (N, H, W, Cin, Cout, KH, KW, stride, pad)):
+            check(lib().mrcnn_conv2d_bwd_filter_active_f32(ptr(x), ptr(gy), ptr(gw), ptr(gb) if want_bias else None, N, H, W, Cin,
+                                                           Cout, KH, KW, stride, pad, int(acc), ptr(wino_v), ptr(active), active.numel(),
+                                                           ptr(ws), ws.numel(), stream_ptr()))
+        return gw, gb
     with _prof('bwd_filter', N * gy.shape[1] * gy.shape[2], KH, KW, Cin, Cout, (N, H, W, Cin, Cout, KH, KW, stride, pad)):
         check(lib().mrcnn_conv2d_bwd_filter_f32(ptr(x), ptr(gy), ptr(gw), ptr(gb) if want_bias else None, N, H, W, Cin,
                                                 Cout, KH, KW, stride, pad, int(acc), ptr(wino_v), ptr(wino_w), ptr(ws), ws.numel(),
diff --git a/chainer-maskrcnn_amd/chainer_maskrcnn/model/fpn_maskrcnn_train_chain.py b/chainer-maskrcnn_amd/chainer_maskrcnn/model/fpn_maskrcnn_train_chain.py
--- a/chainer-maskrcnn_amd/chainer_maskrcnn/model/fpn_maskrcnn_train_chain.py
+++ b/chainer-maskrcnn_amd/chainer_maskrcnn/model/fpn_maskrcnn_train_chain.py
@@ -184,6 +184,7 @@
                                                        getattr(faster_rcnn, 'point_head', None) is not None)
         self._row = dict(self._loss_rows)
         self.pending = None
+        self._mask_active = None
         self._arith_found = None
 
     @property
@@ -298,13 +299,15 @@
             self._box_stages_backward(st, g_feats, into_early)
         g_iou_in = m.maskiou_head.backward(st.g_iou) if st.g_iou is not None else None
         g_pt_in = m.point_head.backward(st.point['g_pred']) if st.point is not None else None
-        g_pool = m.head.backward_mask_convs(st.g_mask)
+        active = self._mask_active
+        self._mask_active = None
+        g_pool = m.head.backward_mask_convs(st.g_mask, active=active)
         if g_iou_in is not None:
             self._maskiou_input_backward(g_iou_in, g_pool)
         main.wait_stream(aux)
         if self.keep_outputs and g_iou_in is not None:
             self.outputs.update(g_feats_box=[g.clone() for g in g_feats])
-        m.head.backward_mask_pool(g_pool, g_feats)
+        m.head.backward_mask_pool(g_pool, g_feats, active=active)
         if g_pt_in is not None:
             self._point_input_backward(st.point, g_pt_in, g_feats)
         if self.keep_outputs and (st.g_later or g_iou_in is not None):
@@ -403,7 +406,10 @@
             stage.backward_box(g_k, g_feats, accumulate=True)
 
     def _mask_loss(self, features, t, scales, losses):
+        from chainer_maskrcnn.nn import core
+        from chainer_maskrcnn._hip import nn as hnn
         head = self.faster_rcnn.head
+        self._mask_active = None
         if self.mask_loss_kind == 'generic':
             g_mask = self._generic_mask_loss(t, features, scales, losses)
             return self._generic_inputs + (None, g_mask)
@@ -419,6 +425,10 @@
         out = losses[self._row['mask_loss']]
         if self.mask_loss_kind == 'mask_bce':
             _, g_mask = ops.mask_bce(mask_out, t['gt_roi_mask'], m_label, out=out)
+            m = self.faster_rcnn
+            if (rows == S and core.MASK_BWD_SKIP_INACTIVE and getattr(m, 'maskiou_head', None) is None
+                    and getattr(m, 'point_head', None) is None):
+                self._mask_active = hnn.active_rows(t['n_pos'].to(torch.int32).contiguous(), S)
         else:
             Rm, Hm, Wm, Cm = mask_out.shape
             K = head.n_keypoints
diff --git a/chainer-maskrcnn_amd/chainer_maskrcnn/model/head/fpn_roi_mask_head.py b/chainer-maskrcnn_amd/chainer_maskrcnn/model/head/fpn_roi_mask_head.py
--- a/chainer-maskrcnn_amd/chainer_maskrcnn/model/head/fpn_roi_mask_head.py
+++ b/chainer-maskrcnn_amd/chainer_maskrcnn/model/head/fpn_roi_mask_head.py
@@ -331,7 +331,7 @@
         m = ops.pixel_shuffle2x(d, bias=bm)
         return m, (h, wm), None
 
-    def _merged_deconv_bwd(self, td, g_mask):
+    def _merged_deconv_bwd(self, td, g_mask, active=None):
         from chainer_maskrcnn._hip import nn as hnn
         dc, c2, C = self.deconv1, self.conv2, self.channels
         x_in, wm = td
@@ -339,8 +339,8 @@
         g4 = ops.pixel_shuffle2x(g_mask, inverse=True)
         hnn.LOGICAL = (dc.cin, 4 * c2.cout)
         try:
-            G, gb4 = hnn.conv2d_bwd_filter_raw(x_in, g4, tuple(wm.shape), 1, 0, True)
-            g = hnn.conv2d_bwd_data_raw(g4, wm, tuple(x_in.shape), 1, 0, relu_x=x_in if self.mask_convs else None)
+            G, gb4 = hnn.conv2d_bwd_filter_raw(x_in, g4, tuple(wm.shape), 1, 0, True, active=active)
+            g = hnn.conv2d_bwd_data_raw(g4, wm, tuple(x_in.shape), 1, 0, relu_x=x_in if self.mask_convs else None, active=active)
         finally:
             hnn.LOGICAL = None
         ps = self.ps
@@ -371,19 +371,28 @@
         if g_mask is not None:
             self.backward_mask_pool(self.backward_mask_convs(g_mask), g_feats)
 
-    def backward_mask_convs(self, g_mask):
+    def _usable_active(self, active):
+        from chainer_maskrcnn.nn import core
+        if active is None or not core.MASK_BWD_SKIP_INACTIVE:
+            return None
+        if self.upsample2x or any(gn is not None for gn in self.mask_gns):
+            return None
+        return active
+
+    def backward_mask_convs(self, g_mask, active=None):
         from chainer_maskrcnn._hip import nn as hnn
+        active = self._usable_active(active)
         tapes, td, tc2, rois, levels, scales, _ = self.mask_tape
         if self.upsample2x:
             g_mask = ops.bilinear2x_bwd(g_mask)
         if self.merge_deconv:
-            g = self._merged_deconv_bwd(td, g_mask)
+            g = self._merged_deconv_bwd(td, g_mask, active)
             n = len(self.mask_convs)
             for i in range(n - 1, -1, -1):
                 t, nt = tapes[i]
                 if self.mask_gns[i] is not None:
                     g = self.mask_gns[i].bwd(nt, g, gy_masked=True)
-                g = self.mask_convs[i].bwd(t, g, gy_masked=True, mask_gx=(i > 0))
+                g = self.mask_convs[i].bwd(t, g, gy_masked=True, mask_gx=(i > 0), active=active)
             return g
         g = self.conv2.bwd(tc2, g_mask)
         g4 = ops.pixel_shuffle2x(g, inverse=True)
@@ -400,10 +409,10 @@
         for cv, gn, (t, nt) in zip(reversed(self.mask_convs), reversed(self.mask_gns), reversed(tapes)):
             if gn is not None:
                 g = gn.bwd(nt, g)
-            g = cv.bwd(t, g)
+            g = cv.bwd(t, g, active=active)
         return g
 
-    def backward_mask_pool(self, g_pool, g_feats):
+    def backward_mask_pool(self, g_pool, g_feats, active=None):
         tapes, td, tc2, rois, levels, scales, plan = self.mask_tape
         roi_align_fpn_bwd(g_pool, g_feats, rois, levels, self.roi_size_mask, scales, accumulate=True, plan=plan)
         self.mask_tape = None
diff --git a/chainer-maskrcnn_amd/chainer_maskrcnn/nn/core.py b/chainer-maskrcnn_amd/chainer_maskrcnn/nn/core.py
--- a/chainer-maskrcnn_amd/chainer_maskrcnn/nn/core.py
+++ b/chainer-maskrcnn_amd/chainer_maskrcnn/nn/core.py
@@ -11,6 +11,7 @@
 
 FILTER_GRAD_ON_SIDE_STREAM = True
 WINOGRAD_SHARED_GY_TRANSFORM = False
+MASK_BWD_SKIP_INACTIVE = True
 LAYER_TILE_HINTS = True
 FWD_TILE_RULE = None
 FUSE_BN_STATS = True
@@ -200,12 +201,14 @@
         hnn.LOGICAL = None
         return y, (x, y if relu else None, v)
 
-    def bwd(self, ctx, gy, need_gx=True, gx_acc=None, accumulate_params=False, gy_masked=False, mask_gx=False):
+    def bwd(self, ctx, gy, need_gx=True, gx_acc=None, accumulate_params=False, gy_masked=False, mask_gx=False, active=None):
         with _layer_tiles(self):
-            return self._bwd(ctx, gy, need_gx, gx_acc, accumulate_params, gy_masked, mask_gx)
-
-    def _bwd(self, ctx, gy, need_gx, gx_acc, accumulate_params, gy_masked, mask_gx):
+            return self._bwd(ctx, gy, need_gx, gx_acc, accumulate_params, gy_masked, mask_gx, active)
+
+    def _bwd(self, ctx, gy, need_gx, gx_acc, accumulate_params, gy_masked, mask_gx, active=None):
         x, y, v = ctx
+        if WINOGRAD_SHARED_GY_TRANSFORM:
+            active = None
         if y is not None and not gy_masked:
             gy = ops.relu_bwd(gy, y)
         gw = self.gW
@@ -233,20 +236,22 @@
                 side.wait_stream(main)
                 with torch.cuda.stream(side):
                     hnn.conv2d_bwd_filter_raw(x, gy, tuple(gw.shape), self.stride, self.pad, self.has_bias, gw=gw, gb=gb,
-                                              accumulate=accumulate_params, wino_v=v)
+                                              accumulate=accumulate_params, wino_v=v, active=active)
                 gy.record_stream(side)
                 x.record_stream(side)
                 if v is not None:
                     v.record_stream(side)
+                if active is not None:
+                    active.record_stream(side)
             else:
                 hnn.conv2d_bwd_filter_raw(x, gy, tuple(gw.shape), self.stride, self.pad, self.has_bias, gw=gw, gb=gb,
-                                          accumulate=accumulate_params, wino_v=v)
+                                          accumulate=accumulate_params, wino_v=v, active=active)
             if not need_gx:
                 return None
             if self.stride == 1:
                 assert not (mask_gx and gx_acc is not None) or self.k == 1
                 return hnn.conv2d_bwd_data_raw(gy, self.W, tuple(x.shape), 1, self.pad, out=gx_acc,
-                                               relu_x=x if mask_gx else None)
+                                               relu_x=x if mask_gx else None, active=active)
             if self.k > 1:
                 assert self.k == 2 * self.pad + 1 and gx_acc is None, 'strided k x k backward-data: odd kernel with "same" padding'
                 N, H, W, _ = x.shape
diff --git a/chainer-maskrcnn_amd/csrc/conv.hip b/chainer-maskrcnn_amd/csrc/conv.hip
--- a/chainer-maskrcnn_amd/csrc/conv.hip
+++ b/chainer-maskrcnn_amd/csrc/conv.hip
@@ -1307,7 +1307,7 @@
 template <int M_>
 __device__ __forceinline__ void wino_input_body(const float *__restrict__ x, float *__restrict__ V, int N, int H, int W, int C,
                                                 int th, int tw, long long T, long long Tp, unsigned blk, const InBN bn = InBN{},
-                                                int panel = 0) {
+                                                int panel = 0, const unsigned char *__restrict__ active = nullptr) {
     constexpr int A_ = M_ + 2;
     const unsigned C4 = (unsigned)C / 4u;
     const unsigned i = blk * 256u + threadIdx.x;
@@ -1340,6 +1340,7 @@
     const int tx = (int)(t - trow * (unsigned)tw);
     const int n = (int)(trow / (unsigned)th);
     const int ty = (int)(trow - (unsigned)n * (unsigned)th);
+    if (active && !active[n]) return;
     const auto rsX = __builtin_amdgcn_make_buffer_rsrc((void *)x, 0, (unsigned)((size_t)N * H * W * C * 4), 0x00020000);
     const unsigned OOB = 0xFFFFFFFFu;
     unsigned rowo[A_], colo[A_];
@@ -1397,16 +1398,16 @@
 __global__ __launch_bounds__(256) void k_wino_input_filter(const float *__restrict__ x, float *__restrict__ V, int N, int H, int W, int C,
                                                            int th, int tw, long long T, long long Tp, const float *__restrict__ w,
                                                            float *__restrict__ U, int Cout_w, int Cin_w, int transposed, unsigned fblocks,
-                                                           int banded, int uplanes, InBN bn) {
+                                                           int banded, int uplanes, InBN bn, const unsigned char *__restrict__ active) {
     if (blockIdx.x < fblocks) wino_filter_body<M_>(w, U, Cout_w, Cin_w, transposed, blockIdx.x, uplanes);
-    else wino_input_body<M_>(x, V, N, H, W, C, th, tw, T, Tp, xcd_banded(blockIdx.x, fblocks, gridDim.x - fblocks, banded), bn, banded);
+    else wino_input_body<M_>(x, V, N, H, W, C, th, tw, T, Tp, xcd_banded(blockIdx.x, fblocks, gridDim.x - fblocks, banded), bn, banded, active);
 }
 
 template <int M_>
 __global__ __launch_bounds__(256) void k_wino_output(const float *__restrict__ Mb, float *__restrict__ y, int N, int H, int W, int C,
                                                      int th, int tw, long long T, long long Tp, const float *__restrict__ bias,
                                                      int relu, int accumulate, const float *__restrict__ relu_x,
-                                                     float *__restrict__ bn_part) {
+                                                     float *__restrict__ bn_part, const unsigned char *__restrict__ active) {
     constexpr int A_ = M_ + 2;
     __shared__ float4 sred[2][256];
     const unsigned C4 = (unsigned)C / 4u;
@@ -1425,49 +1426,61 @@
         const auto rsY = __builtin_amdgcn_make_buffer_rsrc((void *)y, 0, ybytes, 0x00020000);
         const auto rsR = __builtin_amdgcn_make_buffer_rsrc((void *)relu_x, 0, relu_x ? ybytes : 0u, 0x00020000);
         const unsigned mo = (unsigned)(((size_t)t * C + c) * 4);
-        V4 s[M_][A_];
-#pragma unroll
-        for (int q = 0; q < A_; ++q) {
-            V4 m[A_], r[M_];
-#pragma unroll
-            for (int rr = 0; rr < A_; ++rr) m[rr] = v4buf_nt(rsM, mo, (unsigned)(rr * A_ + q) * ks);
-            wino_at<M_, V4>(m, r);
-#pragma unroll
-            for (int a = 0; a < M_; ++a) s[a][q] = r[a];
-        }
-        const V4 bv = bias ? v4ld(bias + c) : v4zero();
-        const unsigned OOB = 0xFFFFFFFFu;
-#pragma unroll
-        for (int a = 0; a < M_; ++a) {
-            V4 row[M_], old[M_], xm[M_];
-            wino_at<M_, V4>(s[a], row);
-            const int h = M_ * ty + a;
-            unsigned off[M_];
-#pragma unroll
-            for (int b = 0; b < M_; ++b) {
-                const int ww = M_ * tx + b;
-                off[b] = (h < H && ww < W) ? (unsigned)((((size_t)n * H + h) * W + ww) * C + c) * 4u : OOB;
-            }
-            if (accumulate) {
-#pragma unroll
-                for (int b = 0; b < M_; ++b) old[b] = v4buf(rsY, off[b], 0);
-            }
-            if (relu_x) {
-#pragma unroll
-                for (int b = 0; b < M_; ++b) xm[b] = v4buf(rsR, off[b], 0);
-            }
-#pragma unroll
-            for (int b = 0; b < M_; ++b) {
-                V4 v = row[b] + bv;
-                if (relu) { v.x = fmaxf(v.x, 0.f); v.y = fmaxf(v.y, 0.f); v.z = fmaxf(v.z, 0.f); v.w = fmaxf(v.w, 0.f); }
-                if (accumulate) v = v + old[b];
+        if (active && !active[n]) {
+            if (!accumulate) {
+#pragma unroll
+                for (int a = 0; a < M_; ++a)
+#pragma unroll
+                    for (int b = 0; b < M_; ++b) {
+                        const int h = M_ * ty + a, ww = M_ * tx + b;
+                        v4bufst(rsY, (h < H && ww < W) ? (unsigned)((((size_t)n * H + h) * W + ww) * C + c) * 4u : 0xFFFFFFFFu, 0, v4zero());
+                    }
+            }
+        } else {
+            V4 s[M_][A_];
+#pragma unroll
+            for (int q = 0; q < A_; ++q) {
+                V4 m[A_], r[M_];
+#pragma unroll
+                for (int rr = 0; rr < A_; ++rr) m[rr] = v4buf_nt(rsM, mo, (unsigned)(rr * A_ + q) * ks);
+                wino_at<M_, V4>(m, r);
+#pragma unroll
+                for (int a = 0; a < M_; ++a) s[a][q] = r[a];
+            }
+            const V4 bv = bias ? v4ld(bias + c) : v4zero();
+            const unsigned OOB = 0xFFFFFFFFu;
+#pragma unroll
+            for (int a = 0; a < M_; ++a) {
+                V4 row[M_], old[M_], xm[M_];
+                wino_at<M_, V4>(s[a], row);
+                const int h = M_ * ty + a;
+                unsigned off[M_];
+#pragma unroll
+                for (int b = 0; b < M_; ++b) {
+                    const int ww = M_ * tx + b;
+                    off[b] = (h < H && ww < W) ? (unsigned)((((size_t)n * H + h) * W + ww) * C + c) * 4u : OOB;
+                }
+                if (accumulate) {
+#pragma unroll
+                    for (int b = 0; b < M_; ++b) old[b] = v4buf(rsY, off[b], 0);
+                }
                 if (relu_x) {
-                    v.x = xm[b].x > 0.f ? v.x : 0.f; v.y = xm[b].y > 0.f ? v.y : 0.f; v.z = xm[b].z > 0.f ? v.z : 0.f; v.w = xm[b].w > 0.f ? v.w : 0.f;
+#pragma unroll
+                    for (int b = 0; b < M_; ++b) xm[b] = v4buf(rsR, off[b], 0);
                 }
-                v4bufst(rsY, off[b], 0, v);
-                if (off[b] != OOB) {
-                    bs = bs + v;
-                    bq.x = fmaf(v.x, v.x, bq.x); bq.y = fmaf(v.y, v.y, bq.y); bq.z = fmaf(v.z, v.z, bq.z); bq.w = fmaf(v.w, v.w, bq.w);
+#pragma unroll
+                for (int b = 0; b < M_; ++b) {
+                    V4 v = row[b] + bv;
+                    if (relu) { v.x = fmaxf(v.x, 0.f); v.y = fmaxf(v.y, 0.f); v.z = fmaxf(v.z, 0.f); v.w = fmaxf(v.w, 0.f); }
+                    if (accumulate) v = v + old[b];
+                    if (relu_x) {
+                        v.x = xm[b].x > 0.f ? v.x : 0.f; v.y = xm[b].y > 0.f ? v.y : 0.f; v.z = xm[b].z > 0.f ? v.z : 0.f; v.w = xm[b].w > 0.f ? v.w : 0.f;
+                    }
+                    v4bufst(rsY, off[b], 0, v);
+                    if (off[b] != OOB) {
+                        bs = bs + v;
+                        bq.x = fmaf(v.x, v.x, bq.x); bq.y = fmaf(v.y, v.y, bq.y); bq.z = fmaf(v.z, v.z, bq.z); bq.w = fmaf(v.w, v.w, bq.w);
+                    }
                 }
             }
         }
@@ -1491,12 +1504,13 @@
 
 template <int M_>
 __global__ __launch_bounds__(256) void k_wino_gy(const float *__restrict__ gy, float *__restrict__ Wt, int N, int H, int W, int C,
-                                                 int th, int tw, long long T, long long Tp, float *__restrict__ bias_part, int wplanes) {
+                                                 int th, int tw, long long T, long long Tp, float *__restrict__ bias_part, int wplanes,
+                                                 const unsigned char *__restrict__ active) {
     constexpr int A_ = M_ + 2;
     __shared__ float4 sred[256];
     const unsigned C4 = (unsigned)C / 4u;
     const unsigned i = blockIdx.x * 256u + threadIdx.x;
-    const bool in_range = i < (unsigned)Tp * C4;
+    bool in_range = i < (unsigned)Tp * C4;
     const unsigned t = in_range ? i / C4 : (unsigned)Tp;
     const int c = in_range ? (int)(i - t * C4) * 4 : 0;
     V4 bsum = v4zero();
@@ -1512,6 +1526,7 @@
         __builtin_amdgcn_raw_buffer_store_b64(u32x2{mid.x, mid.y}, rsW, off + (unsigned)C * 2u, 0, 0);
         __builtin_amdgcn_raw_buffer_store_b64(u32x2{lo.x, lo.y}, rsW, off + (unsigned)C * 4u, 0, 0);
     };
+    if (in_range && active && !pg_rows_active(active, th * tw, (int)T, (int)(t & ~(unsigned)(PG_BK - 1)), PG_BK)) in_range = false;
     if (in_range && t >= (unsigned)T) {
 #pragma unroll
         for (int k = 0; k < A_ * A_; ++k) put(vo + (unsigned)k * ks, v4zero());
@@ -1739,7 +1754,8 @@
 }
 
 int wino_bwd_filter(const float *x, const float *gy, float *gw, const ConvGeom &cg, const InBN &inbn, int accumulate, void *ws,
-                    hipStream_t st, const float *v_cached, const float *w_cached, float *bias_part = nullptr, int *bias_rows = nullptr) {
+                    hipStream_t st, const float *v_cached, const float *w_cached, float *bias_part = nullptr, int *bias_rows = nullptr,
+                    const unsigned char *active = nullptr) {
     const int N = cg.N, H = cg.H, W = cg.W, Cin = cg.Cin, Cout = cg.Cout;
     const WinoFLayout L = wino_filter_layout(cg);
     const WinoGeom &g = L.g;
@@ -1752,8 +1768,9 @@
     const bool fuse_bias = bias_part && bias_rows && !w_cached && C4o <= 256 && 256 % C4o == 0 && !(g_debug_skip & 2);
     if (bias_rows) *bias_rows = fuse_bias ? (int)((nout + 255) / 256) : 0;
     const int big = (L.big && !w_cached) ? 1 : 0;
+    const unsigned char *act = (big && L.kchunk / PG_BK <= PGG_MASK_STEPS) ? active : nullptr;
     if (!w_cached) WINO_LAUNCH(k_wino_gy, g, dim3((unsigned)((nout + 255) / 256)), gy, Wt, N, H, W, Cout, g.th, g.tw, g.T, g.Tp,
-                               fuse_bias ? bias_part : (float *)nullptr, big);
+                               fuse_bias ? bias_part : (float *)nullptr, big, act);
     const int ksplit = big ? L.ksplit : L.ks32;
     const size_t n4 = (size_t)Cout * g.nk * Cin / 4;
     if (big) {
@@ -1763,6 +1780,7 @@
         q.M = Cout; q.N = Cin; q.K = (int)g.Tp; q.batch_rows = (int)g.Tp; q.nbatch = g.nk; q.ksplit = ksplit; q.kchunk = L.kchunk;
         q.bytes_a = (unsigned)((size_t)g.nk * g.Tp * Cout * 6); q.bytes_b = (unsigned)((size_t)g.nk * g.Tp * Cin * 4);
         q.ldc = g.nk * Cin; q.dbg = 0; q.stamps = nullptr;
+        q.active = act; q.act_per = g.th * g.tw; q.act_T = (int)g.T;
         if (!(g_debug_skip & 1)) launch_pgemm<5>(q, PGB_BM, PGB_BN, st);
         MRCNN_LAUNCH_CHECK();
         if (ksplit > 1) if (int e = sum_slabs(slabs, dU, n4, ksplit, 0, st)) return e;
@@ -1798,7 +1816,8 @@
 
 int wino_conv(const float *in, const float *w, float *out, const ConvGeom &cg, int pass, const InBN &inbn,
               const float *bias, int relu, int accumulate, const float *relu_x, void *ws, size_t ws_bytes, hipStream_t st,
-              float *v_keep, float *w_keep = nullptr, float *gbias = nullptr, int gbias_accumulate = 0, float *bn_part = nullptr) {
+              float *v_keep, float *w_keep = nullptr, float *gbias = nullptr, int gbias_accumulate = 0, float *bn_part = nullptr,
+              const unsigned char *active = nullptr) {
     const int N = cg.N, H = cg.H, W = cg.W, Cin = cg.Cin, Cout = cg.Cout;
     const bool transposed = pass == PASS_BWD_DATA;
     const WinoLayout L = wino_layout(cg, pass);
@@ -1808,6 +1827,7 @@
     const long long nin = g.Tp * (Cin / 4), nout = g.T * (Cout / 4);
     const unsigned fblocks = (unsigned)mrcnn::cdiv(Cout * Cin, 256);
     const int big = pg_big_ok(pass, g, Cin, Cout) ? 1 : 0;
+    const unsigned char *act = (big && pass == PASS_BWD_DATA && !w_keep && !v_keep && !bias && !relu && !bn_part && !(accumulate && relu_x)) ? active : nullptr;
     if (w_keep) WINO_LAUNCH(k_wino_filter, g, dim3(fblocks), w, U, transposed ? Cin : Cout, transposed ? Cout : Cin, transposed ? 1 : 0, big);
     if (w_keep) {
         const bool wb = gbias && (256 % (Cin / 4)) == 0;
@@ -1821,17 +1841,18 @@
         }
     } else
         WINO_LAUNCH(k_wino_input_filter, g, dim3(fblocks + (unsigned)((nin + 255) / 256)), in, V, N, H, W, Cin, g.th, g.tw, g.T, g.Tp, w, U,
-                    transposed ? Cin : Cout, transposed ? Cout : Cin, transposed ? 1 : 0, fblocks, g_wino_banded, big, inbn);
+                    transposed ? Cin : Cout, transposed ? Cout : Cin, transposed ? 1 : 0, fblocks, g_wino_banded, big, inbn, act);
     if (big) {
         PlaneGemmP q{};
         q.a = reinterpret_cast<const unsigned short *>(V); q.b = reinterpret_cast<const unsigned short *>(U); q.c = Mb;
         q.M = (int)(g.nk * g.Tp); q.N = Cout; q.K = Cin; q.batch_rows = (int)g.Tp; q.nbatch = g.nk; q.ksplit = 1; q.kchunk = Cin;
         q.bytes_a = (unsigned)((size_t)g.nk * g.Tp * Cin * 4); q.bytes_b = (unsigned)((size_t)g.nk * Cout * Cin * 6);
         q.ldc = Cout; q.dbg = 0; q.stamps = nullptr;
+        q.active = act; q.act_per = g.th * g.tw; q.act_T = (int)g.T;
         if (!(g_debug_skip & 1)) launch_pgemm<4>(q, PGB_BM, PGB_BN, st);
         MRCNN_LAUNCH_CHECK();
         WINO_LAUNCH_OUT(g, dim3((unsigned)((nout + 255) / 256)), Mb, out, N, H, W, Cout, g.th, g.tw, g.T, g.Tp, bias, relu,
-                    accumulate, relu_x, bn_part);
+                    accumulate, relu_x, bn_part, act);
         return 0;
     }
     ConvP p;
@@ -1840,7 +1861,7 @@
     p.bytes_a = (unsigned)((size_t)g.nk * g.Tp * Cin * 4); p.bytes_b = (unsigned)((size_t)g.nk * Cout * Cin * 4);
     if (int e = run_data_conv<MODE_FWD>(p, nsteps, Cout, pass, base + L.inner, ws_bytes - L.inner, st)) return e;
     WINO_LAUNCH_OUT(g, dim3((unsigned)((nout + 255) / 256)), Mb, out, N, H, W, Cout, g.th, g.tw, g.T, g.Tp, bias, relu,
-                accumulate, relu_x, bn_part);
+                accumulate, relu_x, bn_part, (const unsigned char *)nullptr);
     return 0;
 }
 
@@ -2195,22 +2216,40 @@
     return winograd_w_bytes(ConvGeom{N, H, W, Cin, Cout, KH, KW, stride, pad});
 }
 
-extern "C" int mrcnn_conv2d_bwd_data_f32(const float *gy, const float *w, float *gx, const float *relu_x, int N, int H, int W,
-                                         int Cin, int Cout, int KH, int KW, int stride, int pad,
-                                         int accumulate, float *wino_w, float *gbias, int gbias_accumulate, void *ws,
-                                         size_t ws_bytes, void *stream) {
-    const ConvGeom cg{N, H, W, Cin, Cout, KH, KW, stride, pad};
+static int check_active(const unsigned char *active, int n_active, const ConvGeom &cg, const char *who) {
+    if (active && n_active != cg.N) return mrcnn::fail_arg(MRCNN_E_INVALID, "%s: active has %d entries, the call %d images", who, n_active, cg.N);
+    return 0;
+}
+
+static int conv_bwd_data(const float *gy, const float *w, float *gx, const float *relu_x, const ConvGeom &cg,
+                         int accumulate, float *wino_w, float *gbias, int gbias_accumulate, void *ws,
+                         size_t ws_bytes, void *stream, const unsigned char *active) {
+    const int N = cg.N, Cin = cg.Cin, Cout = cg.Cout, KH = cg.KH, KW = cg.KW;
     if (int e = check_conv(gy, w, gx, cg)) return e;
     if (int e = check_bwd_data(cg)) return e;
     ConvP p = make_p(cg);
     if (bwd_data_takes_wino(cg, ws != nullptr, ws_bytes))
         return wino_conv(gy, w, gx, cg.transposed(), PASS_BWD_DATA, InBN{}, nullptr, 0, accumulate, relu_x, ws, ws_bytes, (hipStream_t)stream,
-                         nullptr, wino_w, wino_w ? gbias : nullptr, gbias_accumulate);
+                         nullptr, wino_w, wino_w ? gbias : nullptr, gbias_accumulate, nullptr, active);
     if (wino_w || gbias) return mrcnn::fail_arg(MRCNN_E_UNSUPPORTED, "conv2d_bwd_data: wino_w / gbias only on the Winograd path (mrcnn_conv2d_winograd_w_bytes() > 0)");
     p.a = gy; p.b = w; p.c = gx; p.accumulate = accumulate; p.relu_x = relu_x;
     p.bytes_a = (unsigned)((size_t)N * p.Ho * p.Wo * Cout * 4); p.bytes_b = (unsigned)((size_t)Cout * KH * KW * Cin * 4);
     const int nsteps = bwd_data_gemm(p);
     return run_data_conv<MODE_BWD_DATA>(p, nsteps, Cin, PASS_BWD_DATA, ws, ws_bytes, (hipStream_t)stream);
+}
+extern "C" int mrcnn_conv2d_bwd_data_f32(const float *gy, const float *w, float *gx, const float *relu_x, int N, int H, int W,
+                                         int Cin, int Cout, int KH, int KW, int stride, int pad,
+                                         int accumulate, float *wino_w, float *gbias, int gbias_accumulate, void *ws,
+                                         size_t ws_bytes, void *stream) {
+    return conv_bwd_data(gy, w, gx, relu_x, ConvGeom{N, H, W, Cin, Cout, KH, KW, stride, pad}, accumulate, wino_w, gbias, gbias_accumulate, ws,
+                         ws_bytes, stream, nullptr);
+}
+extern "C" int mrcnn_conv2d_bwd_data_active_f32(const float *gy, const float *w, float *gx, const float *relu_x, int N, int H, int W,
+                                                int Cin, int Cout, int KH, int KW, int stride, int pad, int accumulate,
+                                                const unsigned char *active, int n_active, void *ws, size_t ws_bytes, void *stream) {
+    const ConvGeom cg{N, H, W, Cin, Cout, KH, KW, stride, pad};
+    if (int e = check_active(active, n_active, cg, "conv2d_bwd_data_active")) return e;
+    return conv_bwd_data(gy, w, gx, relu_x, cg, accumulate, nullptr, nullptr, 0, ws, ws_bytes, stream, active);
 }
 
 static size_t bwd_filter_ws_bytes(const ConvGeom &cg) {
@@ -2235,7 +2274,8 @@
 }
 
 static int conv_bwd_filter(const float *x, const float *gy, float *gw, float *gbias, const ConvGeom &cg, int accumulate, const float *wino_v,
-                           const float *wino_w, void *ws, size_t ws_bytes, hipStream_t st, const InBN &inbn = InBN{}) {
+                           const float *wino_w, void *ws, size_t ws_bytes, hipStream_t st, const InBN &inbn = InBN{},
+                           const unsigned char *active = nullptr) {
     if (int e = check_conv(x, gy, gw, cg)) return e;
     if (g_debug_skip & 4) return 0;
     const size_t need = bwd_filter_ws_bytes(cg);
@@ -2248,7 +2288,7 @@
         if (wino_w && winograd_w_bytes(cg) == 0) wino_w = nullptr;
         float *bias_part = (float *)((char *)ws + L.total);
         int bias_rows = 0;
-        if (int e = wino_bwd_filter(x, gy, gw, cg, inbn, accumulate, ws, st, wino_v, wino_w, gbias ? bias_part : nullptr, &bias_rows)) return e;
+        if (int e = wino_bwd_filter(x, gy, gw, cg, inbn, accumulate, ws, st, wino_v, wino_w, gbias ? bias_part : nullptr, &bias_rows, active)) return e;
         if (!gbias) return 0;
         return bias_rows ? colsum_final(bias_part, gbias, bias_rows, Cout, accumulate, st) : colsum(gy, bias_part, gbias, P, Cout, accumulate, st);
     }
@@ -2273,6 +2313,15 @@
                            (hipStream_t)stream);
 }
 
+extern "C" int mrcnn_conv2d_bwd_filter_active_f32(const float *x, const float *gy, float *gw, float *gbias, int N,
+                                                  int H, int W, int Cin, int Cout, int KH, int KW, int stride, int pad,
+                                                  int accumulate, const float *wino_v, const unsigned char *active, int n_active, void *ws,
+                                                  size_t ws_bytes, void *stream) {
+    const ConvGeom cg{N, H, W, Cin, Cout, KH, KW, stride, pad};
+    if (int e = check_active(active, n_active, cg, "conv2d_bwd_filter_active")) return e;
+    return conv_bwd_filter(x, gy, gw, gbias, cg, accumulate, wino_v, nullptr, ws, ws_bytes, (hipStream_t)stream, InBN{}, active);
+}
+
 extern "C" int mrcnn_conv2d_bwd_filter_inbn_f32(const float *x, const float *in_gamma, const float *in_beta, const float *in_mean,
                                                 const float *in_invstd, const float *gy, float *gw, int N, int H, int W, int Cin, int Cout, int KH,
                                                 int KW, int stride, int pad, int accumulate, const float *wino_v, void *ws, size_t ws_bytes,
diff --git a/chainer-maskrcnn_amd/csrc/planes_gemm.h b/chainer-maskrcnn_amd/csrc/planes_gemm.h
--- a/chainer-maskrcnn_amd/csrc/planes_gemm.h
+++ b/chainer-maskrcnn_amd/csrc/planes_gemm.h
@@ -13,7 +13,17 @@
     int ldc;
     unsigned long long *stamps;
     int dbg;
+    const unsigned char *active;
+    int act_per, act_T;
 };
+
+__device__ __forceinline__ bool pg_rows_active(const unsigned char *__restrict__ active, int per, int T, int t0, int nrows) {
+    const int t1 = min(t0 + nrows, T);
+    bool any = false;
+    if (t0 < t1)
+        for (int n = t0 / per, n1 = (t1 - 1) / per; n <= n1; ++n) any |= active[n] != 0;
+    return any;
+}
 
 __device__ __forceinline__ void pg_dma16(__amdgpu_buffer_rsrc_t rs, unsigned char *lds, unsigned voff, unsigned soff) {
     __builtin_amdgcn_raw_ptr_buffer_load_lds(rs, (__attribute__((address_space(3))) void *)lds, 16, voff, soff, 0, 0);
@@ -497,7 +507,18 @@
     unsigned long long st_t0 = 0, st_r0 = 0;
     if (p.stamps) { st_t0 = pg_now(); st_r0 = __builtin_amdgcn_s_memrealtime(); }
     const int ntiles = p.tiles_m * p.tiles_n;
-    const int nj = vid0 < ntiles ? (ntiles - vid0 + (int)gridDim.x - 1) / (int)gridDim.x : 0;
+    const int nj_all = vid0 < ntiles ? (ntiles - vid0 + (int)gridDim.x - 1) / (int)gridDim.x : 0;
+    const bool masked = p.active != nullptr && nj_all <= 64;
+    unsigned long long am = 0;
+    if (masked) {
+        bool a = false;
+        if (lane < nj_all) {
+            const int m0 = (vid0 + lane * (int)gridDim.x) / p.tiles_n * PGB_BM;
+            a = pg_rows_active(p.active, p.act_per, p.act_T, m0 % p.batch_rows, PGB_BM);
+        }
+        am = __ballot(a);
+    }
+    const int nj = masked ? __popcll(am) : nj_all;
     const unsigned rowbytesA = (unsigned)p.K * 4u;
     const unsigned kblocks = (unsigned)p.K / 16u;
     const int nsteps = (int)kblocks;
@@ -506,7 +527,8 @@
     const auto rsA = __builtin_amdgcn_make_buffer_rsrc((void *)p.a, 0, p.bytes_a, 0x00020000);
     const auto rsB = __builtin_amdgcn_make_buffer_rsrc((void *)p.b, 0, p.bytes_b, 0x00020000);
     unsigned voffA[2], voffB[3];
-    int ij = 0, is = 0;
+    unsigned long long ri = am, rc = am;
+    int ij = (masked && am) ? __builtin_ctzll(am) : 0, is = 0;
     auto setup = [&](int j) {
         const int tile = vid0 + j * (int)gridDim.x;
         const int bx = tile / p.tiles_n, by = tile - bx * p.tiles_n;
@@ -536,7 +558,11 @@
 #pragma unroll
             for (int i = 0; i < 3; ++i) pg_dma16(rsB, sb + (wave + 8 * i) * 1024, voffB[i], soffB);
         }
-        if (++is == nsteps) { is = 0; ++ij; }
+        if (++is == nsteps) {
+            is = 0;
+            if (masked) { ri &= ri - 1; ij = ri ? __builtin_ctzll(ri) : nj_all; }
+            else ++ij;
+        }
     };
 
     f32x16 acc[2][4];
@@ -562,7 +588,7 @@
     __builtin_amdgcn_s_barrier();
     __builtin_amdgcn_sched_barrier(0);
     if (half) { __builtin_amdgcn_s_barrier(); __builtin_amdgcn_sched_barrier(0); }
-    int cs = 0, cj = 0;
+    int cs = 0, cj = (masked && am) ? __builtin_ctzll(am) : 0;
     for (int g = 0; g < S; ++g) {
         if (g + 2 < S) issue_next(b2);
         const unsigned a0 = fragA0 + b0, a1 = fragA1 + b0, bb = fragB + b0;
@@ -639,7 +665,9 @@
                         acc[tm][tn][e] = 0.0f;
                     }
                 }
-            cs = 0; ++cj;
+            cs = 0;
+            if (masked) { rc &= rc - 1; cj = rc ? __builtin_ctzll(rc) : nj_all; }
+            else ++cj;
         }
         __builtin_amdgcn_sched_barrier(0);
         __builtin_amdgcn_s_barrier();
@@ -654,6 +682,7 @@
     }
 }
 
+constexpr int PGG_MASK_STEPS = 128;
 __global__ __launch_bounds__(PGB_THREADS, 2) void k_pgemm_gpp(PlaneGemmP p) {
     constexpr int W_ROW = 3 * 512, W_STAGE = 16 * W_ROW, V_ROW = 1024, V_STAGE = 16 * V_ROW;
     static_assert(W_STAGE + V_STAGE == PGB_STAGE, "stage size");
@@ -670,7 +699,22 @@
     const int batch = vid % p.nbatch, split = vid / p.nbatch;
     const int m0 = bx * PGB_BM, n0 = by * PGB_BN;
     const int kbeg = split * p.kchunk, kend = min(p.K, kbeg + p.kchunk);
-    const int nsteps = kend > kbeg ? (kend - kbeg) / PG_BK : 0;
+    const int nsteps_all = kend > kbeg ? (kend - kbeg) / PG_BK : 0;
+    const bool masked = p.active != nullptr && nsteps_all <= PGG_MASK_STEPS;
+    unsigned long long am0 = 0, am1 = 0;
+    if (masked) {
+        am0 = __ballot(lane < nsteps_all && pg_rows_active(p.active, p.act_per, p.act_T, kbeg + lane * PG_BK, PG_BK));
+        am1 = __ballot(lane + 64 < nsteps_all && pg_rows_active(p.active, p.act_per, p.act_T, kbeg + (lane + 64) * PG_BK, PG_BK));
+    }
+    const int nsteps = masked ? __popcll(am0) + __popcll(am1) : nsteps_all;
+    unsigned knext = 0;
+    auto take = [&]() -> unsigned {
+        if (!masked) return knext++;
+        unsigned s;
+        if (am0) { s = (unsigned)__builtin_ctzll(am0); am0 &= am0 - 1; }
+        else { s = 64u + (unsigned)__builtin_ctzll(am1); am1 &= am1 - 1; }
+        return s;
+    };
     const unsigned rowW = (unsigned)p.M * 6u, rowV = (unsigned)p.N * 4u;
 
     const auto rsA = __builtin_amdgcn_make_buffer_rsrc((void *)p.a, 0, p.bytes_a, 0x00020000);
@@ -719,7 +763,7 @@
     const bool loads = !(p.dbg & 8), mfma = !(p.dbg & 1);
     unsigned b0 = 0, b1 = PGB_STAGE, b2 = 2 * PGB_STAGE;
     if (nsteps > 0) {
-        if (loads) { issue(b0, 0); if (nsteps > 1) issue(b1, 1); }
+        if (loads) { issue(b0, take()); if (nsteps > 1) issue(b1, take()); }
         if (nsteps > 1) asm volatile("s_waitcnt vmcnt(5)" ::: "memory");
         else asm volatile("s_waitcnt vmcnt(0)" ::: "memory");
     }
@@ -730,7 +774,7 @@
 #define PG_DSTR(DST, ADDR, OFF) asm volatile("ds_read_b64_tr_b16 %0, %1 offset:%2" : "=v"(DST) : "v"(ADDR), "n"(OFF) : "memory")
 #define PG_DSR2ST64(DST, ADDR, O0, O1) asm volatile("ds_read2st64_b32 %0, %1 offset0:%2 offset1:%3" : "=v"(DST) : "v"(ADDR), "n"(O0), "n"(O1) : "memory")
     for (int s = 0; s < nsteps; ++s) {
-        if (s + 2 < nsteps && loads) issue(b2, (unsigned)(s + 2));
+        if (s + 2 < nsteps && loads) issue(b2, take());
         pg_u32x2 rv[2][4];
         const unsigned av = offV + b0;
 #pragma unroll
diff --git a/chainer-maskrcnn_amd/csrc/targets.hip b/chainer-maskrcnn_amd/csrc/targets.hip
--- a/chainer-maskrcnn_amd/csrc/targets.hip
+++ b/chainer-maskrcnn_amd/csrc/targets.hip
@@ -449,3 +449,23 @@
     MRCNN_LAUNCH_CHECK();
     return 0;
 }
+
+namespace {
+__global__ __launch_bounds__(256) void k_active_rows(const int32_t *__restrict__ n_pos, int rows_per_block, int R, unsigned char *__restrict__ active) {
+    const int r = blockIdx.x * 256 + threadIdx.x;
+    if (r >= R) return;
+    const int blk = r / rows_per_block;
+    active[r] = (r - blk * rows_per_block) < n_pos[blk] ? 1 : 0;
+}
+}
+
+extern "C" int mrcnn_active_rows_u8(const int32_t *n_pos, int n_blocks, int rows_per_block, unsigned char *active, void *stream) {
+    if (n_blocks < 0 || rows_per_block <= 0 || (long long)n_blocks * rows_per_block >= (1ll << 31))
+        return mrcnn::fail_arg(MRCNN_E_INVALID, "active_rows: bad sizes (%d blocks of %d rows)", n_blocks, rows_per_block);
+    if (n_blocks == 0) return 0;
+    if (!n_pos || !active) return mrcnn::fail_arg(MRCNN_E_INVALID, "active_rows: null pointer");
+    const int R = n_blocks * rows_per_block;
+    hipLaunchKernelGGL(k_active_rows, dim3(mrcnn::cdiv(R, 256)), dim3(256), 0, (hipStream_t)stream, n_pos, rows_per_block, R, active);
+    MRCNN_LAUNCH_CHECK();
+    return 0;
+}
diff --git a/include/mrcnn_hip.h b/include/mrcnn_hip.h
--- a/include/mrcnn_hip.h
+++ b/include/mrcnn_hip.h
@@ -119,6 +119,14 @@
                                 int W, int Cin, int Cout, int KH, int KW, int stride, int pad, int accumulate,
                                 const float *wino_v, const float *wino_w,
                                 void *ws, size_t ws_bytes, void *stream);
+int mrcnn_conv2d_bwd_data_active_f32(const float *gy, const float *w, float *gx, const float *relu_x, int N, int H, int W, int Cin,
+                                     int Cout, int KH, int KW, int stride, int pad, int accumulate, const unsigned char *active,
+                                     int n_active, void *ws, size_t ws_bytes, void *stream);
+int mrcnn_conv2d_bwd_filter_active_f32(const float *x, const float *gy, float *gw, float *gbias, int N, int H,
+                                       int W, int Cin, int Cout, int KH, int KW, int stride, int pad, int accumulate,
+                                       const float *wino_v, const unsigned char *active, int n_active,
+                                       void *ws, size_t ws_bytes, void *stream);
+int mrcnn_active_rows_u8(const int32_t *n_pos, int n_blocks, int rows_per_block, unsigned char *active, void *stream);
 
 size_t mrcnn_bn_workspace_bytes(int P, int C);
 int mrcnn_bn_train_fwd_f32(const float *x, const float *gamma, const float *beta, const float *residual,
```
